# LarsELund/Bayesian-Neural-Nets

Hardware: AMD Instinct MI355X
Metric: ELBO forward samples/sec, 784-1200^2-10 MNF MLP, batch 4096 per GPU (higher is better)
Workload: dtype f16 (row-scaled fp16 hi + lo split of the f32 operands: 3 mean + 1 variance MFMA products, f32 accumulate)

## Files before the change

bayesian-neural-nets_amd/_lib.py:

```python
import ctypes
import os

_HERE = os.path.dirname(os.path.abspath(__file__))
LIB_PATH = os.environ.get("LBBNN_LIB_PATH") or os.path.join(_HERE, "csrc", "liblbbnn_hip.so")

c_p = ctypes.c_void_p
c_i = ctypes.c_int
c_u32 = ctypes.c_uint32
c_i64 = ctypes.c_int64
c_u64 = ctypes.c_uint64


class Priors(ctypes.Structure):
    _fields_ = [("mu_prior", ctypes.c_float), ("sigma_prior", ctypes.c_float),
                ("alpha_prior", ctypes.c_float), ("bias_mu_prior", ctypes.c_float),
                ("bias_sigma_prior", ctypes.c_float)]

    def __init__(self, mu_prior=0.0, sigma_prior=1.0, alpha_prior=0.05, bias_mu_prior=0.0,
                 bias_sigma_prior=1.0):
        super().__init__(mu_prior, sigma_prior, alpha_prior, bias_mu_prior, bias_sigma_prior)


MAX_FLOW_T = 16
MAX_LAYERS = 4
# ... 81 lines not shown


class AdamList(ctypes.Structure):
    _fields_ = [("p", c_p * ADAM_MAX_TENSORS), ("g", c_p * ADAM_MAX_TENSORS), ("m", c_p * ADAM_MAX_TENSORS),
                ("v", c_p * ADAM_MAX_TENSORS), ("numel", c_i64 * ADAM_MAX_TENSORS), ("n", c_i)]


ADAM_GROUPS_MAX_TENSORS = 64
ADAM_CHUNK = 4096
ADAM_F_DECOUPLED = 0x1
ADAM_F_INACTIVE = 0x2


class AdamHyper(ctypes.Structure):
    _fields_ = [("lr", ctypes.c_float), ("beta1", ctypes.c_float), ("beta2", ctypes.c_float), ("eps", ctypes.c_float),
                ("weight_decay", ctypes.c_float), ("flags", c_u32)]


class AdamGroupList(ctypes.Structure):
    _fields_ = [("p", c_p * ADAM_GROUPS_MAX_TENSORS), ("g", c_p * ADAM_GROUPS_MAX_TENSORS), ("m", c_p * ADAM_GROUPS_MAX_TENSORS),
                ("v", c_p * ADAM_GROUPS_MAX_TENSORS), ("mask", c_p * ADAM_GROUPS_MAX_TENSORS),
                ("numel", c_i64 * ADAM_GROUPS_MAX_TENSORS), ("group", c_i * ADAM_GROUPS_MAX_TENSORS), ("n", c_i)]


SGD_F_NESTEROV = 0x1
SGD_F_INACTIVE = 0x2


class SgdHyper(ctypes.Structure):
    _fields_ = [("lr", ctypes.c_float), ("momentum", ctypes.c_float), ("dampening", ctypes.c_float),
                ("weight_decay", ctypes.c_float), ("flags", c_u32)]


class StudyArgs(ctypes.Structure):
    _fields_ = [("params", c_p), ("exp_avg", c_p), ("exp_avg_sq", c_p), ("step", c_p), ("rng", c_p), ("skipped", c_p),
                ("x", c_p), ("x_rstride", c_i64), ("y", c_p), ("y_rstride", c_i64), ("priors", c_p), ("priors_rstride", c_i),
                ("hyper", c_p), ("lr", c_p), ("lr_rstride", c_i64), ("restarts", c_p), ("n_restarts", c_i), ("history", c_p),
                ("R", c_i), ("I", c_i), ("O", c_i), ("N", c_i), ("batch", c_i),
                ("epochs", c_i), ("first_epoch", c_i), ("n_epochs", c_i)]


STUDY_MAX_I, STUDY_MAX_O, STUDY_MAX_WEIGHTS, STUDY_MAX_BATCH, STUDY_HISTORY_COLS = 256, 16, 1024, 4096, 6


class CopyList(ctypes.Structure):
    _fields_ = [("dst", c_p * ADAM_MAX_TENSORS), ("src", c_p * ADAM_MAX_TENSORS), ("numel", c_i64 * ADAM_MAX_TENSORS), ("n", c_i)]


class DenseLayer(ctypes.Structure):
    _fields_ = [("q0_mean", c_p), ("q0_log_var", c_p), ("zt", ctypes.POINTER(DenseTransform)), ("rt", ctypes.POINTER(DenseTransform)),
                ("eps_fwd", c_p), ("eps_kl", c_p), ("z_fwd", c_p), ("z_kl", c_p), ("scal", c_p), ("work", c_p),
                ("Tz", c_i), ("Tr", c_i), ("I", c_i), ("want_kl", c_i), ("layer_id", c_u32), ("save", c_p), ("draw_masks", c_i)]


class DenseGrad(ctypes.Structure):
    _fields_ = [("w_in", c_p), ("b_in", c_p), ("w_mid", c_p * 3), ("b_mid", c_p * 3),
                ("w_a", c_p), ("b_a", c_p), ("w_b", c_p), ("b_b", c_p)]


MAX_DENSE_T = 8
MAX_HIDDEN = 128


class GateBwdArgs(ctypes.Structure):
    _fields_ = [(n, c_p) for n in ("mu", "rho", "gamma_alpha", "cgamma", "eps_w", "bias_mu", "bias_rho", "eps_b", "bias_a",
                                   "bias_b", "tau_b", "weight_a", "weight_b", "tau_w", "pa", "pb", "dW", "g_sum", "g_lp", "g_lq",
                                   "d_mu", "d_rho", "d_cgamma", "d_alpha", "w_out", "d_bias_mu", "d_bias_rho", "d_bias_a",
                                   "d_bias_b", "d_tau_b", "d_scalars", "rows")] + \
               [("O", c_i), ("I", c_i), ("exact", c_i), ("layer_id", c_u32)]


class GateDrawArgs(ctypes.Structure):
    _fields_ = [("g", GateArgs), ("lambdal", c_p), ("gammas", c_p), ("alpha", c_p), ("tau_w", c_p), ("tau_b", c_p),
                ("temperature", ctypes.c_float)]


class GateBwdDrawArgs(ctypes.Structure):
    _fields_ = [("g", GateBwdArgs), ("lambdal", c_p), ("d_lambdal", c_p), ("temperature", ctypes.c_float)]


class GateMemberDesc(ctypes.Structure):
    _fields_ = [(n, c_p) for n in ("mu", "rho", "lambdal", "bias_mu", "bias_rho", "w_out", "bias_out", "gate_rows", "gates")] + \
               [(n, c_i) for n in ("O", "I", "ld", "flags", "exact")] + [("layer_id", c_u32)]


class FrozenDesc(ctypes.Structure):
    _fields_ = [(n, c_p) for n in ("weight_mu", "weight_rho", "lambdal", "bias_rho", "q0_mean", "q0_log_var")] + \
               [("z_flow", PlanarFlow)] + \
               [(n, c_p) for n in ("e0", "e_w", "var_w", "bias_var", "kept_rows", "z_fwd", "e_w_members")] + \
               [("z_mstride", c_i64)] + [(n, c_i) for n in ("O", "I", "ld", "flags", "mode")] + \
               [("cut", ctypes.c_float), ("layer_id", c_u32)]


class CompactMap(ctypes.Structure):
    _fields_ = [("rows", c_p), ("cols", c_p), ("O_full", c_i), ("I_full", c_i)]


class SparseDesc(ctypes.Structure):
    _fields_ = [(n, c_p) for n in ("weight_mu", "weight_rho", "lambdal", "bias_rho", "row_ptr", "col", "mean", "var", "bias_var",
                                   "kept_rows")] + [("O", c_i), ("I", c_i), ("nnz", c_i), ("cut", ctypes.c_float)]


MAX_LEVELS = 16


class SparseLevelsDesc(ctypes.Structure):
    _fields_ = [(n, c_p) for n in ("weight_mu", "weight_rho", "lambdal", "bias_rho", "row_ptr", "col", "mean", "var", "bias_var",
                                   "kept_rows")] + [("O", c_i), ("I", c_i), ("nnz", c_i), ("levels", c_i),
                                                    ("cut", ctypes.c_float * MAX_LEVELS)]


class SparseDrawDesc(ctypes.Structure):
    _fields_ = [(n, c_p) for n in ("col", "mean", "var", "bias_mu", "bias_var", "z")] + [("z_mstride", c_i64), ("tpos", c_p), ("wt", c_p), ("w", c_p),
               ("w_mstride", c_i64), ("b", c_p), ("b_mstride", c_i64), ("O", c_i), ("I", c_i), ("nnz", c_i), ("layer_id", c_u32)]


class SparseGatherArgs(ctypes.Structure):
    _fields_ = [("ptr", c_p), ("idx", c_p), ("slot", c_p), ("w", c_p), ("w_mstride", c_i64), ("bias", c_p), ("b_mstride", c_i64),
                ("a", c_p), ("a_mstride", c_i64), ("h", c_p), ("h_mstride", c_i64), ("out", c_p), ("o_mstride", c_i64)] + \
               [(n, c_i) for n in ("lda", "ldh", "ldo", "B", "K", "N", "nnz", "mode", "relu", "out_rows", "a_shared", "blocks",
                                   "per_member")] + [("dot_bias", c_p), ("dot_b_mstride", c_i64), ("dot_acc", c_p)]


class MemberStatsArgs(ctypes.Structure):
    _fields_ = [("t", c_p), ("t_mstride", c_i64)] + [(n, c_i) for n in ("ldt", "S", "C", "F", "B")] + \
               [(n, c_p) for n in ("mean", "std", "prob_pos", "prob_neg", "members", "logits")] + \
               [("ldl", c_i), ("n_logits", c_i), ("targets", c_p), ("intercept", c_p), ("residual", c_p)]


class BaseSparseDesc(ctypes.Structure):
    _fields_ = [(n, c_p) for n in ("mu", "rho", "lambdal", "bias_mu", "bias_rho", "row_ptr", "col", "mean", "sigma", "b_mu",
                                   "b_sigma", "kept_rows")] + [("O", c_i), ("I", c_i), ("nnz", c_i)]


class BaseSparseDrawDesc(ctypes.Structure):
    _fields_ = [(n, c_p) for n in ("row_ptr", "col", "mean", "sigma", "b_mu", "b_sigma", "tpos", "wt", "w")] + \
               [("w_mstride", c_i64), ("b", c_p), ("b_mstride", c_i64), ("O", c_i), ("I", c_i), ("nnz", c_i), ("layer_id", c_u32)]


class BaseFrozenDesc(ctypes.Structure):
    _fields_ = [(n, c_p) for n in ("mu", "rho", "lambdal", "bias_mu", "bias_rho", "w_mu", "w_sigma", "alpha", "e_w", "b_mu",
                                   "b_sigma", "kept_rows", "alpha_rows", "keep")] + \
               [(n, c_i) for n in ("O", "I", "ld", "flags", "exact")] + [("layer_id", c_u32)]


class DenseMembers(ctypes.Structure):
    _fields_ = [("q0_mean", c_p), ("q0_log_var", c_p), ("zt", ctypes.POINTER(DenseTransform)), ("T", c_i), ("I", c_i),
                ("layer_id", c_u32), ("z_fwd", c_p), ("z_mstride", c_i64), ("mask_out", c_p)]


class OutGradArgs(ctypes.Structure):
    _fields_ = [(n, c_p) for n in ("g_out", "out", "std", "eps", "rng", "gm", "gv", "gmT", "gvT", "g_sum", "gv_sum", "work")] + \
               [("row_offset", c_i64), ("rng_stream", c_u32)] + [(n, c_i) for n in ("B", "O", "ldg", "ldo", "relu")] + \
               [("gv_scale", c_p)]


class FlowStep(ctypes.Structure):
    _fields_ = [("p0", c_p), ("p1", c_p), ("p2", c_p), ("type", c_i), ("M", c_i)]


class FlowChain(ctypes.Structure):
    _fields_ = [("step", FlowStep * MAX_FLOW_T), ("n", c_i)]


class PlanarGrad(ctypes.Structure):
    _fields_ = [("u", c_p * MAX_FLOW_T), ("w", c_p * MAX_FLOW_T), ("b", c_p * MAX_FLOW_T)]


class FlowBwdArgs(ctypes.Structure):
    _fields_ = [(n, c_p) for n in ("q0_mean", "q0_log_var", "eps_fwd", "eps_kl", "r0_b1", "r0_b2", "aux",
                                   "dz_fwd", "dz_kl", "g_kl", "bias_mu", "bias_rho", "g_sum", "gv_sum")] + \
               [("z_flow", PlanarFlow), ("r_flow", PlanarFlow), ("priors", Priors)] + \
               [(n, c_p) for n in ("d_q0_mean", "d_q0_log_var", "d_r0_b1", "d_r0_b2", "d_bias_mu", "d_bias_rho")] + \
               [("d_z_flow", PlanarGrad), ("d_r_flow", PlanarGrad), ("work", c_p), ("O", c_i), ("I", c_i),
                ("rng", c_p), ("layer_id", c_u32)]


class DenseBwdArgs(ctypes.Structure):
    _fields_ = [(n, c_p) for n in ("q0_mean", "q0_log_var", "eps_fwd", "eps_kl", "r0_b1", "r0_b2", "aux",
                                   "dz_fwd", "dz_kl", "g_kl", "bias_mu", "bias_rho", "g_sum", "gv_sum")] + \
               [("zt", ctypes.POINTER(DenseTransform)), ("rt", ctypes.POINTER(DenseTransform)),
                ("d_zt", ctypes.POINTER(DenseGrad)), ("d_rt", ctypes.POINTER(DenseGrad)), ("priors", Priors)] + \
               [(n, c_p) for n in ("d_q0_mean", "d_q0_log_var", "d_r0_b1", "d_r0_b2", "d_bias_mu", "d_bias_rho", "save", "work")] + \
               [("Tz", c_i), ("Tr", c_i), ("O", c_i), ("I", c_i), ("rng", c_p), ("layer_id", c_u32)]


EVAL_COUNTS = 6
EVAL_COUNT_NAMES = ("rows", "rows_with_target", "bad_targets", "correct_ensemble", "correct_posterior_mean",
                    "entropy_nonfinite")


class EvalMetricsArgs(ctypes.Structure):
    _fields_ = [("logp", c_p), ("m_stride", c_i64), ("ldp", c_i64), ("mean_logp", c_p), ("ldm", c_i64), ("target", c_p),
                ("ens_logp", c_p), ("pred_ensemble", c_p), ("pred_mean", c_p), ("entropy", c_p),
                ("counts", c_p), ("correct_member", c_p), ("confusion", c_p), ("sums", c_p), ("work", c_p),
                ("S", c_i), ("B", c_i), ("C", c_i)]


MONITOR_COUNTS = 8
MONITOR_COUNT_NAMES = ("steps", "rows", "correct", "bad_targets", "nonfinite_rows", "nonfinite_steps", "skipped_steps", "nll_rows")
MONITOR_SUMS = 5
MONITOR_SUM_NAMES = ("nll_sum", "kl_term_sum", "loss_sum", "last_nll", "last_loss")
MONITOR_WORDS = MONITOR_COUNTS + MONITOR_SUMS
MONITOR_SKIPPED_STEPS = 6


UNC_COUNTS = 6
UNC_COUNT_NAMES = ("rows", "rows_with_target", "bad_targets", "correct_bma", "nonfinite_rows", "log_score_nonfinite")
UNC_SUMS = 6
UNC_SUM_NAMES = ("total_entropy", "expected_entropy", "mutual_information", "confidence", "brier", "log_score")


class EvalUncertaintyArgs(ctypes.Structure):
    _fields_ = [("logp", c_p), ("m_stride", c_i64), ("ldp", c_i64), ("target", c_p),
                ("bma_probs", c_p), ("pred_bma", c_p), ("confidence", c_p), ("total_entropy", c_p), ("expected_entropy", c_p),
                ("mutual_information", c_p), ("brier", c_p), ("log_score", c_p),
                ("counts", c_p), ("sums", c_p), ("bin_rows", c_p), ("bin_rows_with_target", c_p), ("bin_correct", c_p),
                ("bin_conf_sum", c_p), ("hist", c_p), ("work", c_p),
                ("S", c_i), ("B", c_i), ("C", c_i), ("conf_bins", c_i), ("hist_bins", c_i), ("ent_scale", ctypes.c_float)]


REG_COUNTS = 5
REG_COUNT_NAMES = ("elements", "elements_with_target", "bad_targets", "nonfinite_elements", "scored_elements")
REG_SUMS = 8
REG_SUM_NAMES = ("sq_err", "abs_err", "log_density", "epistemic_var", "total_var", "y", "y2", "posterior_mean_sq_err")
REG_ROW_KEYS = ("pred_mean", "epistemic_var", "aleatoric_var", "total_std", "sq_err", "log_density", "pit")


class EvalRegressionArgs(ctypes.Structure):
    _fields_ = [("out", c_p), ("m_stride", c_i64), ("ldp", c_i64), ("mean_out", c_p), ("ldm", c_i64), ("target", c_p),
                ("ldt", c_i64), ("log_var", c_p)] + [(n, c_p) for n in REG_ROW_KEYS] + \
               [("counts", c_p), ("sums", c_p), ("pit_hist", c_p), ("work", c_p), ("S", c_i), ("B", c_i), ("O", c_i),
                ("pit_bins", c_i)]


SCORE_MAX_LEVELS = 4
SCORE_MAX_MEMBERS = 64
SCORE_COUNTS = REG_COUNTS + SCORE_MAX_LEVELS
SCORE_SUMS = REG_SUMS + 2 + 2 * SCORE_MAX_LEVELS
SCORE_SUM_NAMES = REG_SUM_NAMES + ("aleatoric_var", "crps")
SCORE_ROW_KEYS = REG_ROW_KEYS + ("crps",)
SCORE_LEVEL_KEYS = ("lower", "upper", "interval_score")


class EvalScoresArgs(ctypes.Structure):
    _fields_ = [("out", c_p), ("m_stride", c_i64), ("ldp", c_i64), ("mean_out", c_p), ("ldm", c_i64), ("target", c_p),
                ("ldt", c_i64), ("log_var", c_p), ("lv_mstride", c_i64), ("lv_ld", c_i64)] + \
               [(n, c_p) for n in SCORE_ROW_KEYS + SCORE_LEVEL_KEYS] + \
               [("counts", c_p), ("sums", c_p), ("pit_hist", c_p), ("work", c_p), ("S", c_i), ("B", c_i), ("O", c_i),
                ("pit_bins", c_i), ("n_levels", c_i), ("levels", ctypes.c_float * SCORE_MAX_LEVELS)]


STRUCTURE_MAX_LAYERS = 16
STRUCTURE_MAX_WIDTH = 4096


class StructureDesc(ctypes.Structure):
    _fields_ = [("lambdal", c_p), ("O", c_i), ("I", c_i), ("ld", c_i), ("layer_id", c_u32)]


EXPLAIN_SEED, EXPLAIN_MASK, EXPLAIN_FINISH = 0, 1, 2
GATHER_FORWARD, GATHER_SWEEP, GATHER_FINISH = 0, 1, 2
MEMBER_BLOCKS_MAX = 65535
EXPLAIN_MAX_OUTPUTS = 16
EXPLAIN_MAX_ROWS = 1 << 24


class ExplainStepArgs(ctypes.Structure):
    _fields_ = [("mode", c_i), ("B", c_i), ("C", c_i), ("width", c_i), ("g", c_p), ("ldg", c_i64), ("w", c_p), ("ldw", c_i64),
                ("w_rows", c_i), ("targets", c_p), ("h", c_p), ("ldh", c_i64), ("bias", c_p), ("bias_out", c_p),
                ("intercept", c_p), ("active", c_p), ("ld_active", c_i64), ("mask_out", c_p), ("ldm", c_i64),
                ("logits", c_p), ("ldl", c_i64), ("map", c_p), ("full_width", c_i), ("contributions", c_p), ("ldc", c_i64),
                ("residual", c_p)]


SIGNATURES = {
    "lbbnn_abi_version": (c_i, []),
    "lbbnn_error_string": (ctypes.c_char_p, [c_i]),
    "lbbnn_operand_ld": (c_i, [c_i]),
    "lbbnn_weight_pass": (c_i, [c_p, c_p, c_p, c_p, c_p, c_p, c_p, ctypes.POINTER(Priors),
                                c_p, c_p, c_i, c_p, c_p, c_p, c_p, c_i, c_i, c_i, c_p]),
    "lbbnn_weight_pass_f16": (c_i, [c_p, c_p, c_p, c_p, c_p, c_p, c_p, ctypes.POINTER(Priors),
                                    c_p, c_p, c_i, c_p, c_p, c_p, c_p, c_p, c_p, c_i, c_i, c_i, c_p]),
    "lbbnn_lrt_gemm_ex": (c_i, [ctypes.POINTER(GemmDesc), c_p]),
    "lbbnn_head_slab_floats": (c_i64, [c_i, c_i]),
    "lbbnn_format_x": (c_i, [c_p, c_i, c_p, c_i, c_i, c_i, c_p]),
    "lbbnn_lrt_gemm": (c_i, [c_p, c_i, c_p, c_p, c_i, c_p, c_p, c_p, c_p, c_p, c_u32, c_i64,
                             c_p, c_i, c_i, c_i, c_i, c_i, c_p]),
    "lbbnn_lrt_gemm_plan": (c_i, [c_i, c_i, c_i, c_i, c_i, c_i, c_i, c_i, c_i, ctypes.POINTER(GemmPlan)]),
    "lbbnn_transpose_operand": (c_i, [c_p, c_i, c_i, c_i, c_p, c_i, c_i, c_i, c_p]),
    "lbbnn_weight_pass_backward_workspace": (c_i64, [c_i, c_i]),
    "lbbnn_weight_pass_backward": (c_i, [ctypes.POINTER(WpbArgs), c_p]),
    "lbbnn_layers_dense_flows": (c_i, [ctypes.POINTER(DenseLayer), c_i, c_p, c_p]),
    "lbbnn_layers_dense_flows_phase": (c_i, [ctypes.POINTER(DenseLayer), c_i, c_p, c_i, c_p]),
    "lbbnn_flow_dense_save_size": (c_i64, [c_i, c_i, c_i]),
    "lbbnn_mnf_flow_dense_backward_workspace": (c_i64, [c_i]),
    "lbbnn_mnf_flow_dense_backward": (c_i, [ctypes.POINTER(DenseBwdArgs), c_p]),
    "lbbnn_mnf_flow_dense_backward_batch": (c_i, [ctypes.POINTER(DenseBwdArgs), c_i, c_p]),
    "lbbnn_flow_dense_apply_workspace": (c_i64, [c_i, c_i]),
    "lbbnn_flow_dense_apply": (c_i, [ctypes.POINTER(DenseTransform), c_i, c_i, c_p, c_i, c_p, c_p, c_p]),
    "lbbnn_flow_dense_apply_backward": (c_i, [ctypes.POINTER(DenseTransform), ctypes.POINTER(DenseGrad), c_i, c_i, c_p, c_p,
                                              c_p, c_i, c_p, c_p, c_p]),
    "lbbnn_q0_rows": (c_i, [c_p, c_p, c_p, c_p, c_u32, c_i, c_i, c_p, c_p]),
    "lbbnn_flow_dense_rows_max_dim": (c_i, []),
    "lbbnn_flow_dense_rows": (c_i, [ctypes.POINTER(DenseTransform), c_i, c_p, c_p, c_p, c_u32, c_u64, c_p, c_i, c_i, c_i,
                                    c_p, c_i, c_p, c_p]),
    "lbbnn_gate_backward": (c_i, [ctypes.POINTER(GateBwdArgs), c_p, c_p]),
    "lbbnn_format_operand": (c_i, [c_p, c_i, c_i, c_i, c_p, c_i, c_i, c_i, c_p]),
    "lbbnn_multi_copy": (c_i, [ctypes.POINTER(CopyList), c_p]),
    "lbbnn_adam_step": (c_i, [ctypes.POINTER(AdamList), ctypes.c_float, ctypes.c_float, ctypes.c_float, ctypes.c_float,
                              ctypes.c_float, c_p, c_i, c_p]),
    "lbbnn_adam_step_groups": (c_i, [ctypes.POINTER(AdamGroupList), c_p, c_p, c_i, c_p, c_p, c_i, c_p]),
    "lbbnn_sgd_step_groups": (c_i, [ctypes.POINTER(AdamGroupList), c_p, c_p, c_i, c_p, c_p, c_i, c_p]),
    "lbbnn_adam_step_groups_guarded": (c_i, [ctypes.POINTER(AdamGroupList), c_p, c_p, c_i, c_p, c_p, c_i, c_p, c_p, c_p]),
    "lbbnn_sgd_step_groups_guarded": (c_i, [ctypes.POINTER(AdamGroupList), c_p, c_p, c_i, c_p, c_p, c_i, c_p, c_p, c_p]),
    "lbbnn_lrt_study_fit": (c_i, [ctypes.POINTER(StudyArgs), c_p]),
    "lbbnn_grad_sumsq_workspace": (c_i64, [c_i64]),
    "lbbnn_grad_sumsq": (c_i, [ctypes.POINTER(AdamGroupList), c_p, c_i64, c_i64, ctypes.c_float, c_p, c_p, c_p]),
    "lbbnn_matmul_splitk": (c_i, [c_p, c_i, c_p, c_i, c_p, c_i, c_i, c_i, c_i, c_i, c_p]),
    "lbbnn_lrt_gemm_combine": (c_i, [c_p, c_i, c_p, c_i, c_p, c_i, c_p, c_i, c_p, c_i, c_i, c_i, c_i, c_i, c_p]),
    "lbbnn_dx_combine": (c_i, [c_p, c_p, c_p, c_i, c_i, c_i, c_p]),
    "lbbnn_output_grad_workspace": (c_i64, [c_i, c_i]),
    "lbbnn_output_grad": (c_i, [ctypes.POINTER(OutGradArgs), c_p]),
    "lbbnn_head_dx": (c_i, [c_p, c_p, c_i, c_p, c_p, c_i, c_p, c_i, c_p, c_i, c_i, c_i, c_i, c_p]),
    "lbbnn_head_dw": (c_i, [c_p, c_p, c_i, c_p, c_i, c_p, c_p, c_i, c_i, c_i, c_i, c_p]),
    "lbbnn_reduce_partials_batch": (c_i, [c_p, c_i, c_p]),
    "lbbnn_flow_chain": (c_i, [ctypes.POINTER(FlowChain), c_p, c_p, c_p, c_p, c_p, c_u32, c_i, c_p, c_p, c_p, c_p, c_p]),
    "lbbnn_flow_chain_rows": (c_i, [ctypes.POINTER(FlowChain), c_p, c_i, c_i, c_i, c_p, c_i, c_p, c_p]),
    "lbbnn_mnf_aux_backward": (c_i, [c_p, c_p, c_p, c_p, c_p, c_p, c_p, c_i, c_i, c_p, c_p, c_p, c_p, c_u32, c_p]),
    "lbbnn_mnf_aux_backward_batch": (c_i, [c_p, c_i, c_p]),
    "lbbnn_bias_backward": (c_i, [c_p, c_p, c_p, c_p, c_p, c_p, c_p, c_p, c_i, c_p]),
    "lbbnn_bias_backward_partials": (c_i, [c_p, c_i, c_i, c_i, c_p, c_p, c_p, c_p, c_p, c_p, c_p]),
    "lbbnn_mnf_flow_backward_workspace": (c_i64, [c_i, c_i, c_i]),
    "lbbnn_mnf_flow_planar_backward": (c_i, [ctypes.POINTER(FlowBwdArgs), c_p]),
    "lbbnn_mnf_flow_planar_backward_batch": (c_i, [ctypes.POINTER(FlowBwdArgs), c_i, c_p]),
    "lbbnn_mnf_flow_planar": (c_i, [c_p, c_p, c_p, c_p, c_p, c_i, c_p, c_p, c_p, c_i, c_p, c_p,
                                    c_p, c_u32, c_p, c_p, c_p, c_i, c_i, c_p]),
    "lbbnn_flow_dense_workspace": (c_i64, [c_i]),
    "lbbnn_mnf_flow_dense": (c_i, [c_p, c_p, ctypes.POINTER(DenseTransform), c_i, ctypes.POINTER(DenseTransform), c_i,
                                   c_p, c_p, c_p, c_u32, c_p, c_p, c_p, c_p, c_i, c_i, c_p]),
    "lbbnn_kl_finalize": (c_i, [c_p, c_p, c_p, c_i, c_p, c_p, c_p, c_p, c_p, c_i, c_p,
                                ctypes.POINTER(Priors), c_p, c_u32, c_p, c_p, c_i, c_p]),
    "lbbnn_flow_planar_form": (c_i, [c_i, c_p, c_p, c_p, c_p, c_p, c_i]),
    "lbbnn_kl_finalize_form": (c_i, [c_i, c_p, c_p, c_p, c_p, c_i]),
    "lbbnn_layers_prepare": (c_i, [ctypes.POINTER(LayerDesc), c_i, c_p, c_p]),
    "lbbnn_layers_operands_snap": (c_i, [ctypes.POINTER(LayerDesc), c_i, c_p, c_p, c_u64, c_p]),
    "lbbnn_layers_operands_x": (c_i, [ctypes.POINTER(LayerDesc), c_i, c_p, c_p, c_u64, c_p, c_i, c_p, c_i, c_i, c_i, c_p]),
    "lbbnn_ensemble_operands": (c_i, [ctypes.POINTER(LayerDesc), c_i, c_i, c_p, c_u64, c_p]),
    "lbbnn_lrt_gemm_members": (c_i, [c_p, c_i, c_i64, c_p, c_i64, c_p, c_i, c_p, c_p, c_p, c_u32, c_i64, c_u64,
                                     c_p, c_i, c_i64, c_i, c_i, c_i, c_i, c_i, c_p]),
    "lbbnn_layers_operands": (c_i, [ctypes.POINTER(LayerDesc), c_i, c_p, c_p]),
    "lbbnn_layers_finalize": (c_i, [ctypes.POINTER(LayerDesc), c_i, c_p, ctypes.c_uint64, c_p, c_p]),
    "lbbnn_kl_total": (c_i, [c_p, c_i, c_p, c_p]),
    "lbbnn_fold_rows": (c_i, [c_p, c_i, c_i, c_i, c_p, c_p]),
    "lbbnn_gate_sample": (c_i, [ctypes.POINTER(GateArgs), c_p, c_p]),
    "lbbnn_vd_operands": (c_i, [c_p, c_p, c_p, c_i, c_i, c_i, c_i, c_p]),
    "lbbnn_weight_operands_t": (c_i, [c_p, c_p, c_p, c_p, c_p, c_p, c_i, c_i, c_i, c_i, c_p]),
    "lbbnn_rng_advance": (c_i, [c_p, c_u64, c_p]),
    "lbbnn_philox_normal": (c_i, [c_p, c_u32, c_i64, c_i64, c_i64, c_p, c_p]),
    "lbbnn_gate_sample_draw": (c_i, [ctypes.POINTER(GateDrawArgs), c_p, c_p]),
    "lbbnn_gate_backward_draw": (c_i, [ctypes.POINTER(GateBwdDrawArgs), c_p, c_p]),
    "lbbnn_philox_uniform": (c_i, [c_p, c_u32, c_i64, c_i64, c_i64, c_p, c_p]),
    "lbbnn_gate_members": (c_i, [ctypes.POINTER(GateMemberDesc), c_i, c_i, c_i, ctypes.c_float, c_p, c_u64, c_p]),
    "lbbnn_gemm_members_mean": (c_i, [c_p, c_i, c_i64, c_p, c_i64, c_i, c_p, c_i64, c_p, c_i, c_i64, c_i, c_i, c_i, c_i, c_i,
                                      c_p]),
    "lbbnn_vd_gemm_members": (c_i, [c_p, c_i, c_i64, c_p, c_p, c_i, c_p, c_p, c_u32, c_i64, c_u64, c_p, c_i, c_i64,
                                    c_i, c_i, c_i, c_i, c_i, c_i, c_p]),
    "lbbnn_philox_std_gamma": (c_i, [c_p, c_u32, c_p, c_p, c_i64, c_p, c_p]),
    "lbbnn_gamma_grad": (c_i, [c_p, c_p, c_i64, c_p, c_p]),
    "lbbnn_elbo_loss": (c_i, [c_p, c_i, c_p, c_i, c_i, c_p, ctypes.c_float, c_p, c_p]),
    "lbbnn_elbo_loss_monitor": (c_i, [c_p, c_i, c_p, c_i, c_i, c_p, ctypes.c_float, c_p, c_p, c_p, c_p]),
    "lbbnn_elbo_loss_backward": (c_i, [c_p, c_p, c_i, c_i, ctypes.c_float, c_p, c_p, c_p]),
    "lbbnn_elbo_loss_backward_logits": (c_i, [c_p, c_p, c_p, c_i, c_i, c_i, ctypes.c_float, c_p, c_p, c_p, c_p]),
    "lbbnn_log_softmax_backward": (c_i, [c_p, c_i, c_p, c_i, c_p, c_i, c_i, c_i, c_p]),
    "lbbnn_log_softmax_rows": (c_i, [c_p, c_i, c_p, c_i, c_i, c_i, c_p]),
    "lbbnn_binary_head": (c_i, [c_p, c_i, c_i, c_i, c_p, c_i, c_p, c_i, c_p]),
    "lbbnn_elbo_bce_loss": (c_i, [c_p, c_i, c_p, c_i, c_i, c_i, c_p, ctypes.c_float, c_p, c_p, c_i, c_p]),
    "lbbnn_elbo_bce_loss_monitor": (c_i, [c_p, c_i, c_p, c_i, c_i, c_i, c_p, ctypes.c_float, c_p, c_p, c_i, c_p, c_p, c_p]),
    "lbbnn_elbo_bce_loss_backward": (c_i, [c_p, c_p, c_i, c_p, c_i, c_i, c_i, ctypes.c_float, c_p, c_p, c_p, c_p]),
    "lbbnn_sigmoid_backward": (c_i, [c_p, c_i, c_p, c_i, c_p, c_i, c_i, c_i, c_p]),
    "lbbnn_frozen_operands": (c_i, [ctypes.POINTER(FrozenDesc), c_i, c_p]),
    "lbbnn_frozen_members": (c_i, [ctypes.POINTER(FrozenDesc), c_i, c_i, c_p, c_u64, c_p]),
    "lbbnn_flow_dense_members_max_dim": (c_i, []),
    "lbbnn_flow_dense_members": (c_i, [ctypes.POINTER(DenseMembers), c_i, c_i, c_p, c_u64, c_p]),
    "lbbnn_frozen_members_dense": (c_i, [ctypes.POINTER(FrozenDesc), ctypes.POINTER(DenseMembers), c_i, c_i, c_p, c_u64, c_p]),
    "lbbnn_frozen_operands_compact": (c_i, [ctypes.POINTER(FrozenDesc), ctypes.POINTER(CompactMap), c_i, c_p]),
    "lbbnn_frozen_members_compact": (c_i, [ctypes.POINTER(FrozenDesc), ctypes.POINTER(CompactMap), c_i, c_i, c_p, c_u64, c_p]),
    "lbbnn_gather_columns": (c_i, [c_p, c_i, c_p, c_i, c_p, c_i, c_i, c_p]),
    "lbbnn_sparse_count": (c_i, [ctypes.POINTER(SparseDesc), c_i, c_p]),
    "lbbnn_sparse_pack": (c_i, [ctypes.POINTER(SparseDesc), c_i, c_p]),
    "lbbnn_frozen_members_z": (c_i, [ctypes.POINTER(FrozenDesc), c_i, c_i, c_p, c_u64, c_p]),
    "lbbnn_sparse_layer_members": (c_i, [c_p, c_p, c_p, c_p, c_i, c_p, c_p, c_p, c_i, c_i64, c_p, c_i64, c_p, c_u32, c_i64, c_u64,
                                         c_p, c_i, c_i64, c_i, c_i, c_i, c_i, c_i, c_i, c_p]),
    "lbbnn_sparse_count_levels": (c_i, [ctypes.POINTER(SparseLevelsDesc), c_i, c_p]),
    "lbbnn_sparse_pack_levels": (c_i, [ctypes.POINTER(SparseLevelsDesc), c_i, c_p]),
    "lbbnn_sparse_layer_levels": (c_i, [c_p, c_p, c_p, c_p, c_i, c_p, c_p, c_p, c_i, c_i64, c_p, c_i64, c_p, c_u32, c_i64, c_u64,
                                        c_p, c_i, c_i64, c_i, c_i, c_i, c_i, c_i, c_i, c_i, c_p]),
    "lbbnn_base_frozen_operands": (c_i, [ctypes.POINTER(BaseFrozenDesc), ctypes.POINTER(CompactMap), c_i, c_i, ctypes.c_float, c_p]),
    "lbbnn_base_frozen_members": (c_i, [ctypes.POINTER(BaseFrozenDesc), ctypes.POINTER(CompactMap), c_i, c_i, c_i, ctypes.c_float,
                                        ctypes.POINTER(c_p), ctypes.POINTER(c_p), ctypes.POINTER(c_p), c_p, c_u64, c_p]),
    "lbbnn_eval_metrics_work_bytes": (c_i64, [c_i, c_i, c_i]),
    "lbbnn_eval_metrics": (c_i, [ctypes.POINTER(EvalMetricsArgs), c_p]),
    "lbbnn_eval_uncertainty_work_bytes": (c_i64, [c_i, c_i, c_i, c_i]),
    "lbbnn_eval_uncertainty": (c_i, [ctypes.POINTER(EvalUncertaintyArgs), c_p]),
    "lbbnn_eval_regression_work_bytes": (c_i64, [c_i, c_i, c_i]),
    "lbbnn_eval_regression": (c_i, [ctypes.POINTER(EvalRegressionArgs), c_p]),
    "lbbnn_eval_regression_scores_work_bytes": (c_i64, [c_i, c_i, c_i, c_i]),
    "lbbnn_eval_regression_scores": (c_i, [ctypes.POINTER(EvalScoresArgs), c_p]),
    "lbbnn_elbo_gaussian_loss": (c_i, [c_p, c_i, c_p, c_i, c_p, c_i, c_i, c_i, c_p, ctypes.c_float, c_p, c_p, c_p, c_p]),
    "lbbnn_elbo_gaussian_loss_monitor": (c_i, [c_p, c_i, c_p, c_i, c_p, c_i, c_i, c_i, c_p, ctypes.c_float, c_p, c_p, c_p, c_p, c_p,
                                               c_p]),
    "lbbnn_elbo_gaussian_loss_backward": (c_i, [c_p, c_p, c_i, c_p, c_i, c_p, c_i, c_i, c_i, ctypes.c_float, c_p, c_p, c_p, c_p,
                                                c_p]),
    "lbbnn_gate_structure_width": (c_i64, [ctypes.POINTER(StructureDesc), c_i]),
    "lbbnn_gate_structure": (c_i, [ctypes.POINTER(StructureDesc), c_i, c_i, c_p, c_p, c_p, c_p, c_p, c_p, c_p, c_p]),
    "lbbnn_explain_step": (c_i, [ctypes.POINTER(ExplainStepArgs), c_p]),
    "lbbnn_explain_work_bytes": (c_i64, [c_i, c_i, c_i]),
    "lbbnn_explain_totals": (c_i, [c_p, c_i64, c_p, c_i, c_i, c_i, c_p, c_p, c_p, c_p, c_p]),
    "lbbnn_explain_operand": (c_i, [c_p, c_i, c_i, c_i, c_p, c_p]),
    "lbbnn_sparse_draw_members": (c_i, [ctypes.POINTER(SparseDrawDesc), c_i, c_i, c_p, c_i, c_p]),
    "lbbnn_sparse_gather_members": (c_i, [ctypes.POINTER(SparseGatherArgs), c_p]),
    "lbbnn_explain_seed": (c_i, [c_p, c_p, c_i, c_p, c_p, c_i64, c_p, c_i, c_p, c_i, c_i, c_i, c_i, c_p, c_u64, c_p]),
    "lbbnn_explain_member_stats": (c_i, [ctypes.POINTER(MemberStatsArgs), c_p]),
    "lbbnn_base_sparse_count": (c_i, [ctypes.POINTER(BaseSparseDesc), c_i, ctypes.c_float, c_p]),
    "lbbnn_base_sparse_pack": (c_i, [ctypes.POINTER(BaseSparseDesc), c_i, ctypes.c_float, c_p]),
    "lbbnn_base_sparse_draw_members": (c_i, [ctypes.POINTER(BaseSparseDrawDesc), c_i, c_i, c_p, c_u64, c_i, c_p]),
}

_lib = None


def lib():
    global _lib
    if _lib is None:
        if not os.path.exists(LIB_PATH):
            raise RuntimeError(
                "bnn_amd: HIP extension not built: %s is missing. Build it with "
                "`python -c 'import __graft_entry__ as g; g.build()'` or "
                "`make -C bayesian-neural-nets_amd/csrc` (hipcc, --offload-arch=gfx950). "
                "There is no CPU fallback." % LIB_PATH)
        l = ctypes.CDLL(LIB_PATH)
        for name, (res, args) in SIGNATURES.items():
            fn = getattr(l, name)
            fn.restype = res
            fn.argtypes = args
        _lib = l
    if RECORD is not None:
        return _Recorder(_lib)
    return _lib


RECORD = None


class _Recorder:
    def __init__(self, l):
        self._l = l

    def __getattr__(self, name):
        fn = getattr(self._l, name)

        def call(*args):
            if RECORD is not None and fn.argtypes and fn.argtypes[-1] is ctypes.c_void_p:
                RECORD.append((name, fn, args))
            return fn(*args)
        return call


def check(rc, what):
    if rc != 0:
        msg = lib().lbbnn_error_string(rc)
        raise RuntimeError("bnn_amd: %s failed (%d): %s" % (what, rc, msg.decode() if msg else "?"))
# ... 6 lines not shown
```

bayesian-neural-nets_amd/csrc/lrt_gemm.hip:

```cpp
#include <cstdlib>
#include "lbbnn_device.h"
#include "lbbnn_internal.h"
#include "kl_piggy.h"
#include "gemm_common.h"
#include "../../include/lbbnn.h"

namespace {

using namespace lbbnn;
typedef float floatx4 __attribute__((ext_vector_type(4)));

constexpr int BK = 16;
constexpr int LDS_LD = 20;

struct GemmArgs {
    const float* x; const float* e_w; const float* var_w;
    const float* bias_mean; const float* bias_var; const float* var_scale;
    const float* eps; const uint64_t* rng;
    float* out;
    float* std_out;
    long long row_offset;
    int ldx, ld, ldo, B, I, O;
    uint32_t rng_stream;
    int relu, log_softmax;
    int kchunk;
    long long split_stride;
    const float* comb_x; const float* comb_add;
    int ld_cx, ld_ca;
    FinalizePiggy fin;
    int single16;
    int members;
    long long x_ms, w_ms, o_ms, b_ms;
    unsigned long long m_adv, m_off;
    int fan;
};

__device__ __forceinline__ GemmArgs member_view(const GemmArgs& in) {
    GemmArgs a = in;
    a.m_off = 0;
    if (in.members > 1) {
        const long long m = blockIdx.z;
        a.x = in.x + m * in.x_ms; a.e_w = in.e_w + m * in.w_ms; a.out = in.out + m * in.o_ms;
        if (in.bias_mean) a.bias_mean = in.bias_mean + m * in.b_ms;
        a.m_off = (unsigned long long)m * in.m_adv;
    }
    return a;
}

struct EpiCtx { bool ovec; uint64_t seed, offs; };

template <bool MEAN_ONLY>
__device__ __forceinline__ EpiCtx make_epi_ctx(const GemmArgs& a) {
    EpiCtx c;
    c.ovec = ((a.O & 3) == 0) && ((a.ldo & 3) == 0) && ((reinterpret_cast<uintptr_t>(a.out) & 15u) == 0) &&
             (!a.eps || (reinterpret_cast<uintptr_t>(a.eps) & 15u) == 0) &&
             (!a.std_out || (reinterpret_cast<uintptr_t>(a.std_out) & 15u) == 0);
    c.seed = 0; c.offs = 0;
    if (!MEAN_ONLY && !a.eps) { c.seed = a.rng[0]; c.offs = a.rng[1] + a.m_off; }
    return c;
}

struct OConst { float bm[4], bv[4], vs[4]; };

__device__ __forceinline__ void load4_or_fill(const float* p, int o, int O, float fill, float out[4]) {
    if (!p) { out[0] = out[1] = out[2] = out[3] = fill; return; }
    if (o + 3 < O && ((reinterpret_cast<uintptr_t>(p + o) & 15u) == 0)) {
        const float4 t = *reinterpret_cast<const float4*>(p + o);
        out[0] = t.x; out[1] = t.y; out[2] = t.z; out[3] = t.w;
    } else {
#pragma unroll
        for (int r = 0; r < 4; ++r) out[r] = (o + r < O) ? p[o + r] : fill;
    }
}

__device__ __forceinline__ OConst load_oconst(const GemmArgs& a, int o) {
    OConst c;
    load4_or_fill(a.bias_mean, o, a.O, 0.f, c.bm);
    load4_or_fill(a.bias_var, o, a.O, 0.f, c.bv);
    load4_or_fill(a.var_scale, o, a.O, 1.f, c.vs);
    return c;
}

template <bool MEAN_ONLY>
__device__ __forceinline__ void epilogue4(const GemmArgs& a, const EpiCtx& c, const OConst& oc, int b, int o,
                                          const floatx4& am, const floatx4& av, const float* e_in, const float* cx_in,
                                          const float* ca_in, float res[4], float sd[4]) {
    float e[4] = {0.f, 0.f, 0.f, 0.f};
    if (!MEAN_ONLY) {
        if (a.eps) {
#pragma unroll
            for (int r = 0; r < 4; ++r) e[r] = e_in[r];
        } else {
            philox_normal4(c.seed, c.offs, a.rng_stream, (uint64_t)(a.row_offset + b), (uint32_t)(o >> 2), e);
        }
    }
#pragma unroll
    for (int r = 0; r < 4; ++r) {
        float mean = am[r] + oc.bm[r];
        sd[r] = 0.f;
        if (!MEAN_ONLY) { sd[r] = sqrt_hw(av[r] * oc.vs[r] + oc.bv[r]); mean += sd[r] * e[r]; }
        res[r] = a.relu ? fmaxf(mean, 0.f) : mean;
    }
    if (MEAN_ONLY && a.comb_x) {
#pragma unroll
        for (int r = 0; r < 4; ++r) res[r] = ca_in[r] + 2.f * cx_in[r] * res[r];
    }
}

__device__ __forceinline__ void load4_rows(const float* p, bool vec, int o, int O, float out[4]) {
    if (vec) { const float4 t = *reinterpret_cast<const float4*>(p); out[0] = t.x; out[1] = t.y; out[2] = t.z; out[3] = t.w; }
    else {
#pragma unroll
        for (int r = 0; r < 4; ++r) out[r] = (o + r < O) ? p[r] : 0.f;
    }
}

__device__ __forceinline__ void store4_rows(float* p, bool vec, int o, int O, const float v[4]) {
    if (vec) *reinterpret_cast<float4*>(p) = make_float4(v[0], v[1], v[2], v[3]);
    else {
#pragma unroll
        for (int r = 0; r < 4; ++r) if (o + r < O) p[r] = v[r];
    }
}

__device__ __forceinline__ void fan_store4(const GemmArgs& a, const EpiCtx& ec, const OConst& oc, int m, int b, int o,
                                           const floatx4& am, const floatx4& av) {
    EpiCtx em = ec;
    em.offs = ec.offs + (unsigned long long)m * a.m_adv;
    float res[4], sd[4];
    epilogue4<false>(a, em, oc, b, o, am, av, nullptr, nullptr, nullptr, res, sd);
    store4_rows(a.out + (size_t)m * a.o_ms + (size_t)b * a.ldo + o, ec.ovec, o, a.O, res);
}

template <int TO, int TB, bool MEAN_ONLY, bool FAN = false>
__device__ __forceinline__ void epilogue_tile(const GemmArgs& a, int o0, int q, int brow0,
                                              const floatx4 (&accm)[TO][TB], const floatx4 (&accv)[TO][TB]) {
    static_assert(!FAN || !MEAN_ONLY, "fan-out draws noise");
    EpiCtx ec = make_epi_ctx<MEAN_ONLY>(a);
    OConst oc[TO];
#pragma unroll
    for (int i = 0; i < TO; ++i) {
        const int o = o0 + i * 16 + 4 * q;
        if (o < a.O) oc[i] = load_oconst(a, o);
    }
    if (FAN) {
        __builtin_amdgcn_sched_barrier(0);
        for (int m = 0; m < a.fan; ++m) {
#pragma unroll
            for (int i = 0; i < TO; ++i) {
                const int o = o0 + i * 16 + 4 * q;
                if (o >= a.O) continue;
#pragma unroll
                for (int j = 0; j < TB; ++j) {
                    const int b = brow0 + j * 16;
                    if (b < a.B) fan_store4(a, ec, oc[i], m, b, o, accm[i][j], accv[i][j]);
                }
            }
        }
        return;
    }
    const bool pre_eps = !MEAN_ONLY && a.eps != nullptr;
    const bool pre_comb = MEAN_ONLY && a.comb_x != nullptr;
    const bool comb_vec = pre_comb && ec.ovec && ((a.ld_cx | a.ld_ca) & 3) == 0 &&
                          ((reinterpret_cast<uintptr_t>(a.comb_x) | reinterpret_cast<uintptr_t>(a.comb_add)) & 15u) == 0;
    float pa[TO][TB][4], pb[TO][TB][4];
    if (pre_eps || pre_comb) {
#pragma unroll
        for (int i = 0; i < TO; ++i) {
            const int o = o0 + i * 16 + 4 * q;
#pragma unroll
            for (int j = 0; j < TB; ++j) {
                const int b = brow0 + j * 16;
                if (o >= a.O || b >= a.B) continue;
                if (pre_eps) load4_rows(a.eps + (size_t)b * a.O + o, ec.ovec, o, a.O, pa[i][j]);
                else {
                    load4_rows(a.comb_x + (size_t)b * a.ld_cx + o, comb_vec, o, a.O, pa[i][j]);
                    load4_rows(a.comb_add + (size_t)b * a.ld_ca + o, comb_vec, o, a.O, pb[i][j]);
                }
            }
        }
    }
    __builtin_amdgcn_sched_barrier(0);
#pragma unroll
    for (int i = 0; i < TO; ++i) {
        const int o = o0 + i * 16 + 4 * q;
        if (o >= a.O) continue;
#pragma unroll
        for (int j = 0; j < TB; ++j) {
            const int b = brow0 + j * 16;
            if (b >= a.B) continue;
            float res[4], sd[4];
            epilogue4<MEAN_ONLY>(a, ec, oc[i], b, o, accm[i][j], accv[i][j], pa[i][j], pa[i][j], pb[i][j], res, sd);
            store4_rows(a.out + (size_t)b * a.ldo + o, ec.ovec, o, a.O, res);
            if (!MEAN_ONLY && a.std_out) store4_rows(a.std_out + (size_t)b * a.O + o, ec.ovec, o, a.O, sd);
        }
    }
}

template <int TO, int TB, int WB, bool MEAN_ONLY, bool XVEC, bool FAN = false>
__global__ __launch_bounds__(WB * 64, 2) void lrt_gemm_f32_kernel(const GemmArgs a_in) {
    const GemmArgs a = member_view(a_in);
    constexpr int NT = WB * 64;
    constexpr int BN = TO * 16;
    constexpr int BM = TB * WB * 16;
    constexpr int NW = MEAN_ONLY ? 1 : 2;
    extern __shared__ __attribute__((aligned(16))) float smem[];
    constexpr int ROWS = BM + NW * BN;
    constexpr int BUF = ROWS * LDS_LD;

    const int tid = threadIdx.x, lane = tid & 63, wv = tid >> 6;
    const int lr = lane & 15, q = lane >> 4;
    const int o0 = blockIdx.x * BN;
    const int b0 = blockIdx.y * BM;

    constexpr int SLOTS = ROWS * 4;
    constexpr int NIT = (SLOTS + NT - 1) / NT;
    const float* gp[NIT];
    int loff[NIT];
    int kcol[NIT];
#pragma unroll
    for (int it = 0; it < NIT; ++it) {
        int sl = tid + it * NT;
        if (sl >= SLOTS) sl -= SLOTS;
        const int row = sl >> 2, c4 = (sl & 3) << 2;
        loff[it] = row * LDS_LD + c4;
        if (row < BM) {
            const int bb = min(b0 + row, a.B - 1);
            gp[it] = a.x + (size_t)bb * a.ldx + c4;
            kcol[it] = c4;
        } else {
            const int wr = row - BM;
            const bool isv = (!MEAN_ONLY) && wr >= BN;
            const int oo = min(o0 + (isv ? wr - BN : wr), a.O - 1);
            gp[it] = (isv ? a.var_w : a.e_w) + (size_t)oo * a.ld + c4;
            kcol[it] = -1;
        }
    }
    float4 stage[NIT];
    auto load_full = [&](int c) {
#pragma unroll
        for (int it = 0; it < NIT; ++it) {
            const float* p = gp[it] + c * BK;
            if (XVEC) stage[it] = *reinterpret_cast<const float4*>(p);
            else if (kcol[it] < 0) stage[it] = *reinterpret_cast<const float4*>(p);
            else stage[it] = make_float4(p[0], p[1], p[2], p[3]);
        }
    };
    auto load_tail = [&](int c) {
#pragma unroll
        for (int it = 0; it < NIT; ++it) {
            const float* p = gp[it] + c * BK;
            if (kcol[it] < 0) {
                stage[it] = *reinterpret_cast<const float4*>(p);
            } else {
                const int k = c * BK + kcol[it];
                float4 v = make_float4(0.f, 0.f, 0.f, 0.f);
                if (k + 0 < a.I) v.x = p[0];
                if (k + 1 < a.I) v.y = p[1];
                if (k + 2 < a.I) v.z = p[2];
                if (k + 3 < a.I) v.w = p[3];
                stage[it] = v;
            }
        }
    };
    auto store_chunk = [&](float* buf) {
#pragma unroll
        for (int it = 0; it < NIT; ++it) *reinterpret_cast<float4*>(buf + loff[it]) = stage[it];
    };

    floatx4 accm[TO][TB], accv[TO][TB];
#pragma unroll
    for (int i = 0; i < TO; ++i)
#pragma unroll
        for (int j = 0; j < TB; ++j) { accm[i][j] = floatx4{0.f, 0.f, 0.f, 0.f}; accv[i][j] = floatx4{0.f, 0.f, 0.f, 0.f}; }

    const int nfull = a.I / BK;
    const int nchunks = (a.I + BK - 1) / BK;
    if (nfull > 0) load_full(0); else load_tail(0);
    store_chunk(smem);
    __syncthreads();

    const int xoff = (wv * TB * 16 + lr) * LDS_LD + 4 * q;
    const int woff = (BM + lr) * LDS_LD + 4 * q;

    auto compute = [&](const float* cur) {
        float xf[TB][4], xs[TB][4], wm[TO][4], wq[TO][4];
#pragma unroll
        for (int j = 0; j < TB; ++j) {
            const float4 t = *reinterpret_cast<const float4*>(cur + xoff + j * 16 * LDS_LD);
            xf[j][0] = t.x; xf[j][1] = t.y; xf[j][2] = t.z; xf[j][3] = t.w;
        }
#pragma unroll
        for (int i = 0; i < TO; ++i) {
            const float4 t = *reinterpret_cast<const float4*>(cur + woff + i * 16 * LDS_LD);
            wm[i][0] = t.x; wm[i][1] = t.y; wm[i][2] = t.z; wm[i][3] = t.w;
            if (!MEAN_ONLY) {
                const float4 u = *reinterpret_cast<const float4*>(cur + woff + (BN + i * 16) * LDS_LD);
                wq[i][0] = u.x; wq[i][1] = u.y; wq[i][2] = u.z; wq[i][3] = u.w;
            }
        }
#pragma unroll
        for (int j = 0; j < TB; ++j)
#pragma unroll
            for (int k = 0; k < 4; ++k) xs[j][k] = xf[j][k] * xf[j][k];
#pragma unroll
        for (int k = 0; k < 4; ++k) {
#pragma unroll
            for (int i = 0; i < TO; ++i) {
#pragma unroll
                for (int j = 0; j < TB; ++j) {
                    accm[i][j] = __builtin_amdgcn_mfma_f32_16x16x4f32(wm[i][k], xf[j][k], accm[i][j], 0, 0, 0);
                    if (!MEAN_ONLY)
                        accv[i][j] = __builtin_amdgcn_mfma_f32_16x16x4f32(wq[i][k], xs[j][k], accv[i][j], 0, 0, 0);
                }
            }
        }
    };

    int c = 0;
    for (; c + 1 < nfull; ++c) {
        load_full(c + 1);
        __builtin_amdgcn_sched_barrier(0);
        compute(smem + (c & 1) * BUF);
        __builtin_amdgcn_sched_barrier(0);
        store_chunk(smem + ((c & 1) ^ 1) * BUF);
        __syncthreads();
    }
    for (; c < nchunks; ++c) {
        const bool more = (c + 1) < nchunks;
        if (more) load_tail(c + 1);
        __builtin_amdgcn_sched_barrier(0);
        compute(smem + (c & 1) * BUF);
        __builtin_amdgcn_sched_barrier(0);
        if (more) store_chunk(smem + ((c & 1) ^ 1) * BUF);
        __syncthreads();
    }

    epilogue_tile<TO, TB, MEAN_ONLY, FAN>(a, o0, q, b0 + wv * TB * 16 + lr, accm, accv);
}

constexpr int DROW = 16;

__device__ __forceinline__ int swz(int rowgrp) { return (0x78 >> (2 * (rowgrp & 3))) & 3; }

template <int TO, int TB, int WB, bool MEAN_ONLY, bool FAN = false>
__global__ __launch_bounds__(WB * 64, 2) void lrt_gemm_f32_dma_kernel(const GemmArgs a_in) {
    const GemmArgs a = member_view(a_in);
    constexpr int BN = TO * 16, BM = TB * WB * 16;
    constexpr int NW = MEAN_ONLY ? 1 : 2;
    constexpr int ROWS = BM + NW * BN;
    constexpr int NG = ROWS / 16;
    constexpr int NPW = (NG + WB - 1) / WB;
    constexpr int BUF = ROWS * DROW;
    extern __shared__ __attribute__((aligned(16))) float smem[];

    const int tid = threadIdx.x, lane = tid & 63;
    const int wv = __builtin_amdgcn_readfirstlane(tid >> 6);
    const int lr = lane & 15, q = lane >> 4;
    if (a.fin.n > 0 && blockIdx.y == gridDim.y - 1) {
        if (blockIdx.x == 0) kl_finalize_piggy<WB>(kernarg_as<GemmArgs>()->fin, smem);
        return;
    }
    int tox, tby;
    tile_of_block(tox, tby, a.fin.n > 0 ? 1 : 0);
    const int o0 = tox * BN;
    const int b0 = tby * BM;

    const int srow = lane >> 2;
    const int scol = ((lane & 3) ^ swz(lane >> 4)) << 2;
    const float* gp[NPW];
#pragma unroll
    for (int u = 0; u < NPW; ++u) {
        const int g = wv + WB * u;
        const int row = 16 * g + srow;
        if (row < BM) {
            gp[u] = a.x + (size_t)min(b0 + row, a.B - 1) * a.ldx + scol;
        } else {
            const int wr = row - BM;
            const bool isv = (!MEAN_ONLY) && wr >= BN;
            const int oo = min(o0 + (isv ? wr - BN : wr), a.O - 1);
            gp[u] = (isv ? a.var_w : a.e_w) + (size_t)oo * a.ld + scol;
        }
    }
    auto dma_chunk = [&](int c, float* buf) {
#pragma unroll
        for (int u = 0; u < NPW; ++u) {
            const int g = wv + WB * u;
            if (g < NG)
                __builtin_amdgcn_global_load_lds(
                    (const __attribute__((address_space(1))) void*)(gp[u] + c * BK),
                    (__attribute__((address_space(3))) void*)(buf + g * 16 * DROW), 16, 0, 0);
        }
    };

    floatx4 accm[TO][TB], accv[TO][TB];
#pragma unroll
    for (int i = 0; i < TO; ++i)
#pragma unroll
        for (int j = 0; j < TB; ++j) { accm[i][j] = floatx4{0.f, 0.f, 0.f, 0.f}; accv[i][j] = floatx4{0.f, 0.f, 0.f, 0.f}; }

    const int fcol = (q ^ swz(lr >> 2)) << 2;
    const int xoff = (wv * TB * 16 + lr) * DROW + fcol;
    const int woff = (BM + lr) * DROW + fcol;

    float xf[TB][4], xs[TB][4], wm[TO][4], wq[TO][4];
    auto read_frags = [&](const float* cur) {
#pragma unroll
        for (int j = 0; j < TB; ++j) {
            const float4 t = *reinterpret_cast<const float4*>(cur + xoff + j * 16 * DROW);
            xf[j][0] = t.x; xf[j][1] = t.y; xf[j][2] = t.z; xf[j][3] = t.w;
        }
#pragma unroll
        for (int i = 0; i < TO; ++i) {
            const float4 t = *reinterpret_cast<const float4*>(cur + woff + i * 16 * DROW);
            wm[i][0] = t.x; wm[i][1] = t.y; wm[i][2] = t.z; wm[i][3] = t.w;
            if (!MEAN_ONLY) {
                const float4 u = *reinterpret_cast<const float4*>(cur + woff + (BN + i * 16) * DROW);
                wq[i][0] = u.x; wq[i][1] = u.y; wq[i][2] = u.z; wq[i][3] = u.w;
            }
        }
    };
    auto mfmas = [&]() {
#pragma unroll
        for (int j = 0; j < TB; ++j)
#pragma unroll
            for (int k = 0; k < 4; ++k) xs[j][k] = xf[j][k] * xf[j][k];
#pragma unroll
        for (int k = 0; k < 4; ++k) {
#pragma unroll
            for (int i = 0; i < TO; ++i) {
#pragma unroll
                for (int j = 0; j < TB; ++j) {
                    accm[i][j] = __builtin_amdgcn_mfma_f32_16x16x4f32(wm[i][k], xf[j][k], accm[i][j], 0, 0, 0);
                    if (!MEAN_ONLY)
                        accv[i][j] = __builtin_amdgcn_mfma_f32_16x16x4f32(wq[i][k], xs[j][k], accv[i][j], 0, 0, 0);
                }
            }
        }
    };

    const int nchunks = a.I / BK;
    dma_chunk(0, smem);
    __syncthreads();
    for (int c = 0; c < nchunks; ++c) {
        read_frags(smem + (c & 1) * BUF);
        __builtin_amdgcn_sched_barrier(0);
        if (c + 1 < nchunks) dma_chunk(c + 1, smem + ((c & 1) ^ 1) * BUF);
        __builtin_amdgcn_sched_barrier(0);
        mfmas();
        __builtin_amdgcn_sched_barrier(0);
        __syncthreads();
    }

    epilogue_tile<TO, TB, MEAN_ONLY, FAN>(a, o0, q, b0 + wv * TB * 16 + lr, accm, accv);
}

typedef __bf16 bf16x8 __attribute__((ext_vector_type(8)));
typedef __bf16 bf16x2 __attribute__((ext_vector_type(2)));
typedef float floatx2 __attribute__((ext_vector_type(2)));
constexpr int BKS = 32;

__device__ __forceinline__ int swzx(int r) { return (((r >> 1) & 3) << 1) | ((r >> 3) & 1); }

typedef _Float16 f16x8 __attribute__((ext_vector_type(8)));
typedef _Float16 f16x2 __attribute__((ext_vector_type(2)));
template <int TO, int TB, int WB, bool MEAN_ONLY, int NP, bool F16, bool FAN>
__device__ __forceinline__ void lrt_gemm_bf16x3_body(const GemmArgs& a_in) {
    static_assert(!F16 || NP == 1, "fp16 operands exist in the single-product form only");
    const GemmArgs a = member_view(a_in);
    constexpr int BN = TO * 16, BM = TB * WB * 16;
    constexpr int NWR = MEAN_ONLY ? 1 : 2;
    constexpr int XB = BM * 128;
    constexpr int WRB = BN * 128;
    constexpr int BUFB = XB + NWR * WRB;
    constexpr int NGX = BM / 8, NGW = BN / 8;
    constexpr int NG = NGX + NWR * NGW;
    constexpr int NPW = (NG + WB - 1) / WB;
    extern __shared__ __attribute__((aligned(16))) char smc[];

    const int tid = threadIdx.x, lane = tid & 63;
    const int wv = __builtin_amdgcn_readfirstlane(tid >> 6);
    const int lr = lane & 15, q = lane >> 4;
    if (a.fin.n > 0 && blockIdx.y == gridDim.y - 1) {
        if (blockIdx.x == 0) kl_finalize_piggy<WB>(kernarg_as<GemmArgs>()->fin, reinterpret_cast<float*>(smc));
        return;
    }
    int tox, tby;
    tile_of_block(tox, tby, a.fin.n > 0 ? 1 : 0);
    const int o0 = tox * BN;
    const int b0 = tby * BM;
    const int kbeg = a.kchunk ? (int)blockIdx.z * a.kchunk : 0;
    const int Iloc = a.kchunk ? min(a.I - kbeg, a.kchunk) : a.I;
    const char* const eb = reinterpret_cast<const char*>(a.e_w);
    const char* const vb = reinterpret_cast<const char*>(a.var_w);
    const char* const zsrc = eb + split_hi_index(0, a.I, a.ld) * 2;

    const unsigned xbytes = (unsigned)min((size_t)0x7FFFFFF0u, ((size_t)(a.B - 1) * a.ldx + a.I) * 4);
    const unsigned wbytes = (unsigned)min((size_t)0x7FFFFFF0u, (size_t)a.O * a.ld * 4);
    const __amdgpu_buffer_rsrc_t rx = __builtin_amdgcn_make_buffer_rsrc((void*)a.x, 0, (int)xbytes, 0x00020000);
    const __amdgpu_buffer_rsrc_t re = __builtin_amdgcn_make_buffer_rsrc((void*)a.e_w, 0, (int)wbytes, 0x00020000);
    const __amdgpu_buffer_rsrc_t rv = __builtin_amdgcn_make_buffer_rsrc((void*)(MEAN_ONLY ? a.e_w : a.var_w), 0, (int)wbytes, 0x00020000);
    (void)eb; (void)vb; (void)zsrc;
    int gv[NPW];
    int kx[NPW];
#pragma unroll
    for (int u = 0; u < NPW; ++u) {
        const int g = wv + WB * u;
        if (g < NGX) {
            const int row = 8 * g + (lane >> 3);
            const int slot = (lane & 7) ^ swzx(row & 15);
            gv[u] = (int)(((size_t)min(b0 + row, a.B - 1) * a.ldx + kbeg) * 4) + 16 * slot;
            kx[u] = 4 * slot;
        } else {
            const int gw = g - NGX, row = 8 * (gw % NGW) + (lane >> 3);
            const int slot = (lane & 7) ^ swzx(row & 15);
            gv[u] = (int)((size_t)min(o0 + row, a.O - 1) * a.ld * 4) + (kbeg >> 5) * 128 + 16 * slot;
            kx[u] = -1;
        }
    }
    const int nsteps = (Iloc + BKS - 1) / BKS;
    const bool has_tail = (Iloc % BKS) != 0;
    int gvt[NPW];
#pragma unroll
    for (int u = 0; u < NPW; ++u)
        gvt[u] = (kx[u] >= 0 && (nsteps - 1) * BKS + kx[u] >= Iloc) ? 0x7FFFFFF0 : gv[u];
    auto dma_pieces = [&](int c, char* buf, const int (&va)[NPW]) {
#pragma unroll
        for (int u = 0; u < NPW; ++u) {
            const int g = wv + WB * u;
            if (g < NG) {
                const int loff = g < NGX ? g * 1024 : XB + (g - NGX) * 1024;
                auto* dst = (__attribute__((address_space(3))) void*)(buf + loff);
                if (g < NGX)                 __builtin_amdgcn_raw_ptr_buffer_load_lds(rx, dst, 16, va[u], c * 128, 0, 0);
                else if (g - NGX < NGW)      __builtin_amdgcn_raw_ptr_buffer_load_lds(re, dst, 16, va[u], c * 128, 0, 0);
                else                         __builtin_amdgcn_raw_ptr_buffer_load_lds(rv, dst, 16, va[u], c * 128, 0, 0);
            }
        }
    };
    auto dma_step = [&](int c, char* buf) {
        if (has_tail && c == nsteps - 1) dma_pieces(c, buf, gvt);
        else dma_pieces(c, buf, gv);
    };

    floatx4 accm[TO][TB], accv[TO][TB];
#pragma unroll
    for (int i = 0; i < TO; ++i)
#pragma unroll
        for (int j = 0; j < TB; ++j) { accm[i][j] = floatx4{0.f, 0.f, 0.f, 0.f}; accv[i][j] = floatx4{0.f, 0.f, 0.f, 0.f}; }

    const int gx = swzx(lr);
    const int xo0 = (wv * TB * 16 + lr) * 128 + 16 * ((2 * q) ^ gx);
    const int xo1 = (wv * TB * 16 + lr) * 128 + 16 * ((2 * q + 1) ^ gx);
    const int woh = XB + lr * 128 + 16 * ((2 * q) ^ gx);
    const int wol = XB + lr * 128 + 16 * ((2 * q + 1) ^ gx);

    float4 xr[TB][2];
    uint4 wh[TO], wl[TO], wvh[TO], wvl[TO];
    auto read_frags = [&](const char* cur) {
#pragma unroll
        for (int j = 0; j < TB; ++j) {
            xr[j][0] = *reinterpret_cast<const float4*>(cur + xo0 + j * 16 * 128);
            xr[j][1] = *reinterpret_cast<const float4*>(cur + xo1 + j * 16 * 128);
        }
#pragma unroll
        for (int i = 0; i < TO; ++i) {
            wh[i] = *reinterpret_cast<const uint4*>(cur + woh + i * 16 * 128);
            if (NP == 3) wl[i] = *reinterpret_cast<const uint4*>(cur + wol + i * 16 * 128);
            if (!MEAN_ONLY) {
                wvh[i] = *reinterpret_cast<const uint4*>(cur + WRB + woh + i * 16 * 128);
                if (NP == 3) wvl[i] = *reinterpret_cast<const uint4*>(cur + WRB + wol + i * 16 * 128);
            }
        }
    };
    auto mfmas = [&]() {
        bf16x8 xh[TB], xl[TB], sh[TB], sl[TB];
#pragma unroll
        for (int j = 0; j < TB; ++j) {
            const float v[8] = {xr[j][0].x, xr[j][0].y, xr[j][0].z, xr[j][0].w, xr[j][1].x, xr[j][1].y, xr[j][1].z, xr[j][1].w};
            uint32_t ph[4], pl[4], qh[4], ql[4];
#pragma unroll
            for (int t = 0; t < 4; ++t) {
                if (NP == 1) {
                    const floatx2 hv = {v[2 * t], v[2 * t + 1]};
                    ph[t] = F16 ? __builtin_bit_cast(uint32_t, __builtin_convertvector(hv, f16x2))
                                : __builtin_bit_cast(uint32_t, __builtin_convertvector(hv, bf16x2));
                    pl[t] = 0; qh[t] = 0; ql[t] = 0;
                    if (!MEAN_ONLY) {
                        const floatx2 sv = {v[2 * t] * v[2 * t], v[2 * t + 1] * v[2 * t + 1]};
                        qh[t] = F16 ? __builtin_bit_cast(uint32_t, __builtin_convertvector(sv, f16x2))
                                    : __builtin_bit_cast(uint32_t, __builtin_convertvector(sv, bf16x2));
                    }
                    continue;
                }
                const uint32_t u0 = __float_as_uint(v[2 * t]), u1 = __float_as_uint(v[2 * t + 1]);
                ph[t] = __builtin_amdgcn_perm(u1, u0, 0x07060302);
                const floatx2 lo = {v[2 * t] - __uint_as_float(u0 & 0xFFFF0000u), v[2 * t + 1] - __uint_as_float(u1 & 0xFFFF0000u)};
                pl[t] = __builtin_bit_cast(uint32_t, __builtin_convertvector(lo, bf16x2));
                if (!MEAN_ONLY) {
                    const float s0 = v[2 * t] * v[2 * t], s1 = v[2 * t + 1] * v[2 * t + 1];
                    const uint32_t w0 = __float_as_uint(s0), w1 = __float_as_uint(s1);
                    qh[t] = __builtin_amdgcn_perm(w1, w0, 0x07060302);
                    const floatx2 slo = {s0 - __uint_as_float(w0 & 0xFFFF0000u), s1 - __uint_as_float(w1 & 0xFFFF0000u)};
                    ql[t] = __builtin_bit_cast(uint32_t, __builtin_convertvector(slo, bf16x2));
                }
            }
            xh[j] = __builtin_bit_cast(bf16x8, make_uint4(ph[0], ph[1], ph[2], ph[3]));
            xl[j] = __builtin_bit_cast(bf16x8, make_uint4(pl[0], pl[1], pl[2], pl[3]));
            if (!MEAN_ONLY) {
                sh[j] = __builtin_bit_cast(bf16x8, make_uint4(qh[0], qh[1], qh[2], qh[3]));
                sl[j] = __builtin_bit_cast(bf16x8, make_uint4(ql[0], ql[1], ql[2], ql[3]));
            }
        }
#pragma unroll
        for (int j = 0; j < TB; ++j) {
#pragma unroll
            for (int i = 0; i < TO; ++i) {
                if (F16) {
                    accm[i][j] = __builtin_amdgcn_mfma_f32_16x16x32_f16(__builtin_bit_cast(f16x8, wh[i]), __builtin_bit_cast(f16x8, xh[j]),
                                                                        accm[i][j], 0, 0, 0);
                    if (!MEAN_ONLY)
                        accv[i][j] = __builtin_amdgcn_mfma_f32_16x16x32_f16(__builtin_bit_cast(f16x8, wvh[i]), __builtin_bit_cast(f16x8, sh[j]),
                                                                            accv[i][j], 0, 0, 0);
                    continue;
                }
                const bf16x8 ah = __builtin_bit_cast(bf16x8, wh[i]);
                const bf16x8 al = NP == 3 ? __builtin_bit_cast(bf16x8, wl[i]) : ah;
                accm[i][j] = __builtin_amdgcn_mfma_f32_16x16x32_bf16(ah, xh[j], accm[i][j], 0, 0, 0);
                if (NP == 3) {
                    accm[i][j] = __builtin_amdgcn_mfma_f32_16x16x32_bf16(al, xh[j], accm[i][j], 0, 0, 0);
                    accm[i][j] = __builtin_amdgcn_mfma_f32_16x16x32_bf16(ah, xl[j], accm[i][j], 0, 0, 0);
                }
                if (!MEAN_ONLY) {
                    const bf16x8 bh = __builtin_bit_cast(bf16x8, wvh[i]);
                    accv[i][j] = __builtin_amdgcn_mfma_f32_16x16x32_bf16(bh, sh[j], accv[i][j], 0, 0, 0);
                    if (NP == 3) {
                        accv[i][j] = __builtin_amdgcn_mfma_f32_16x16x32_bf16(__builtin_bit_cast(bf16x8, wvl[i]), sh[j], accv[i][j], 0, 0, 0);
                        accv[i][j] = __builtin_amdgcn_mfma_f32_16x16x32_bf16(bh, sl[j], accv[i][j], 0, 0, 0);
                    }
                }
            }
        }
    };

    dma_step(0, smc);
    __syncthreads();
    for (int c = 0; c < nsteps; ++c) {
        read_frags(smc + (c & 1) * BUFB);
        __builtin_amdgcn_sched_barrier(0);
        if (c + 1 < nsteps) dma_step(c + 1, smc + ((c & 1) ^ 1) * BUFB);
        __builtin_amdgcn_sched_barrier(0);
        mfmas();
        __builtin_amdgcn_sched_barrier(0);
        __syncthreads();
    }

    GemmArgs ao = a;
    if (a.kchunk) ao.out = a.out + (size_t)blockIdx.z * a.split_stride;
    epilogue_tile<TO, TB, MEAN_ONLY, FAN>(ao, o0, q, b0 + wv * TB * 16 + lr, accm, accv);
}
template <int TO, int TB, int WB, bool MEAN_ONLY, int NP = 3, bool F16 = false, bool FAN = false>
__global__ __launch_bounds__(WB * 64, (TB * TO > 10) ? 1 : (WB == 8 ? 4 : 2)) void lrt_gemm_bf16x3_kernel(const GemmArgs a_in) {
    lrt_gemm_bf16x3_body<TO, TB, WB, MEAN_ONLY, NP, F16, FAN>(a_in);
}


constexpr int SK_WAVES = 16;
constexpr int SK_NCH = 5;

template <bool MEAN_ONLY, bool XVEC, bool FAN = false>
__global__ __launch_bounds__(SK_WAVES * 64) void lrt_gemm_skinny_kernel(const GemmArgs a_in) {
    static_assert(!FAN || !MEAN_ONLY, "fan-out draws noise");
    const GemmArgs a = member_view(a_in);
    __shared__ __attribute__((aligned(16))) float red[SK_WAVES][2][64][4];
    const int tid = threadIdx.x, lane = tid & 63, wv = tid >> 6;
    const int lr = lane & 15, q = lane >> 4;
    constexpr int SKR = 16;
    const int b0 = blockIdx.x * SKR;
    const int b = b0 + lr;
    const bool brow = b < a.B && lr < SKR, orow = lr < a.O;
    floatx4 accm = {0.f, 0.f, 0.f, 0.f}, accv = {0.f, 0.f, 0.f, 0.f};
    const EpiCtx ec = make_epi_ctx<MEAN_ONLY>(a);
    const int o = 4 * q;
    const bool live = brow && o < a.O;
    OConst oc;
    float pa[4] = {0.f, 0.f, 0.f, 0.f}, pb[4] = {0.f, 0.f, 0.f, 0.f};
    if (wv == 0 && live) {
        oc = load_oconst(a, o);
        if (!MEAN_ONLY && a.eps) load4_rows(a.eps + (size_t)b * a.O + o, ec.ovec, o, a.O, pa);
        if (MEAN_ONLY && a.comb_x) {
            const bool cvec = ec.ovec && ((a.ld_cx | a.ld_ca) & 3) == 0 &&
                              ((reinterpret_cast<uintptr_t>(a.comb_x) | reinterpret_cast<uintptr_t>(a.comb_add)) & 15u) == 0;
            load4_rows(a.comb_x + (size_t)b * a.ld_cx + o, cvec, o, a.O, pa);
            load4_rows(a.comb_add + (size_t)b * a.ld_ca + o, cvec, o, a.O, pb);
        }
    }
    const int nchunks = (a.I + BK - 1) / BK;
    for (int cb = wv; cb < nchunks; cb += SK_WAVES * SK_NCH) {
        float4 xf[SK_NCH], wm[SK_NCH], wvv[SK_NCH];
#pragma unroll
        for (int u = 0; u < SK_NCH; ++u) {
            const int c = cb + u * SK_WAVES;
            const int k = c * BK + 4 * q;
            float4 vx = make_float4(0.f, 0.f, 0.f, 0.f), vm = vx, vv = vx;
            if (c < nchunks) {
                if (brow) {
                    const float* p = a.x + (size_t)b * a.ldx + k;
                    if (XVEC) { if (k < a.I) vx = *reinterpret_cast<const float4*>(p); }
                    else {
                        if (k + 0 < a.I) vx.x = p[0];
                        if (k + 1 < a.I) vx.y = p[1];
                        if (k + 2 < a.I) vx.z = p[2];
                        if (k + 3 < a.I) vx.w = p[3];
                    }
                }
                if (orow) {
                    vm = *reinterpret_cast<const float4*>(a.e_w + (size_t)lr * a.ld + k);
                    if (!MEAN_ONLY) vv = *reinterpret_cast<const float4*>(a.var_w + (size_t)lr * a.ld + k);
                }
            }
            xf[u] = vx; wm[u] = vm; wvv[u] = vv;
        }
#pragma unroll
        for (int u = 0; u < SK_NCH; ++u) {
            accm = __builtin_amdgcn_mfma_f32_16x16x4f32(wm[u].x, xf[u].x, accm, 0, 0, 0);
            accm = __builtin_amdgcn_mfma_f32_16x16x4f32(wm[u].y, xf[u].y, accm, 0, 0, 0);
            accm = __builtin_amdgcn_mfma_f32_16x16x4f32(wm[u].z, xf[u].z, accm, 0, 0, 0);
            accm = __builtin_amdgcn_mfma_f32_16x16x4f32(wm[u].w, xf[u].w, accm, 0, 0, 0);
            if (!MEAN_ONLY) {
                accv = __builtin_amdgcn_mfma_f32_16x16x4f32(wvv[u].x, xf[u].x * xf[u].x, accv, 0, 0, 0);
                accv = __builtin_amdgcn_mfma_f32_16x16x4f32(wvv[u].y, xf[u].y * xf[u].y, accv, 0, 0, 0);
                accv = __builtin_amdgcn_mfma_f32_16x16x4f32(wvv[u].z, xf[u].z * xf[u].z, accv, 0, 0, 0);
                accv = __builtin_amdgcn_mfma_f32_16x16x4f32(wvv[u].w, xf[u].w * xf[u].w, accv, 0, 0, 0);
            }
        }
    }
    *reinterpret_cast<floatx4*>(&red[wv][0][lane][0]) = accm;
    if (!MEAN_ONLY) *reinterpret_cast<floatx4*>(&red[wv][1][lane][0]) = accv;
    __syncthreads();
    if (wv != 0) return;
    floatx4 sm = *reinterpret_cast<const floatx4*>(&red[0][0][lane][0]);
    floatx4 sv = {0.f, 0.f, 0.f, 0.f};
    if (!MEAN_ONLY) sv = *reinterpret_cast<const floatx4*>(&red[0][1][lane][0]);
#pragma unroll 3
    for (int w = 1; w < SK_WAVES; ++w) {
        sm += *reinterpret_cast<const floatx4*>(&red[w][0][lane][0]);
        if (!MEAN_ONLY) sv += *reinterpret_cast<const floatx4*>(&red[w][1][lane][0]);
    }
    if (FAN) {
        if (live)
            for (int m = 0; m < a.fan; ++m) fan_store4(a, ec, oc, m, b, o, sm, sv);
        return;
    }
    float res[4] = {0.f, 0.f, 0.f, 0.f}, sd[4] = {0.f, 0.f, 0.f, 0.f};
    if (live) epilogue4<MEAN_ONLY>(a, ec, oc, b, o, sm, sv, pa, pa, pb, res, sd);
    if (a.log_softmax) {
        float mx = -INFINITY;
#pragma unroll
        for (int r = 0; r < 4; ++r) if (live && o + r < a.O) mx = fmaxf(mx, res[r]);
        mx = fmaxf(mx, __shfl_xor(mx, 16, 64));
        mx = fmaxf(mx, __shfl_xor(mx, 32, 64));
        float se = 0.f;
#pragma unroll
        for (int r = 0; r < 4; ++r) if (live && o + r < a.O) se += expf(res[r] - mx);
        se += __shfl_xor(se, 16, 64);
        se += __shfl_xor(se, 32, 64);
        const float lse = mx + logf(se);
#pragma unroll
        for (int r = 0; r < 4; ++r) res[r] -= lse;
    }
    if (live) {
        store4_rows(a.out + (size_t)b * a.ldo + o, ec.ovec, o, a.O, res);
        if (!MEAN_ONLY && a.std_out) store4_rows(a.std_out + (size_t)b * a.O + o, ec.ovec, o, a.O, sd);
    }
}

struct PlanIn {
    int B, I, O, ldx;
    bool x_aligned;
    int flags, members, fan, kchunk;
    int ld;
    bool solo;
};

int plan_check(const PlanIn& p) {
    if (p.B <= 0 || p.I <= 0 || p.O <= 0 || p.ldx < p.I) return LBBNN_E_SHAPE;
    const int flags = p.flags;
    if (flags & ~(LBBNN_F_RELU | LBBNN_F_MEAN_ONLY | LBBNN_F_SPLIT16 | LBBNN_F_LOG_SOFTMAX | LBBNN_F_SINGLE16 | LBBNN_F_HALF16))
        return LBBNN_E_FLAGS;
    if ((flags & LBBNN_F_HALF16) && (!(flags & LBBNN_F_SINGLE16) || (flags & LBBNN_F_MEAN_ONLY))) return LBBNN_E_FLAGS;
    if ((flags & LBBNN_F_LOG_SOFTMAX) && (p.O > 16 || (flags & LBBNN_F_RELU))) return LBBNN_E_FLAGS;
    if ((flags & LBBNN_F_SINGLE16) && !(flags & LBBNN_F_SPLIT16)) return LBBNN_E_FLAGS;
    return 0;
}

constexpr int kPlanLarge = 1 << 2, kPlanXvec = 1 << 3, kPlanMean = 1 << 4, kPlanFan = 1 << 5, kPlanSingle = 1 << 6,
              kPlanHalf = 1 << 7;

int plan_select(const PlanIn& p, lbbnn_gemm_plan_t& out) {
    const int B = p.B, I = p.I, O = p.O;
    const bool split = (p.flags & LBBNN_F_SPLIT16) != 0;
    const bool mean_only = (p.flags & LBBNN_F_MEAN_ONLY) != 0;
    const bool solo = p.solo || p.kchunk;
    if (p.kchunk && !(split && mean_only)) return LBBNN_E_FLAGS;
    if (p.members > 1 && solo) return LBBNN_E_FLAGS;
    if (p.fan && (p.members != 1 || mean_only || solo || (p.flags & LBBNN_F_LOG_SOFTMAX))) return LBBNN_E_FLAGS;

    const bool xvec = ((I & 3) == 0) && ((p.ldx & 3) == 0) && p.x_aligned;
    lbbnn_gemm_plan_t pl{};
    pl.mean_only = mean_only; pl.fan = p.fan > 0; pl.products = 1;
    if (split) {
        const bool tail = (I % BKS) != 0;
        if (!xvec || (I & 7) || O <= 16 || (p.ld && tail && (p.ld - I) < 8)) return LBBNN_E_ALIGN;
        if (((size_t)(B - 1) * p.ldx + I) * 4 >= 0x7FFFFFF0u || (p.ld && (size_t)O * p.ld * 4 >= 0x7FFFFFF0u)) return LBBNN_E_SHAPE;
        const long nz = p.kchunk ? (I + p.kchunk - 1) / p.kchunk : 1;
        const long blocks_big = (long)((O + 79) / 80) * ((B + 127) / 128) * nz;
        pl.family = LBBNN_GEMM_SPLIT; pl.xvec = 1;
        pl.large_tile = blocks_big >= 256 && B >= 96;
        if ((p.flags & LBBNN_F_SINGLE16) && !mean_only) { pl.products = 1; pl.half = (p.flags & LBBNN_F_HALF16) != 0; }
        else pl.products = 3;
    } else if (O <= 16) {
        pl.family = LBBNN_GEMM_SKINNY; pl.xvec = xvec;
    } else {
        static const bool no_dma = getenv("LBBNN_GEMM_NO_DMA") != nullptr;
        const long blocks_big = (long)((O + 79) / 80) * ((B + 127) / 128);
        pl.large_tile = blocks_big >= 256;
        const bool dma = xvec && (I % BK) == 0 && !no_dma;
        pl.family = dma ? LBBNN_GEMM_DMA : LBBNN_GEMM_STAGED; pl.xvec = xvec;
    }
    pl.kernel_id = pl.family | (pl.large_tile ? kPlanLarge : 0) | (pl.xvec ? kPlanXvec : 0) | (pl.mean_only ? kPlanMean : 0) |
                   (pl.fan ? kPlanFan : 0) | ((pl.family == LBBNN_GEMM_SPLIT && pl.products == 1) ? kPlanSingle : 0) |
                   (pl.half ? kPlanHalf : 0);
    out = pl;
    return 0;
}

template <int TO, int TB, int WB>
int launch_f32(GemmArgs& a, const lbbnn_gemm_plan_t& p, hipStream_t s, bool* hosted) {
    constexpr int BN = TO * 16, BM = TB * WB * 16;
    dim3 grid((a.O + BN - 1) / BN, (a.B + BM - 1) / BM, a.members > 1 ? a.members : 1);
    dim3 block(WB * 64);
    const long nblocks = (long)grid.x * grid.y * grid.z;
    const int fin_n = a.fin.n;
    a.fin.n = 0;
    if (p.family == LBBNN_GEMM_DMA) {
        const size_t l_full = lds_request(2u * (BM + 2 * BN) * DROW * sizeof(float), nblocks);
        const size_t l_mean = lds_request(2u * (BM + BN) * DROW * sizeof(float), nblocks);
        if (fin_n > 0 && hosted) {
            a.fin.n = fin_n;
            if (piggy_lds_bytes(a.fin) <= (p.mean_only ? l_mean : l_full)) { grid.y += 1; *hosted = true; }
            else a.fin.n = 0;
        }
        if (p.fan) return launch_one(lrt_gemm_f32_dma_kernel<TO, TB, WB, false, true>, grid, block, l_full, s, a);
        if (p.mean_only) return launch_one(lrt_gemm_f32_dma_kernel<TO, TB, WB, true>, grid, block, l_mean, s, a);
        return launch_one(lrt_gemm_f32_dma_kernel<TO, TB, WB, false>, grid, block, l_full, s, a);
    }
    const size_t lds_full = lds_request(2u * (BM + 2 * BN) * LDS_LD * sizeof(float), nblocks);
    const size_t lds_mean = lds_request(2u * (BM + BN) * LDS_LD * sizeof(float), nblocks);
    if (p.fan) {
        if (p.xvec) return launch_one(lrt_gemm_f32_kernel<TO, TB, WB, false, true, true>, grid, block, lds_full, s, a);
        return launch_one(lrt_gemm_f32_kernel<TO, TB, WB, false, false, true>, grid, block, lds_full, s, a);
    }
    if (p.mean_only) {
        if (p.xvec) return launch_one(lrt_gemm_f32_kernel<TO, TB, WB, true, true>, grid, block, lds_mean, s, a);
        return launch_one(lrt_gemm_f32_kernel<TO, TB, WB, true, false>, grid, block, lds_mean, s, a);
    }
    if (p.xvec) return launch_one(lrt_gemm_f32_kernel<TO, TB, WB, false, true>, grid, block, lds_full, s, a);
    return launch_one(lrt_gemm_f32_kernel<TO, TB, WB, false, false>, grid, block, lds_full, s, a);
}

template <int TO, int TB, int WB>
int launch_split(GemmArgs& a, const lbbnn_gemm_plan_t& p, hipStream_t s, bool* hosted) {
    constexpr int BN = TO * 16, BM = TB * WB * 16;
    dim3 grid((a.O + BN - 1) / BN, (a.B + BM - 1) / BM,
              a.kchunk ? (a.I + a.kchunk - 1) / a.kchunk : (a.members > 1 ? a.members : 1));
    dim3 block(WB * 64);
    const long nblocks = (long)grid.x * grid.y * grid.z;
    const size_t l_full = lds_request(2u * (BM * 128 + 2 * BN * 128), nblocks);
    const size_t l_mean = lds_request(2u * (BM * 128 + 1 * BN * 128), nblocks);
    const int fin_n = a.fin.n;
    a.fin.n = 0;
    if (fin_n > 0 && hosted && !a.kchunk) {
        a.fin.n = fin_n;
        if (piggy_lds_bytes(a.fin) <= (p.mean_only ? l_mean : l_full)) { grid.y += 1; *hosted = true; }
        else a.fin.n = 0;
    }
    if (p.fan) {
        if (p.half) return launch_one(lrt_gemm_bf16x3_kernel<TO, TB, WB, false, 1, true, true>, grid, block, l_full, s, a);
        if (p.products == 1) return launch_one(lrt_gemm_bf16x3_kernel<TO, TB, WB, false, 1, false, true>, grid, block, l_full, s, a);
        return launch_one(lrt_gemm_bf16x3_kernel<TO, TB, WB, false, 3, false, true>, grid, block, l_full, s, a);
    }
    if (p.half) return launch_one(lrt_gemm_bf16x3_kernel<TO, TB, WB, false, 1, true>, grid, block, l_full, s, a);
    if (p.products == 1) return launch_one(lrt_gemm_bf16x3_kernel<TO, TB, WB, false, 1>, grid, block, l_full, s, a);
    if (p.mean_only) return launch_one(lrt_gemm_bf16x3_kernel<TO, TB, WB, true>, grid, block, l_mean, s, a);
    return launch_one(lrt_gemm_bf16x3_kernel<TO, TB, WB, false>, grid, block, l_full, s, a);
}

int launch_skinny(GemmArgs& a, const lbbnn_gemm_plan_t& p, hipStream_t s) {
    a.fin.n = 0;
    dim3 grid((a.B + 15) / 16, 1, a.members > 1 ? a.members : 1), block(SK_WAVES * 64);
    if (p.fan) {
        if (p.xvec) hipLaunchKernelGGL((lrt_gemm_skinny_kernel<false, true, true>), grid, block, 0, s, a);
        else        hipLaunchKernelGGL((lrt_gemm_skinny_kernel<false, false, true>), grid, block, 0, s, a);
    } else if (p.mean_only) {
        if (p.xvec) hipLaunchKernelGGL((lrt_gemm_skinny_kernel<true, true>), grid, block, 0, s, a);
        else        hipLaunchKernelGGL((lrt_gemm_skinny_kernel<true, false>), grid, block, 0, s, a);
    } else {
        if (p.xvec) hipLaunchKernelGGL((lrt_gemm_skinny_kernel<false, true>), grid, block, 0, s, a);
        else        hipLaunchKernelGGL((lrt_gemm_skinny_kernel<false, false>), grid, block, 0, s, a);
    }
    return (int)hipGetLastError();
}

int launch_plan(GemmArgs& a, const lbbnn_gemm_plan_t& p, hipStream_t s, bool* hosted) {
    switch (p.family) {
        case LBBNN_GEMM_SKINNY: return launch_skinny(a, p, s);
        case LBBNN_GEMM_SPLIT:
            return p.large_tile ? launch_split<5, 2, 4>(a, p, s, hosted) : launch_split<5, 1, 2>(a, p, s, hosted);
        default:
            return p.large_tile ? launch_f32<5, 2, 4>(a, p, s, hosted) : launch_f32<5, 1, 2>(a, p, s, hosted);
    }
}

}

static GemmArgs gemm_args(const float* x, int ldx, const void* e_w, const void* var_w, int ld, float* out, int ldo,
                          int B, int I, int O) {
    GemmArgs a{};
    a.x = x; a.e_w = static_cast<const float*>(e_w); a.var_w = static_cast<const float*>(var_w); a.out = out;
    a.ldx = ldx; a.ld = ld; a.ldo = ldo; a.B = B; a.I = I; a.O = O; a.members = 1;
    return a;
}

static int lrt_gemm_dispatch(GemmArgs& a, int flags, void* stream, bool* hosted = nullptr) {
    const int B = a.B, I = a.I, O = a.O, ld = a.ld;
    if (B == 0 && I > 0 && O > 0) return 0;
    if (!a.x || !a.e_w || !a.out) return LBBNN_E_NULL;
    if (a.ldo < O) return LBBNN_E_SHAPE;
    PlanIn pin{B, I, O, a.ldx, (reinterpret_cast<uintptr_t>(a.x) & 15u) == 0, flags, a.members, a.fan, a.kchunk, ld,
               a.fin.n > 0 || a.eps || a.std_out || a.comb_x};
    if (const int rc = plan_check(pin)) return rc;
    const bool mean_only = (flags & LBBNN_F_MEAN_ONLY) != 0;
    if (!mean_only && !a.var_w) return LBBNN_E_NULL;
    if (!mean_only && !a.eps && !a.rng) return LBBNN_E_NOISE;
    if (ld < I || (ld & 31)) return LBBNN_E_ALIGN;
    if ((reinterpret_cast<uintptr_t>(a.e_w) & 15u) || (reinterpret_cast<uintptr_t>(a.var_w) & 15u)) return LBBNN_E_ALIGN;

    a.relu = (flags & LBBNN_F_RELU) ? 1 : 0; a.log_softmax = (flags & LBBNN_F_LOG_SOFTMAX) ? 1 : 0;
    a.single16 = (flags & LBBNN_F_HALF16) ? 2 : ((flags & LBBNN_F_SINGLE16) ? 1 : 0);
    a.split_stride = (long long)B * a.ldo; a.m_off = 0;
    lbbnn_gemm_plan_t plan;
    if (const int rc = plan_select(pin, plan)) return rc;
    return launch_plan(a, plan, static_cast<hipStream_t>(stream), hosted);
}

extern "C" int lbbnn_lrt_gemm_plan(int B, int I, int O, int ldx, int x_aligned, int flags, int members, int fan, int kchunk,
                                   lbbnn_gemm_plan_t* plan) {
    if (!plan) return LBBNN_E_NULL;
    *plan = lbbnn_gemm_plan_t{};
    plan->family = LBBNN_GEMM_NONE; plan->kernel_id = -1;
    if (members < 1 || members > 65535 || fan < 0 || fan > 65535) return LBBNN_E_SHAPE;
    if (kchunk < 0 || (kchunk & 31)) return LBBNN_E_ALIGN;
    if (B == 0 && I > 0 && O > 0) return 0;
    const PlanIn pin{B, I, O, ldx, x_aligned != 0, flags, members, fan, kchunk, 0, false};
    if (const int rc = plan_check(pin)) return rc;
    return plan_select(pin, *plan);
}

extern "C" int lbbnn_lrt_gemm(const float* x, int ldx, const void* e_w, const void* var_w, int ld,
                              const float* bias_mean, const float* bias_var, const float* var_scale,
                              const float* eps, const uint64_t* rng, uint32_t rng_stream, int64_t row_offset,
                              float* out, int ldo, int B, int I, int O, int flags, void* stream) {
    GemmArgs a = gemm_args(x, ldx, e_w, var_w, ld, out, ldo, B, I, O);
    a.bias_mean = bias_mean; a.bias_var = bias_var; a.var_scale = var_scale;
    a.eps = eps; a.rng = rng; a.rng_stream = rng_stream; a.row_offset = row_offset;
    return lrt_gemm_dispatch(a, flags, stream);
}

int lbbnn::gemm_desc_f32(const lbbnn_gemm_desc_t& d, void* stream) {
    const int flags = d.flags, n = d.n_layers;
    if ((flags & (LBBNN_F_VAR1 | LBBNN_F_XPLANES)) || d.mean_scale || d.wvar_scale || d.out_planes || d.head_out) return LBBNN_E_FLAGS;
    if (n < 0 || (n > 0 && !d.layers)) return LBBNN_E_SHAPE;
    if (d.advance && !d.rng_live) return LBBNN_E_NULL;
    if ((flags & LBBNN_F_MEAN_ONLY) && d.std_out) return LBBNN_E_FLAGS;
    GemmArgs a = gemm_args(static_cast<const float*>(d.x), d.ldx, d.e_w, d.var_w, d.ld, d.out, d.ldo, d.B, d.I, d.O);
    a.bias_mean = d.bias_mean; a.bias_var = d.bias_var; a.var_scale = d.var_scale;
    a.eps = d.eps; a.rng = d.rng; a.rng_stream = d.rng_stream; a.row_offset = d.row_offset; a.std_out = d.std_out;
    if (n == 0) {
        const int rc = lrt_gemm_dispatch(a, flags, stream);
        if (rc || !d.advance) return rc;
        return lbbnn_rng_advance(d.rng_live, d.advance, stream);
    }
    FinalizePiggy& fin = a.fin;
    if (const int rc = fill_finalize_args(d.layers, n, d.fin_rng, fin.l, fin.active)) return rc;
    if (d.kl_total) for (int i = 0; i < n; ++i) if (!fin.active[i]) return LBBNN_E_NULL;
    fin.n = n; fin.total = d.kl_total;
    fin.rng_adv = d.advance ? d.rng_live : nullptr; fin.adv = d.advance;
    bool hosted = false;
    const int rc = lrt_gemm_dispatch(a, flags, stream, &hosted);
    if (rc) return rc;
    if (hosted) return 0;
    return launch_kl_finalize_all(fin.l, fin.active, n, fin.rng_adv, d.advance, d.kl_total, static_cast<hipStream_t>(stream));
}

extern "C" int lbbnn_lrt_gemm_members(const float* x, int ldx, int64_t x_mstride, const void* e_w, int64_t w_mstride,
                                      const void* var_w, int ld, const float* bias_mean, const float* bias_var,
                                      const uint64_t* rng, uint32_t rng_stream, int64_t row_offset, uint64_t member_advance,
                                      float* out, int ldo, int64_t o_mstride, int B, int I, int O, int flags, int members,
                                      void* stream) {
    if (members < 1 || members > 65535) return LBBNN_E_SHAPE;
    if (x_mstride < 0 || w_mstride < 0 || o_mstride < (int64_t)B * ldo) return LBBNN_E_SHAPE;
    if ((x_mstride & 3) || (w_mstride & 3) || (o_mstride & 3)) return LBBNN_E_ALIGN;
    if (flags & LBBNN_F_SPLIT16)
        if (((size_t)(B - 1) * ldx + I) * 4 >= 0x7FFFFFF0u) return LBBNN_E_SHAPE;
    GemmArgs a = gemm_args(x, ldx, e_w, var_w, ld, out, ldo, B, I, O);
    a.bias_mean = bias_mean; a.bias_var = bias_var; a.rng = rng; a.rng_stream = rng_stream; a.row_offset = row_offset;
    a.members = members; a.x_ms = x_mstride; a.w_ms = w_mstride; a.o_ms = o_mstride; a.m_adv = member_advance;
    return lrt_gemm_dispatch(a, flags, stream);
}

extern "C" int lbbnn_vd_gemm_members(const float* x, int ldx, int64_t x_mstride, const void* e_w, const void* var_w, int ld,
                                     const float* var_scale, const uint64_t* rng, uint32_t rng_stream, int64_t row_offset,
                                     uint64_t member_advance, float* out, int ldo, int64_t o_mstride,
                                     int B, int I, int O, int flags, int members, int fanout, void* stream) {
    if (members < 1 || members > 65535) return LBBNN_E_SHAPE;
    if (fanout != 0 && fanout != 1) return LBBNN_E_SHAPE;
    if (fanout && x_mstride != 0) return LBBNN_E_SHAPE;
    if (x_mstride < 0 || o_mstride < 0 || o_mstride < (int64_t)B * ldo) return LBBNN_E_SHAPE;
    if ((x_mstride & 3) || (o_mstride & 3)) return LBBNN_E_ALIGN;
    if (flags & ~(LBBNN_F_RELU | LBBNN_F_SPLIT16 | LBBNN_F_SINGLE16 | LBBNN_F_HALF16)) return LBBNN_E_FLAGS;
    if (!rng) return LBBNN_E_NOISE;
    if (flags & LBBNN_F_SPLIT16)
        if (((size_t)(B - 1) * ldx + I) * 4 >= 0x7FFFFFF0u) return LBBNN_E_SHAPE;
    GemmArgs a = gemm_args(x, ldx, e_w, var_w, ld, out, ldo, B, I, O);
    a.var_scale = var_scale; a.rng = rng; a.rng_stream = rng_stream; a.row_offset = row_offset;
    a.x_ms = x_mstride; a.o_ms = o_mstride; a.m_adv = member_advance;
    if (fanout) a.fan = members; else a.members = members;
    return lrt_gemm_dispatch(a, flags, stream);
}

extern "C" int lbbnn_gemm_members_mean(const float* x, int ldx, int64_t x_mstride, const void* w, int64_t w_mstride, int ld,
                                       const float* bias, int64_t b_mstride, float* out, int ldo, int64_t o_mstride,
                                       int B, int I, int O, int flags, int members, void* stream) {
    if (!x || !w || !out) return LBBNN_E_NULL;
    if (members < 1 || members > 65535) return LBBNN_E_SHAPE;
    if (flags & ~(LBBNN_F_RELU | LBBNN_F_SPLIT16 | LBBNN_F_LOG_SOFTMAX)) return LBBNN_E_FLAGS;
    if ((flags & LBBNN_F_LOG_SOFTMAX) && O > 16) return LBBNN_E_FLAGS;
    if (x_mstride < 0 || w_mstride < 0 || b_mstride < 0 || o_mstride < (int64_t)B * ldo) return LBBNN_E_SHAPE;
    if ((x_mstride & 3) || (w_mstride & 3) || (o_mstride & 3)) return LBBNN_E_ALIGN;
    if (flags & LBBNN_F_SPLIT16)
        if (((size_t)(B - 1) * ldx + I) * 4 >= 0x7FFFFFF0u) return LBBNN_E_SHAPE;
    GemmArgs a = gemm_args(x, ldx, w, nullptr, ld, out, ldo, B, I, O);
    a.bias_mean = bias; a.members = members; a.x_ms = x_mstride; a.w_ms = w_mstride; a.o_ms = o_mstride; a.b_ms = b_mstride;
    return lrt_gemm_dispatch(a, flags | LBBNN_F_MEAN_ONLY, stream);
}

extern "C" int lbbnn_lrt_gemm_combine(const float* x, int ldx, const void* w_op, int ld, const float* comb_x, int ld_cx,
                                      const float* comb_add, int ld_ca, float* out, int ldo, int B, int I, int O, int flags,
                                      void* stream) {
    if (!comb_x || !comb_add) return LBBNN_E_NULL;
    if (ld_cx < O || ld_ca < O) return LBBNN_E_SHAPE;
    if (flags & ~LBBNN_F_SPLIT16) return LBBNN_E_FLAGS;
    if (O <= 16) return LBBNN_E_SHAPE;
    GemmArgs a = gemm_args(x, ldx, w_op, nullptr, ld, out, ldo, B, I, O);
    a.comb_x = comb_x; a.ld_cx = ld_cx; a.comb_add = comb_add; a.ld_ca = ld_ca;
    return lrt_gemm_dispatch(a, flags | LBBNN_F_MEAN_ONLY, stream);
}

extern "C" int lbbnn_matmul_splitk(const float* x, int ldx, const void* w_op, int ld, float* out, int ldo,
                                   int B, int I, int O, int kchunk, void* stream) {
    if (kchunk <= 0 || (kchunk & 31)) return LBBNN_E_ALIGN;
    GemmArgs a = gemm_args(x, ldx, w_op, nullptr, ld, out, ldo, B, I, O);
    a.kchunk = kchunk;
    return lrt_gemm_dispatch(a, LBBNN_F_MEAN_ONLY | LBBNN_F_SPLIT16, stream);
}
```

bayesian-neural-nets_amd/csrc/output_grad.hip:

```cpp
#include "lbbnn_device.h"
#include "lbbnn_internal.h"
#include "reduce_partials.h"

namespace {

using namespace lbbnn;
constexpr int TS = 64;

__global__ __launch_bounds__(256) void output_grad_kernel(const lbbnn_outgrad_args_t a, int nbt) {
    __shared__ float tm[TS][TS + 1], tv[TS][TS + 1];
    const int b0 = blockIdx.y * TS, o0 = blockIdx.x * TS, tid = threadIdx.x;
    const bool stoch = a.std != nullptr;
    uint64_t seed = 0, offs = 0;
    if (stoch && !a.eps) { seed = a.rng[0]; offs = a.rng[1]; }
    const bool vec = ((a.O & 3) == 0) && ((a.ldg & 3) == 0) && ((a.ldo & 3) == 0) &&
                     ((reinterpret_cast<uintptr_t>(a.g_out) & 15u) == 0) && (!a.out || (reinterpret_cast<uintptr_t>(a.out) & 15u) == 0) &&
                     (!stoch || (reinterpret_cast<uintptr_t>(a.std) & 15u) == 0) && (!a.eps || (reinterpret_cast<uintptr_t>(a.eps) & 15u) == 0) &&
                     (!a.gm || (reinterpret_cast<uintptr_t>(a.gm) & 15u) == 0) && (!stoch || !a.gv || (reinterpret_cast<uintptr_t>(a.gv) & 15u) == 0);
#pragma unroll
    for (int k = 0; k < 4; ++k) {
        const int idx = tid + 256 * k, r = idx >> 4, c = (idx & 15) * 4;
        const int b = b0 + r, o = o0 + c;
        float gm[4] = {0.f, 0.f, 0.f, 0.f}, gv[4] = {0.f, 0.f, 0.f, 0.f};
        if (b < a.B && o < a.O) {
            float g[4], y[4] = {1.f, 1.f, 1.f, 1.f}, sd[4] = {1.f, 1.f, 1.f, 1.f}, e[4] = {0.f, 0.f, 0.f, 0.f};
            const size_t ig = (size_t)b * a.ldg + o, io = (size_t)b * a.ldo + o;
            if (vec) {
                const float4 t = *reinterpret_cast<const float4*>(a.g_out + ig);
                g[0] = t.x; g[1] = t.y; g[2] = t.z; g[3] = t.w;
                if (a.relu) { const float4 u = *reinterpret_cast<const float4*>(a.out + io); y[0] = u.x; y[1] = u.y; y[2] = u.z; y[3] = u.w; }
                if (stoch) { const float4 u = *reinterpret_cast<const float4*>(a.std + io); sd[0] = u.x; sd[1] = u.y; sd[2] = u.z; sd[3] = u.w; }
                if (stoch && a.eps) { const float4 u = *reinterpret_cast<const float4*>(a.eps + (size_t)b * a.O + o); e[0] = u.x; e[1] = u.y; e[2] = u.z; e[3] = u.w; }
            } else {
#pragma unroll
                for (int q = 0; q < 4; ++q) {
                    const bool in = o + q < a.O;
                    g[q] = in ? a.g_out[ig + q] : 0.f;
                    if (a.relu) y[q] = in ? a.out[io + q] : 0.f;
                    if (stoch) sd[q] = in ? a.std[io + q] : 1.f;
                    if (stoch && a.eps) e[q] = in ? a.eps[(size_t)b * a.O + o + q] : 0.f;
                }
            }
            if (stoch && !a.eps) philox_normal4(seed, offs, a.rng_stream, (uint64_t)(a.row_offset + b), (uint32_t)(o >> 2), e);
#pragma unroll
            for (int q = 0; q < 4; ++q) {
                gm[q] = (a.relu && !(y[q] > 0.f)) ? 0.f : g[q];
                if (stoch) gv[q] = gm[q] * e[q] / (2.f * sd[q]);
                if (o + q >= a.O) { gm[q] = 0.f; gv[q] = 0.f; }
                else if (stoch && a.gv_scale) gv[q] *= a.gv_scale[o + q];
            }
            const size_t id = (size_t)b * a.O + o;
            if (a.gm) {
                if (vec) {
                    *reinterpret_cast<float4*>(a.gm + id) = make_float4(gm[0], gm[1], gm[2], gm[3]);
                    if (stoch && a.gv) *reinterpret_cast<float4*>(a.gv + id) = make_float4(gv[0], gv[1], gv[2], gv[3]);
                } else {
#pragma unroll
                    for (int q = 0; q < 4; ++q) if (o + q < a.O) { a.gm[id + q] = gm[q]; if (stoch && a.gv) a.gv[id + q] = gv[q]; }
                }
            }
        }
#pragma unroll
        for (int q = 0; q < 4; ++q) { tm[r][c + q] = gm[q]; tv[r][c + q] = gv[q]; }
    }
    __syncthreads();
#pragma unroll
    for (int k = 0; k < 16; ++k) {
        const int idx = tid + 256 * k, oc = idx >> 6, br = idx & 63;
        const int o = o0 + oc, b = b0 + br;
        if (o < a.O && b < a.B) {
            a.gmT[(size_t)o * a.B + b] = tm[br][oc];
            if (stoch) a.gvT[(size_t)o * a.B + b] = tv[br][oc];
        }
    }
    if (tid < 2 * TS) {
        const int oc = tid & 63, which = tid >> 6;
        if (which == 0 || stoch) {
            float s = 0.f;
#pragma unroll 8
            for (int r = 0; r < TS; ++r) s += which ? tv[r][oc] : tm[r][oc];
            const int o = o0 + oc;
            if (o < a.O) a.work[((size_t)which * nbt + blockIdx.y) * a.O + o] = s;
        }
    }
}

__global__ __launch_bounds__(1024) void output_grad_sum_kernel(const float* __restrict__ work, int nbt, int O, float* g_sum, float* gv_sum) {
    __shared__ float part[3][16][64];
    float* const out[3] = {g_sum, gv_sum, nullptr};
    reduce_partials_body(work, O, (long long)nbt * O, nbt, O, gv_sum ? 2 : 1, out, blockIdx.x, part);
}

__global__ __launch_bounds__(1024) void bias_backward_partials_kernel(const float* __restrict__ work, int nbt, int O, int has_gv,
                                                                      const float* bias_mu, const float* bias_rho,
                                                                      const float* g_kl, lbbnn_priors_t priors,
                                                                      float* d_bias_mu, float* d_bias_rho) {
    __shared__ float part[2][16][64];
    const int lane = threadIdx.x & 63, w = threadIdx.x >> 6;
    const int i = blockIdx.x * 64 + lane;
    float s0 = 0.f, s1 = 0.f;
    if (i < O)
        for (int b = w; b < nbt; b += 16) {
            const float* p = work + (size_t)b * O + i;
            s0 += p[0];
            if (has_gv) s1 += p[(size_t)nbt * O];
        }
    part[0][w][lane] = s0; part[1][w][lane] = s1;
    __syncthreads();
    if (w < 2 && i < O) {
        float s = 0.f;
#pragma unroll
        for (int k = 0; k < 16; ++k) s += part[w][k][lane];
        const float G = g_kl ? g_kl[0] : 0.f, inv = 1.f / (priors.bias_sigma_prior * priors.bias_sigma_prior);
        if (w == 0) {
            float gm = s;
            if (g_kl) gm += G * (bias_mu[i] - priors.bias_mu_prior) * inv;
            d_bias_mu[i] = gm;
        } else {
            const float er = expf(bias_rho[i]);
            const float sb = log1pf(er), dsig = er / (1.f + er);
            float gs = has_gv ? s * 2.f * sb : 0.f;
            if (g_kl) gs += G * (sb * inv - 1.f / sb);
            d_bias_rho[i] = gs * dsig;
        }
    }
}

struct ReduceBatch { lbbnn_reduce_job_t j[LBBNN_MAX_REDUCE_JOBS]; };
__global__ __launch_bounds__(1024) void reduce_partials_batch_kernel(const ReduceBatch bt) {
    __shared__ float part[3][16][64];
    const LBBNN_CONST_AS lbbnn_reduce_job_t& j = kernarg_as<ReduceBatch>()->j[blockIdx.y];
    if ((int)blockIdx.x * 64 >= j.ncols) return;
    float* const out[3] = {j.out[0], j.out[1], j.out[2]};
    reduce_partials_body(j.work, j.block_stride, j.q_stride, j.nblk, j.ncols, j.nq, out, blockIdx.x, part);
}

__global__ __launch_bounds__(256) void dx_combine_kernel(float* __restrict__ gx, const float* __restrict__ gxv,
                                                         const float* __restrict__ x, int ldx, int B, int I) {
    const int b = blockIdx.y;
    for (int i = blockIdx.x * 256 + threadIdx.x; i < I; i += gridDim.x * 256)
        gx[(size_t)b * I + i] += 2.f * x[(size_t)b * ldx + i] * gxv[(size_t)b * I + i];
}

constexpr int HD_ROWS = 16, HD_COLS = 256, HD_MAXC = 16;

__global__ __launch_bounds__(HD_COLS) void head_dx_kernel(const float* __restrict__ gm, const float* __restrict__ gv, int ldg,
                                                          const float* __restrict__ wmT, const float* __restrict__ wvT, int ldw,
                                                          const float* __restrict__ x, int ldx, float* __restrict__ out, int ldo,
                                                          int B, int C, int I) {
    __shared__ float sgm[HD_ROWS][HD_MAXC], sgv[HD_ROWS][HD_MAXC];
    const int b0 = blockIdx.y * HD_ROWS, i = blockIdx.x * HD_COLS + threadIdx.x;
    for (int t = threadIdx.x; t < HD_ROWS * HD_MAXC; t += HD_COLS) {
        const int r = t / HD_MAXC, c = t % HD_MAXC;
        const bool in = b0 + r < B && c < C;
        sgm[r][c] = in ? gm[(size_t)(b0 + r) * ldg + c] : 0.f;
        sgv[r][c] = (in && gv) ? gv[(size_t)(b0 + r) * ldg + c] : 0.f;
    }
    float wm[HD_MAXC], wv[HD_MAXC];
#pragma unroll
    for (int c = 0; c < HD_MAXC; ++c) {
        const bool in = i < I && c < C;
        wm[c] = in ? wmT[(size_t)i * ldw + c] : 0.f;
        wv[c] = (in && wvT) ? wvT[(size_t)i * ldw + c] : 0.f;
    }
    __syncthreads();
    if (i >= I) return;
#pragma unroll 4
    for (int r = 0; r < HD_ROWS; ++r) {
        const int b = b0 + r;
        if (b >= B) break;
        float am = 0.f, av = 0.f;
#pragma unroll
        for (int c = 0; c < HD_MAXC; ++c) { am += sgm[r][c] * wm[c]; av += sgv[r][c] * wv[c]; }
        out[(size_t)b * ldo + i] = gv ? am + 2.f * x[(size_t)b * ldx + i] * av : am;
    }
}

template <int C>
__global__ __launch_bounds__(HD_COLS) void head_dx_c_kernel(const float* __restrict__ gm, const float* __restrict__ gv, int ldg,
                                                            const float* __restrict__ wmT, const float* __restrict__ wvT, int ldw,
                                                            const float* __restrict__ x, int ldx, float* __restrict__ out, int ldo,
                                                            int B, int I) {
    const int b0 = blockIdx.y * HD_ROWS, i = blockIdx.x * HD_COLS + threadIdx.x;
    if (i >= I) return;
    float wm[C], wv[C];
#pragma unroll
    for (int c = 0; c < C; ++c) { wm[c] = wmT[(size_t)i * ldw + c]; wv[c] = wvT[(size_t)i * ldw + c]; }
    const int nr = min(HD_ROWS, B - b0);
#pragma unroll 4
    for (int r = 0; r < nr; ++r) {
        const float* __restrict__ pm = gm + (size_t)(b0 + r) * ldg;
        const float* __restrict__ pv = gv + (size_t)(b0 + r) * ldg;
        const float xv = x[(size_t)(b0 + r) * ldx + i];
        float am = 0.f, av = 0.f;
#pragma unroll
        for (int c = 0; c < C; ++c) { am += pm[c] * wm[c]; av += pv[c] * wv[c]; }
        out[(size_t)(b0 + r) * ldo + i] = am + 2.f * xv * av;
    }
}

constexpr int HW_COLS = 64, HW_LANES = 8;

template <int C>
__global__ __launch_bounds__(HW_COLS * HW_LANES) void head_dw_kernel(const float* __restrict__ gm, const float* __restrict__ gv,
                                                                     int ldg, const float* __restrict__ x, int ldx,
                                                                     float* __restrict__ dWm, float* __restrict__ dWv,
                                                                     int B, int I, int rows_per_slab) {
    __shared__ float red[HW_LANES][2 * C][HW_COLS];
    const int cg = threadIdx.x & (HW_COLS - 1);
    const int rl = __builtin_amdgcn_readfirstlane(threadIdx.x / HW_COLS);
    const int i = blockIdx.x * HW_COLS + cg, s = blockIdx.y;
    const int r0 = s * rows_per_slab, r1 = min(r0 + rows_per_slab, B);
    float am[C], av[C];
#pragma unroll
    for (int c = 0; c < C; ++c) { am[c] = 0.f; av[c] = 0.f; }
    if (i < I) {
#pragma unroll 4
        for (int b = r0 + rl; b < r1; b += HW_LANES) {
            const float* __restrict__ pm = gm + (size_t)b * ldg;
            const float xv = x[(size_t)b * ldx + i], x2 = xv * xv;
#pragma unroll
            for (int c = 0; c < C; ++c) am[c] += pm[c] * xv;
            if (gv) {
                const float* __restrict__ pv = gv + (size_t)b * ldg;
#pragma unroll
                for (int c = 0; c < C; ++c) av[c] += pv[c] * x2;
            }
        }
    }
#pragma unroll
    for (int c = 0; c < C; ++c) { red[rl][c][cg] = am[c]; red[rl][C + c][cg] = av[c]; }
    __syncthreads();
    if (i < I)
        for (int q = rl; q < 2 * C; q += HW_LANES) {
            float v = red[0][q][cg];
#pragma unroll
            for (int l = 1; l < HW_LANES; ++l) v += red[l][q][cg];
            if (q < C) dWm[((size_t)s * C + q) * I + i] = v;
            else if (dWv) dWv[((size_t)s * C + (q - C)) * I + i] = v;
        }
}

}

extern "C" int lbbnn_head_dw(const float* gm, const float* gv, int ldg, const float* x, int ldx, float* dWm, float* dWv,
                             int B, int C, int I, int nslabs, void* stream) {
    if (!gm || !x || !dWm) return LBBNN_E_NULL;
    if ((gv == nullptr) != (dWv == nullptr)) return LBBNN_E_NULL;
    if (B <= 0 || C <= 0 || C > HD_MAXC || I <= 0 || ldg < C || ldx < I || nslabs <= 0 || nslabs > B) return LBBNN_E_SHAPE;
    const int rows = (B + nslabs - 1) / nslabs;
    const dim3 grid((I + HW_COLS - 1) / HW_COLS, nslabs), block(HW_COLS * HW_LANES);
    hipStream_t s = static_cast<hipStream_t>(stream);
#define LBBNN_HEAD_DW(CC) case CC: hipLaunchKernelGGL(head_dw_kernel<CC>, grid, block, 0, s, gm, gv, ldg, x, ldx, dWm, dWv, B, I, rows); break;
    switch (C) {
        LBBNN_HEAD_DW(1) LBBNN_HEAD_DW(2) LBBNN_HEAD_DW(3) LBBNN_HEAD_DW(4) LBBNN_HEAD_DW(5) LBBNN_HEAD_DW(6) LBBNN_HEAD_DW(7) LBBNN_HEAD_DW(8)
        LBBNN_HEAD_DW(9) LBBNN_HEAD_DW(10) LBBNN_HEAD_DW(11) LBBNN_HEAD_DW(12) LBBNN_HEAD_DW(13) LBBNN_HEAD_DW(14) LBBNN_HEAD_DW(15) LBBNN_HEAD_DW(16)
    }
#undef LBBNN_HEAD_DW
    return (int)hipGetLastError();
}

extern "C" int lbbnn_head_dx(const float* gm, const float* gv, int ldg, const float* wmT, const float* wvT, int ldw,
                             const float* x, int ldx, float* out, int ldo, int B, int C, int I, void* stream) {
    if (!gm || !wmT || !out) return LBBNN_E_NULL;
    if ((gv == nullptr) != (wvT == nullptr) || (gv && !x)) return LBBNN_E_NULL;
    if (B <= 0 || C <= 0 || C > HD_MAXC || I <= 0 || ldg < C || ldw < C || ldo < I || (x && ldx < I)) return LBBNN_E_SHAPE;
    const dim3 grid((I + HD_COLS - 1) / HD_COLS, (B + HD_ROWS - 1) / HD_ROWS);
    if (C == 10 && gv)
        hipLaunchKernelGGL(head_dx_c_kernel<10>, grid, dim3(HD_COLS), 0, static_cast<hipStream_t>(stream), gm, gv, ldg, wmT, wvT,
                           ldw, x, ldx, out, ldo, B, I);
    else
        hipLaunchKernelGGL(head_dx_kernel, grid, dim3(HD_COLS), 0, static_cast<hipStream_t>(stream), gm, gv, ldg, wmT, wvT, ldw,
                           x, ldx, out, ldo, B, C, I);
    return (int)hipGetLastError();
}

extern "C" int64_t lbbnn_output_grad_workspace(int B, int O) {
    if (B <= 0 || O <= 0) return 0;
    return 2LL * ((B + TS - 1) / TS) * O;
}

extern "C" int lbbnn_output_grad(const lbbnn_outgrad_args_t* p, void* stream) {
    if (!p) return LBBNN_E_NULL;
    const lbbnn_outgrad_args_t& a = *p;
    if (!a.g_out || !a.gmT || !a.work) return LBBNN_E_NULL;
    if (!a.g_sum && a.gv_sum) return LBBNN_E_NULL;
    if (a.relu && !a.out) return LBBNN_E_NULL;
    if (a.std && (!a.gvT || (a.g_sum && !a.gv_sum) || ((a.gm == nullptr) != (a.gv == nullptr)))) return LBBNN_E_NULL;
    if (a.std && !a.eps && !a.rng) return LBBNN_E_NOISE;
    if (a.B <= 0 || a.O <= 0 || a.ldg < a.O || ((a.relu || a.std) && a.ldo < a.O)) return LBBNN_E_SHAPE;
    hipStream_t s = static_cast<hipStream_t>(stream);
    const int nbt = (a.B + TS - 1) / TS;
    hipLaunchKernelGGL(output_grad_kernel, dim3((a.O + TS - 1) / TS, nbt), dim3(256), 0, s, a, nbt);
    if (a.g_sum)
        hipLaunchKernelGGL(output_grad_sum_kernel, dim3((a.O + 63) / 64), dim3(1024), 0, s, a.work, nbt, a.O, a.g_sum,
                           a.std ? a.gv_sum : nullptr);
    return (int)hipGetLastError();
}

extern "C" int lbbnn_bias_backward_partials(const float* work, int B, int O, int has_gv, const float* bias_mu,
                                            const float* bias_rho, const float* g_kl, const lbbnn_priors_t* priors,
                                            float* d_bias_mu, float* d_bias_rho, void* stream) {
    if (!work || !bias_mu || !bias_rho || !priors || !d_bias_mu || !d_bias_rho) return LBBNN_E_NULL;
    if (B <= 0 || O <= 0) return LBBNN_E_SHAPE;
    const int nbt = (B + TS - 1) / TS;
    hipLaunchKernelGGL(bias_backward_partials_kernel, dim3((O + 63) / 64), dim3(1024), 0, static_cast<hipStream_t>(stream), work,
                       nbt, O, has_gv ? 1 : 0, bias_mu, bias_rho, g_kl, *priors, d_bias_mu, d_bias_rho);
    return (int)hipGetLastError();
}

extern "C" int lbbnn_reduce_partials_batch(const lbbnn_reduce_job_t* jobs, int n, void* stream) {
    if (n == 0) return LBBNN_OK;
    if (!jobs) return LBBNN_E_NULL;
    if (n < 0 || n > LBBNN_MAX_REDUCE_JOBS) return LBBNN_E_SHAPE;
    ReduceBatch bt;
    int maxcols = 0;
    for (int k = 0; k < n; ++k) {
        const lbbnn_reduce_job_t& j = jobs[k];
        if (!j.work) return LBBNN_E_NULL;
        if (j.nblk <= 0 || j.ncols <= 0 || j.nq < 1 || j.nq > 3 || j.block_stride < j.ncols || j.q_stride < j.ncols) return LBBNN_E_SHAPE;
        bt.j[k] = j;
        maxcols = j.ncols > maxcols ? j.ncols : maxcols;
    }
    hipLaunchKernelGGL(reduce_partials_batch_kernel, dim3((maxcols + 63) / 64, n), dim3(1024), 0, static_cast<hipStream_t>(stream), bt);
    return (int)hipGetLastError();
}

extern "C" int lbbnn_dx_combine(float* gx, const float* gxv, const float* x, int ldx, int B, int I, void* stream) {
    if (!gx || !gxv || !x) return LBBNN_E_NULL;
    if (B <= 0 || I <= 0 || ldx < I) return LBBNN_E_SHAPE;
    hipLaunchKernelGGL(dx_combine_kernel, dim3((I + 1023) / 1024, B), dim3(256), 0, static_cast<hipStream_t>(stream),
                       gx, gxv, x, ldx, B, I);
    return (int)hipGetLastError();
}
```

bayesian-neural-nets_amd/layers.py:

```python
import itertools
import weakref
from typing import Dict, Optional

import torch
import torch.nn as nn
import torch.nn.functional as F

from . import _grad, _lib, ops
from ._lib import Priors
from .distributions import Bernoulli, Gaussian
from .flows import PropagateFlow

import os as _os
_DENSE_HIP_BWD = _os.environ.get("LBBNN_DENSE_TORCH_BWD", "0") != "1"
_MASKS_IN_KERNEL = _os.environ.get("LBBNN_TORCH_MASKS", "0") != "1"
_DENSE_DEFER = {"0": False, "always": "always"}.get(_os.environ.get("LBBNN_DENSE_DEFER", "1"), True)
_HEAD_FOLD = _os.environ.get("LBBNN_HEAD_FOLD", "1") != "0"
_ADV_RIDE = _os.environ.get("LBBNN_ADV_RIDE", "1") != "0"
_V1_BATCH = _os.environ.get("LBBNN_V1_BATCH", "1") != "0"
_DEFER_SUMS = _os.environ.get("LBBNN_DEFER_SUMS", "1") != "0"
_LRT_BIAS_HIP = _os.environ.get("LBBNN_LRT_BIAS_HIP", "1") != "0"
_HEAD_DW = _os.environ.get("LBBNN_HEAD_DW", "1") != "0"
_F16_FIRST_PLANES = {"f32": False, "planes": True}.get(_os.environ.get("LBBNN_F16_FIRST", ""))
_SIDE = {}


def _side_stream(dev):
    key = dev.index if dev.index is not None else torch.cuda.current_device()
    st = _SIDE.get(key)
    if st is None:
        st = _SIDE[key] = torch.cuda.Stream(device=dev)
    return st


_OVERLAP = {"on": False, "planar": [], "dense": [], "adopt": [], "sums": []}


def _drop_deferred():
    for k in ("planar", "dense", "adopt", "sums"):
        _OVERLAP[k].clear()


def join_vector_backward():
    bad = [name for (name, p, ptr) in _OVERLAP["adopt"] if p.grad is None or p.grad.data_ptr() != ptr]
    if bad:
        _drop_deferred()
        raise RuntimeError("bnn_amd: a deferred vector-backward gradient was not adopted as .grad (%s ...): the backward "
                           "pass ran under conditions vector_backward_overlap does not support; nothing was launched, "
                           "the gradients of this step are incomplete" % ", ".join(bad[:3]))
    _OVERLAP["adopt"].clear()
    if _OVERLAP["sums"]:
        ops.reduce_partials_flush(_OVERLAP["sums"])
    if _OVERLAP["planar"]:
        ops.mnf_flow_planar_backward_flush(_OVERLAP["planar"])
    if _OVERLAP["dense"]:
        ops.mnf_flow_dense_backward_flush(_OVERLAP["dense"])


class vector_backward_overlap:

    def __enter__(self):
        self._was = _OVERLAP["on"]
        _OVERLAP["on"] = True
        return self

    def __exit__(self, exc_type, exc, tb):
        _OVERLAP["on"] = self._was
        if exc_type is not None:
            _drop_deferred()
            return False
        join_vector_backward()
        return False


class _NodeToken:
    __slots__ = ("multi", "__weakref__")

    def __init__(self):
        self.multi = False


def _has_grad_hooks(p):
    return bool(getattr(p, "_backward_hooks", None)) or bool(getattr(p, "_post_accumulate_grad_hooks", None))


def _deferral_ok(layer, token):
    if not _OVERLAP["on"] or torch.is_grad_enabled() or token is None or token.multi:
        return False
    vec = layer._param_list()[3:]
    return all(p.grad is None and p.requires_grad and p.is_leaf and not _has_grad_hooks(p) for p in vec)


def _file_adoption_checks(layer, grads):
    vec = layer._param_list()[3:]
    assert len(vec) == len(grads)
    for k, (p, g) in enumerate(zip(vec, grads)):
        _OVERLAP["adopt"].append(("%s[%d]" % (type(layer).__name__, k), p, g.data_ptr()))


_layer_ids = itertools.count()
MAX_DEPTH = 16


class _BayesLinearFn(torch.autograd.Function):

    @staticmethod
    def forward(ctx, layer, x, cfg, *params):
        if layer._mnf:
            ws = layer._workspace()
            fresh = ("act_mu", "act_var") if layer._preflow is not None else ("z_fwd", "z_kl", "scal", "act_mu", "act_var")
            if layer._preprep is not None:
                fresh = ()
            for name in fresh:
                setattr(ws, name, torch.empty_like(getattr(ws, name)))
        dense = layer._mnf and layer._check_flows() == "dense" and _DENSE_HIP_BWD
        layer._keep_dense = dense
        layer._last_flow_rng = None
        try:
            out, kl, saved = layer._forward_hip(x, cfg, advance=layer._advance_rng, save_rng=True, want_std=cfg[0])
        finally:
            layer._keep_dense = False
            layer._preflow = None
            layer._preprep = None
        if dense:
            saved["dense_save"], layer._last_dense_save = layer._last_dense_save, None
            saved["rng_flow"], layer._last_flow_rng = layer._last_flow_rng, None
        if layer._mnf:
            saved["z_fwd"] = ws.z_fwd
            if cfg[1]:
                saved["act_mu"], saved["act_var"], saved["z_kl"], saved["scal"] = ws.act_mu, ws.act_var, ws.z_kl, ws.scal
        layer._v1_slot = None
        if layer._mnf and cfg[1] and _V1_BATCH and not saved.get("noise") and saved.get("rng") is not None \
                and (layer._check_flows() == "planar" or dense) and "r0_b1" in layer._vec_names:
            slot = {"in": dict(act_mu=saved["act_mu"], act_var=saved["act_var"], zb_last=saved["scal"][3:4], rng=saved["rng"],
                               r0_b1=layer.r0_b1, r0_b2=layer.r0_b2, layer_id=layer._layer_id)}
            saved["v1_slot"] = layer._v1_slot = slot
        ctx.layer, ctx.cfg, ctx.saved = layer, cfg, saved
        from . import graphs
        graphs.mark_autograd_node(ctx, layer)
        live = layer.__dict__.setdefault("_live_nodes", weakref.WeakSet())
        ctx.token = _NodeToken()
        if len(live):
            ctx.token.multi = True
            for t in live:
                t.multi = True
        live.add(ctx.token)
        std = saved.pop("std", None)
        ctx.has_std = std is not None
        ctx.save_for_backward(x, out, *([std] if std is not None else []), *params)
        if kl is None:
            kl = out.new_zeros(())
        return out, kl

    @staticmethod
    def backward(ctx, g_out, g_kl):
        layer, cfg = ctx.layer, ctx.cfg
        token = getattr(ctx, "token", None)
        can_defer = _deferral_ok(layer, token)
        if token is not None:
            layer.__dict__.get("_live_nodes", set()).discard(token)
        stochastic, want_kl, relu = cfg
        tens = list(ctx.saved_tensors)
        x, out = tens[0], tens[1]
        std = tens[2] if ctx.has_std else None
        params = tens[3 if ctx.has_std else 2:]
        mu, rho, lam = params[0], params[1], params[2]
        B = x.shape[0]
        explicit = ctx.saved.get("noise") or {}
        if ctx.saved.get("lsm"):
            from . import losses
            left = losses._HEAD_GRAD.take(out, g_out)
            g_out = left if left is not None else ops.log_softmax_backward(g_out, out)
        planar = layer._mnf and layer._check_flows() == "planar"
        dense = layer._mnf and ctx.saved.get("dense_save") is not None
        defer_sums = _OVERLAP["sums"] if (can_defer and (planar or dense) and _DEFER_SUMS) else None
        lrt_job = [] if (not layer._mnf and _LRT_BIAS_HIP and B > 0) else None
        g, g_v, gT, g_vT, g_sum, gv_sum = ops.output_grad(
            g_out, out=out if relu else None, std=std if stochastic else None, eps=explicit.get("eps_out"),
            rng=ctx.saved.get("rng"), rng_stream=ops.STREAM_EPS_OUT * 64 + layer._layer_id, row_offset=layer.row_offset,
            relu=relu, want_g=bool(ctx.needs_input_grad[1]), defer_sums=lrt_job if lrt_job is not None else defer_sums)
        rng_snap = ctx.saved.get("rng")
        in_kernel = (planar or dense) and not explicit and rng_snap is not None
        noise = {} if in_kernel else layer._noise_for_backward(ctx.saved, B, need_out=False)
        g_kl = g_kl.contiguous() if want_kl else None
        da_mu = da_var = aux = r0_c = vg = None
        if planar or dense:
            P = dict(zip(layer._vec_names, params[3:3 + len(layer._vec_names)]))
            z_k = ctx.saved["z_fwd"]
            z2 = ctx.saved["z_kl"] if want_kl else None
            if want_kl:
                r0_c = P["r0_c"]
                slot = ctx.saved.get("v1_slot")
                if slot is not None and "out" in slot and slot["out"][3].data_ptr() == g_kl.data_ptr():
                    da_mu, da_var, aux = slot.pop("out")[:3]
                else:
                    da_mu, da_var, aux = ops.mnf_aux_backward(ctx.saved["act_mu"], ctx.saved["act_var"], noise.get("eps_act"),
                                                              P["r0_b1"], P["r0_b2"], ctx.saved["scal"][3:4], g_kl,
                                                              rng=rng_snap, layer_id=layer._layer_id)
        elif not layer._mnf and _LRT_BIAS_HIP:
            z_k = z2 = None
        else:
            with torch.enable_grad():
                vs = [p.detach().requires_grad_(True) for p in params[3:]]
                am = av = None
                if layer._mnf and want_kl:
                    am = ctx.saved["act_mu"].detach().requires_grad_(True)
                    av = ctx.saved["act_var"].detach().requires_grad_(True)
                vg = layer._vector_graph(vs, cfg, noise, am, av)
            z_k = vg["z_k"].detach() if vg["z_k"] is not None else None
            z2 = vg["z2"].detach() if vg["z2"] is not None else None
            if am is not None:
                r0_c = params[3 + layer._vec_names.index("r0_c")]
                da_mu, da_var = torch.autograd.grad(vg["kl"], [am, av], g_kl, retain_graph=True)
        gx = None
        if ctx.needs_input_grad[1]:
            from . import _lib
            O, I = layer.out_features, layer.in_features
            split_m = _operand_split_ok(g, O, I, layer)
            split_v = _operand_split_ok(g_v, O, I, layer) if stochastic else split_m
            ld = ops.operand_ld(O)
            e_t = torch.empty((I, ld), dtype=torch.float32, device=x.device)
            v_t = torch.empty((I, ld), dtype=torch.float32, device=x.device) if stochastic else None
            if split_m == split_v:
                _lib.check(_lib.lib().lbbnn_weight_operands_t(
                    mu.data_ptr(), rho.data_ptr(), lam.data_ptr(), z_k.data_ptr() if z_k is not None else None,
                    e_t.data_ptr(), v_t.data_ptr() if v_t is not None else None, ld, O, I,
                    ops.F_SPLIT16 if split_m else 0, torch.cuda.current_stream(x.device).cuda_stream), "lbbnn_weight_operands_t")
                w_shape = torch.empty((O, I), device="meta")
                if O <= 16 and not split_m and x.stride(1) == 1 and g.stride(0) == (g_v.stride(0) if stochastic else g.stride(0)):
                    gx = ops.head_dx(g, g_v if stochastic else None, e_t, v_t if stochastic else None, x, C=O, I=I)
                    stochastic_done = True
                else:
                    stochastic_done = False
                    gx = _hip_matmul_nt(g, None, w_shape, op=e_t, module=layer)
                if stochastic and not stochastic_done:
                    if I > 16 and x.stride(1) == 1:
                        gx = ops.lrt_gemm_combine(g_v, v_t, K=O, N=I, comb_x=x, comb_add=gx, split=split_v)
                    else:
                        gx = ops.dx_combine(gx, _hip_matmul_nt(g_v, None, w_shape, op=v_t, module=layer), x)
            else:
                ws = layer._workspace()
                bw = ws.backward_operands()
                ops.weight_pass(mu, rho, lam, z_fwd=z_k, priors=layer.priors, e_w=bw[0],
                                var_w=bw[1] if stochastic else None)
                gx = _hip_matmul_nt(g, ops.transpose_operand, bw[0][:, :I], module=layer)
                if stochastic:
                    gx = ops.dx_combine(gx, _hip_matmul_nt(g_v, ops.transpose_operand, bw[1][:, :I], module=layer), x)
        if (_HEAD_DW and layer.out_features <= 16 and g is not None and (g_v is not None or not stochastic) and x.dim() == 2
                and x.stride(1) == 1 and x.dtype == torch.float32 and B >= 64):
            dWm, dWv = ops.head_dw(g, g_v if stochastic else None, x,
                                   nslabs=16 if (layer.out_features * layer.in_features) % 4 == 0 else 1)
            if dWm.shape[0] == 1:
                dWm, dWv = dWm[0], (dWv[0] if dWv is not None else None)
        else:
            pair = _x_operand_pair(x, gT, g_vT, layer) if stochastic else None
            dWm = _hip_matmul_nt(gT, ops.transpose_operand, x, allow_splitk=True, op=pair[0] if pair else None, module=layer)
            dWv = (_hip_matmul_nt(g_vT, ops.transpose_operand, x, square=True, allow_splitk=True, op=pair[1] if pair else None,
                                  module=layer) if stochastic else None)
        dmu, drho, dlam, dz_k, dz2, dr0c = ops.weight_pass_backward(
            mu, rho, lam, dWm, dWv, z_fwd=z_k, z_kl=z2, r0_c=r0_c, da_mu=da_mu, da_var=da_var, g_kl=g_kl,
            priors=layer.priors, defer_sums=defer_sums)
        if not layer._mnf and _LRT_BIAS_HIP:
            if lrt_job:
                d_bmu, d_brho = ops.bias_backward_partials(lrt_job[0], B, params[3], params[4], g_kl, layer.priors)
            else:
                d_bmu, d_brho = ops.bias_backward(params[3], params[4], g_sum, gv_sum if stochastic else None, g_kl, layer.priors)
            return (None, gx, None, dmu, drho, dlam, d_bmu, d_brho)
        if planar:
            zp, rp = layer._planar_params_from(params)
            e1 = None if in_kernel else noise["eps_z"].contiguous()
            e2 = noise["eps_z2"].contiguous() if (want_kl and not in_kernel) else None
            G = ops.mnf_flow_planar_backward(
                P["q0_mean"], P["q0_log_var"], zp, rp, eps_fwd=e1, eps_kl=e2,
                rng=rng_snap, layer_id=layer._layer_id, r0_b1=P["r0_b1"], r0_b2=P["r0_b2"], aux=aux,
                dz_fwd=dz_k, dz_kl=dz2, g_kl=g_kl, bias_mu=P["bias_mu"], bias_rho=P["bias_rho"], g_sum=g_sum,
                gv_sum=gv_sum, priors=layer.priors, defer=_OVERLAP["planar"] if can_defer else None)
            G["r0_c"] = dr0c if dr0c is not None else torch.zeros_like(P["q0_mean"])
            vgrads = [G[n] for n in layer._vec_names]
            for key in ("z_flow", "r_flow"):
                for g3 in G[key]:
                    vgrads += list(g3)
            if can_defer:
                _file_adoption_checks(layer, vgrads)
            return (None, gx, None, dmu, drho, dlam, *vgrads)
        if dense:
            masks = ctx.saved["masks"]
            zd, Tz, k1 = layer.z_flow.dense_descs(masks["zmask"], masks.get("zmask2"))
            rd, Tr, k2 = layer.r_flow.dense_descs(None, masks.get("rmask")) if want_kl else (None, 0, None)
            rest = list(params[len(layer._names):])
            nz = len(list(layer.z_flow.parameters()))
            e1 = None if in_kernel else noise["eps_z"].contiguous()
            e2 = noise["eps_z2"].contiguous() if (want_kl and not in_kernel) else None
            rng_f = ctx.saved.get("rng_flow") if ctx.saved.get("rng_flow") is not None else rng_snap
            G = ops.mnf_flow_dense_backward(
                P["q0_mean"], P["q0_log_var"], zd, Tz, 0 if layer.z_flow.kind == "RNVP" else 1, rest[:nz],
                rd, Tr, 0 if layer.r_flow.kind == "RNVP" else 1, rest[nz:], save=ctx.saved["dense_save"],
                eps_fwd=e1, eps_kl=e2, rng=rng_f, layer_id=layer._layer_id, r0_b1=P["r0_b1"], r0_b2=P["r0_b2"], aux=aux,
                dz_fwd=dz_k, dz_kl=dz2, g_kl=g_kl, bias_mu=P["bias_mu"], bias_rho=P["bias_rho"], g_sum=g_sum,
                gv_sum=gv_sum, priors=layer.priors, defer=_OVERLAP["dense"] if can_defer else None,
                keep=(k1, k2))
            del k1, k2
            G["r0_c"] = dr0c if dr0c is not None else torch.zeros_like(P["q0_mean"])
            if not want_kl:
                G["r_flow"] = [torch.zeros_like(p) for p in rest[nz:]]
            vgrads = [*[G[n] for n in layer._vec_names], *G["z_flow"], *G["r_flow"]]
            if can_defer:
                _file_adoption_checks(layer, vgrads)
            return (None, gx, None, dmu, drho, dlam, *vgrads)
        outs, gouts = [vg["bmean"]], [g_sum]
        if stochastic:
            outs.append(vg["bvar"]); gouts.append(gv_sum)
        if z_k is not None:
            outs.append(vg["z_k"]); gouts.append(dz_k)
        if want_kl and vg["kl"] is not None:
            outs.append(vg["kl"]); gouts.append(g_kl)
            if z2 is not None:
                outs.append(vg["z2"]); gouts.append(dz2)
        vgrads = list(torch.autograd.grad(outs, vs, gouts, allow_unused=True))
        if dr0c is not None:
            k = layer._vec_names.index("r0_c")
            vgrads[k] = dr0c if vgrads[k] is None else vgrads[k] + dr0c
        return (None, gx, None, dmu, drho, dlam, *vgrads)


def _operand_split_ok(a, K, N, module=None):
    return (ops.split_precision(module) and ops.split_eligible(K, N)
            and a.stride(0) % 4 == 0 and a.data_ptr() % 16 == 0)


def _hip_matmul_nt(a, transpose_fn, w, square=False, allow_splitk=False, op=None, module=None):
    M, K = a.shape
    N = w.shape[1]
    assert w.shape[0] == K
    split = _operand_split_ok(a, K, N, module)
    if op is None:
        op = transpose_fn(w if w.stride(1) == 1 else w.contiguous(), square=square, split=split)
    if allow_splitk and split and K >= 1024:
        tiles = ((N + 79) // 80) * ((M + 127) // 128 if M >= 96 else (M + 31) // 32)
        S = max(1, min(16, (400 + tiles - 1) // tiles, K // 256))
        if S > 1:
            kchunk = ((K + S - 1) // S + 31) // 32 * 32
            return ops.matmul_splitk(a, op, K=K, N=N, kchunk=kchunk)
    return ops.lrt_gemm(a, op, None, I=K, O=N, mean_only=True, split=split)


def _x_operand_pair(x, gT, g_vT, module=None):
    from . import _lib
    B, I = x.shape
    if not x.is_contiguous():
        return None
    split = _operand_split_ok(gT, B, I, module)
    if split != _operand_split_ok(g_vT, B, I, module):
        return None
    ld = ops.operand_ld(B)
    xt = torch.empty((I, ld), dtype=torch.float32, device=x.device)
    x2t = torch.empty((I, ld), dtype=torch.float32, device=x.device)
    _lib.check(_lib.lib().lbbnn_vd_operands(x.data_ptr(), xt.data_ptr(), x2t.data_ptr(), ld, B, I,
                                            ops.F_SPLIT16 if split else 0, torch.cuda.current_stream(x.device).cuda_stream),
               "lbbnn_vd_operands")
    return xt, x2t


class _SigmoidHeadFn(torch.autograd.Function):

    @staticmethod
    def forward(ctx, logits):
        probs = ops.binary_head(logits)
        ctx.save_for_backward(probs)
        return probs

    @staticmethod
    def backward(ctx, g):
        from . import losses
        (probs,) = ctx.saved_tensors
        left = losses._HEAD_GRAD.take(probs, g)
        losses.HANDOVER["sigmoid_backward" if left is None else "taken"] += 1
        return left if left is not None else ops.sigmoid_backward(g, probs)


HEADS = ("log_softmax", "sigmoid", "identity")


class _BayesLinearBase(nn.Module):
    _mnf = False

    def _common_init(self, in_features, out_features, mu_range, priors, lambdal_init=(0, 1)):
        self.in_features = in_features
        self.out_features = out_features
        self.priors = priors if priors is not None else Priors()
        self.weight_mu = nn.Parameter(torch.Tensor(out_features, in_features).uniform_(-mu_range, mu_range))
        self.weight_rho = nn.Parameter(torch.Tensor(out_features, in_features).uniform_(-5, -4))
        self.weight = Gaussian(self.weight_mu, self.weight_rho)
        lo, hi = (float(v) for v in lambdal_init)
        if not lo <= hi:
            raise ValueError("bnn_amd: lambdal_init must be (lo, hi) with lo <= hi, got %r" % (lambdal_init,))
        self.lambdal = nn.Parameter(torch.Tensor(out_features, in_features).uniform_(lo, hi))
        self._alpha_q_init = torch.Tensor(out_features, in_features).uniform_(0.999, 0.9999)
        self.gamma = Bernoulli(self._alpha_q_init)
        self.gamma.bind(self._alpha_now)
        self.bias_mu = nn.Parameter(torch.Tensor(out_features).uniform_(-0.2, 0.2))
        self.bias_rho = nn.Parameter(torch.Tensor(out_features).uniform_(-5, -4))
        self.bias = Gaussian(self.bias_mu, self.bias_rho)
        self.kl = 0
        self.noise: Optional[Dict[str, torch.Tensor]] = None
        self.row_offset = 0
        self._layer_id = next(_layer_ids) % 64
        self._ws = None
        self._split_now = False
        self._keep_dense = False
        self._last_dense_save = None
        self._preflow = None
        self._advance_rng = True
        self._last_flow_rng = None
        self._mask_pool = None
        self._preprep = None
        self._lsm_now = False
        self._kl_slot = None
        self._last_masks = None

    @property
    def mu_prior(self):
        return torch.full_like(self.weight_mu, self.priors.mu_prior).detach()

    @property
    def sigma_prior(self):
        return torch.full_like(self.weight_mu, self.priors.sigma_prior).detach()

    @property
    def alpha_prior(self):
        return torch.full_like(self.weight_mu, self.priors.alpha_prior).detach()

    def _workspace(self):
        dev = self.weight_mu.device
        if self._ws is None or self._ws.device != dev:
            self._ws = ops.LayerWorkspace(self.out_features, self.in_features, dev, self._mnf)
        return self._ws

    def _alpha_now(self):
        return 1 / (1 + torch.exp(-self.lambdal))

    precision = None

    def _split(self, x=None, cfg=None):
        if not ops.split_precision(self) or not ops.split_eligible(self.in_features, self.out_features):
            return 0
        if x is not None and (x.stride(0) % 4 != 0 or x.data_ptr() % 16 != 0 or x.stride(1) != 1
                              or x.shape[0] * x.stride(0) * 4 >= 0x7FFFFFF0):
            return 0
        if (ops.f16s_precision(self) and (cfg is None or cfg[0]) and ops.f16s_eligible(self.in_features, self.out_features)
                and getattr(self, "_f16s_net_ok", True)):
            return 3 if (ops.get_precision(self) == "fp16x3f" and self.in_features >= ops.F16_VAR1_MIN_I) else 2
        return 1

    def _single(self):
        return ops.get_precision(self) in ("bf16", "fp16")

    @property
    def alpha_q(self):
        return self._alpha_now()

    def _param_list(self):
        raise NotImplementedError

    def _fusable(self):
        return True

    def _fill_desc(self, d, cfg, kl_layer):
        ws = self._workspace()
        noise = self.noise or {}
        d.weight_mu, d.weight_rho, d.lambdal = self.weight_mu.data_ptr(), self.weight_rho.data_ptr(), self.lambdal.data_ptr()
        d.bias_mu, d.bias_rho = self.bias_mu.data_ptr(), self.bias_rho.data_ptr()
        d.priors = self.priors
        d.O, d.I, d.layer_id = self.out_features, self.in_features, self._layer_id
        d.stochastic, d.want_kl = int(cfg[0]), int(cfg[1])
        d.split = int(self._split_now)
# ... 820 lines not shown
```

bayesian-neural-nets_amd/ops.py:

```python
import ctypes
from typing import NamedTuple, Optional, Sequence

import torch

from . import _lib
from ._lib import Priors

F_RELU = 0x1
F_MEAN_ONLY = 0x2
F_SPLIT16 = 0x4
F_LOG_SOFTMAX = 0x8
F_SINGLE16 = 0x10
F_HALF16 = 0x20
F_F16S = 0x40
F_VAR1 = 0x80
F_XPLANES = 0x100

STREAM_EPS_OUT = 0
STREAM_EPS_Z = 1
STREAM_EPS_Z2 = 2
STREAM_EPS_ACT = 3
STREAM_EPS_W = 4
STREAM_EPS_B = 5
STREAM_MASK = 6
STREAM_ROW_MASK = 7
STREAM_GATE = 8
STREAM_GAMMA_W = 9
STREAM_GAMMA_B = 10
GATES_SAMPLE = 0
GATES_MPM = 1
GATE_MEMBERS_MAX_LD = 4096


PRECISIONS = ("fp32", "bf16x3", "bf16", "fp16", "fp16x3", "fp16x3f")
_PRECISION = "fp32"


def set_precision(name: str):
    global _PRECISION
    if name not in PRECISIONS:
        raise ValueError("precision must be one of %s" % (PRECISIONS,))
    _PRECISION = name


def get_precision(module=None) -> str:
    own = getattr(module, "precision", None) if module is not None else None
    if own is not None:
        if own not in PRECISIONS:
            raise ValueError("precision must be one of %s" % (PRECISIONS,))
        return own
    return _PRECISION


def split_precision(module=None) -> bool:
    return get_precision(module) != "fp32"


def f16s_precision(module=None) -> bool:
    return get_precision(module) in ("fp16x3", "fp16x3f")


def split_eligible(I: int, O: int) -> bool:
    return O > 16 and I % 8 == 0 and (I % 32 == 0 or operand_ld(I) - I >= 8) and O * operand_ld(I) * 4 < 0x7FFFFFF0


F16_VAR1_MIN_I = 256


def f16s_eligible(I: int, O: int) -> bool:
    return split_eligible(I, O) and operand_ld(I) <= 1280


def _stream() -> int:
    return torch.cuda.current_stream().cuda_stream


def _ptr(t: Optional[torch.Tensor], name: str = "tensor") -> Optional[int]:
    if t is None:
        return None
    if not t.is_cuda:
        raise RuntimeError("bnn_amd: %s is on %s; the HIP path needs a GPU tensor (no CPU fallback)" % (name, t.device))
    if t.dtype != torch.float32 and t.dtype != torch.int64:
        raise RuntimeError("bnn_amd: %s has dtype %s, expected float32" % (name, t.dtype))
    if not t.is_contiguous():
        raise RuntimeError("bnn_amd: %s must be contiguous" % name)
    return t.data_ptr()


def _ptr_rows(t: torch.Tensor, name: str) -> int:
    if not t.is_cuda:
        raise RuntimeError("bnn_amd: %s is on %s; the HIP path needs a GPU tensor (no CPU fallback)" % (name, t.device))
    if t.dtype != torch.float32 or t.dim() != 2 or t.stride(1) != 1:
        raise RuntimeError("bnn_amd: %s must be a 2-D float32 tensor with dense rows" % name)
    return t.data_ptr()


def operand_ld(I: int) -> int:
    return ((I + 31) // 32) * 32


class RngState:
    _states = {}
    _requested = None

    def __init__(self, device: torch.device):
        self.device = device
        self.seed = None
        self.t = torch.zeros(4, dtype=torch.int64, device=device)
        req = RngState._requested
        self.reseed(torch.initial_seed(), req[1] if (req is not None and req[0] == torch.initial_seed()) else 0)

    def reseed(self, seed: int, offset: int = 0):
        self.seed = int(seed)
        s = self.seed & 0xFFFFFFFFFFFFFFFF
        if s >= 1 << 63:
            s -= 1 << 64
        self.t[:2].copy_(torch.tensor([s, int(offset)], dtype=torch.int64))

    @classmethod
    def get(cls, device: torch.device) -> "RngState":
        key = (device.type, device.index if device.index is not None else torch.cuda.current_device())
        st = cls._states.get(key)
        if st is None:
            st = cls(device)
            cls._states[key] = st
        elif st.seed != torch.initial_seed() and not torch.cuda.is_current_stream_capturing():
            st.reseed(torch.initial_seed())
        return st

    def advance(self, delta: int = 1):
        _lib.check(_lib.lib().lbbnn_rng_advance(self.t.data_ptr(), delta, _stream()), "lbbnn_rng_advance")


def manual_seed(seed: int, offset: int = 0):
    torch.manual_seed(seed)
    RngState._requested = (int(seed), int(offset))
    for st in RngState._states.values():
        st.reseed(seed, offset)


def philox_normal(rng: torch.Tensor, stream_id: int, rows: int, cols: int, row_base: int = 0) -> torch.Tensor:
    out = torch.empty((rows, cols) if rows > 0 else (cols,), dtype=torch.float32, device=rng.device)
    _lib.check(_lib.lib().lbbnn_philox_normal(rng.data_ptr(), stream_id, row_base, rows, cols, out.data_ptr(),
                                              _stream()), "lbbnn_philox_normal")
    return out


def philox_uniform(rng: torch.Tensor, stream_id: int, rows: int, cols: int, row_base: int = 0) -> torch.Tensor:
    out = torch.empty((rows, cols), dtype=torch.float32, device=rng.device)
    _lib.check(_lib.lib().lbbnn_philox_uniform(rng.data_ptr(), stream_id, row_base, rows, cols, out.data_ptr(), _stream()),
               "lbbnn_philox_uniform")
    return out


def philox_std_gamma(rng: torch.Tensor, stream_id: int, a: torch.Tensor, rate: Optional[torch.Tensor] = None) -> torch.Tensor:
    a = a.detach().float().contiguous()
    rate = None if rate is None else rate.detach().float().contiguous()
    out = torch.empty_like(a)
    _lib.check(_lib.lib().lbbnn_philox_std_gamma(rng.data_ptr(), stream_id, a.data_ptr(), _ptr(rate, "rate"), a.numel(),
                                                 out.data_ptr(), _stream()), "lbbnn_philox_std_gamma")
    return out


def gamma_grad(x: torch.Tensor, a: torch.Tensor) -> torch.Tensor:
    x = x.detach().float().contiguous()
    a = a.detach().float().contiguous()
    if x.shape != a.shape:
        raise ValueError("bnn_amd.ops.gamma_grad: x and a must have the same shape")
    out = torch.empty_like(x)
    _lib.check(_lib.lib().lbbnn_gamma_grad(x.data_ptr(), a.data_ptr(), x.numel(), out.data_ptr(), _stream()), "lbbnn_gamma_grad")
    return out


def weight_pass(mu, rho, lambdal, *, z_fwd=None, z_kl=None, r0_c=None, bias_rho=None,
                priors: Priors, e_w=None, var_w=None, kl_rows=None, act_mu=None, act_var=None,
                bias_var=None, split=False, e_scale=None, v_scale=None):
    O, I = mu.shape
    ld = operand_ld(I)
    if int(split) >= 2:
        rc = _lib.lib().lbbnn_weight_pass_f16(
            _ptr(mu, "weight_mu"), _ptr(rho, "weight_rho"), _ptr(lambdal, "lambdal"),
            _ptr(z_fwd), _ptr(z_kl), _ptr(r0_c), _ptr(bias_rho), ctypes.byref(priors),
            _ptr(e_w), _ptr(var_w), ld, _ptr(e_scale, "e_scale"), _ptr(v_scale, "v_scale"),
            _ptr(kl_rows), _ptr(act_mu), _ptr(act_var), _ptr(bias_var), O, I, F_VAR1 if int(split) == 3 else 0, _stream())
        _lib.check(rc, "lbbnn_weight_pass_f16")
        return
    rc = _lib.lib().lbbnn_weight_pass(
        _ptr(mu, "weight_mu"), _ptr(rho, "weight_rho"), _ptr(lambdal, "lambdal"),
        _ptr(z_fwd), _ptr(z_kl), _ptr(r0_c), _ptr(bias_rho), ctypes.byref(priors),
        _ptr(e_w), _ptr(var_w), ld, _ptr(kl_rows), _ptr(act_mu), _ptr(act_var), _ptr(bias_var),
        O, I, F_SPLIT16 if split else 0, _stream())
    _lib.check(rc, "lbbnn_weight_pass")


def output_grad(g_out, *, out=None, std=None, eps=None, rng=None, rng_stream: int = 0, row_offset: int = 0,
                relu: bool = False, gv_scale=None, want_g: bool = True, defer_sums=None):
    B, O = g_out.shape
    f = dict(dtype=torch.float32, device=g_out.device)
    if g_out.stride(1) != 1:
        g_out = g_out.contiguous()
    stoch = std is not None
    gm, gmT, g_sum = (torch.empty((B, O), **f) if want_g else None), torch.empty((O, B), **f), torch.empty(O, **f)
    gv = gvT = gv_sum = None
    if stoch:
        gv, gvT, gv_sum = (torch.empty((B, O), **f) if want_g else None), torch.empty((O, B), **f), torch.empty(O, **f)
    if B == 0:
        g_sum.zero_()
        if stoch:
            gv_sum.zero_()
        return gm, gv, gmT, gvT, g_sum, gv_sum
    a = _lib.OutGradArgs()
    a.g_out = _ptr_rows(g_out, "g_out")
    a.out = _ptr_rows(out, "out") if (relu and out is not None) else None
    a.std = _ptr_rows(std, "std") if stoch else None
    ldo = out.stride(0) if (relu and out is not None) else (std.stride(0) if stoch else O)
    if relu and stoch and out.stride(0) != std.stride(0):
        raise ValueError("bnn_amd: out and std must share a row stride")
    a.eps = _ptr(eps, "eps") if (stoch and eps is not None) else None
    a.rng = rng.data_ptr() if rng is not None else None
    work = torch.empty(_lib.lib().lbbnn_output_grad_workspace(B, O), **f)
    a.gm, a.gmT, a.work = (gm.data_ptr() if gm is not None else None), gmT.data_ptr(), work.data_ptr()
    a.g_sum = g_sum.data_ptr() if defer_sums is None else None
    if stoch:
        a.gv, a.gvT = (gv.data_ptr() if gv is not None else None), gvT.data_ptr()
        a.gv_sum = gv_sum.data_ptr() if defer_sums is None else None
    if defer_sums is not None:
        nbt = (B + 63) // 64
        defer_sums.append(dict(work=work, outs=(g_sum, gv_sum, None), block_stride=O, q_stride=nbt * O, nblk=nbt, ncols=O,
                               nq=2 if stoch else 1))
    a.row_offset, a.rng_stream = row_offset, rng_stream
    a.gv_scale = _ptr(gv_scale, "gv_scale") if (stoch and gv_scale is not None) else None
    a.B, a.O, a.ldg, a.ldo, a.relu = B, O, g_out.stride(0), ldo, 1 if relu else 0
    _lib.check(_lib.lib().lbbnn_output_grad(ctypes.byref(a), _stream()), "lbbnn_output_grad")
    return gm, gv, gmT, gvT, g_sum, gv_sum


def head_dx(gm, gv, wmT, wvT, x, *, C: int, I: int):
    B = gm.shape[0]
    gm_ptr, gv_ptr = _ptr_rows(gm, "gm"), (_ptr_rows(gv, "gv") if gv is not None else None)
    if gv is not None and gv.stride(0) != gm.stride(0):
        raise ValueError("bnn_amd: gm and gv must share a row stride (got %d and %d)" % (gm.stride(0), gv.stride(0)))
    out = torch.empty((B, I), dtype=torch.float32, device=gm.device)
    rc = _lib.lib().lbbnn_head_dx(gm_ptr, gv_ptr, gm.stride(0),
                                  _ptr(wmT), _ptr(wvT), wmT.stride(0), _ptr_rows(x, "x") if gv is not None else None,
                                  x.stride(0) if gv is not None else 0, out.data_ptr(), I, B, C, I, _stream())
    _lib.check(rc, "lbbnn_head_dx")
    return out



def head_dw(gm, gv, x, *, nslabs: int = 16):
    B, C = gm.shape
    I = x.shape[1]
    S = max(1, min(int(nslabs), B))
    dWm = torch.empty((S, C, I), dtype=torch.float32, device=gm.device)
    dWv = torch.empty((S, C, I), dtype=torch.float32, device=gm.device) if gv is not None else None
    rc = _lib.lib().lbbnn_head_dw(_ptr_rows(gm, "gm"), _ptr_rows(gv, "gv") if gv is not None else None, gm.stride(0),
                                  _ptr_rows(x, "x"), x.stride(0), dWm.data_ptr(), dWv.data_ptr() if dWv is not None else None,
                                  B, C, I, S, _stream())
    _lib.check(rc, "lbbnn_head_dw")
    return dWm, dWv


def matmul_splitk(a, w_op, *, K: int, N: int, kchunk: int):
    M = a.shape[0]
    S = (K + kchunk - 1) // kchunk
    out = torch.empty((S, M, N), dtype=torch.float32, device=a.device)
    rc = _lib.lib().lbbnn_matmul_splitk(_ptr_rows(a, "a"), a.stride(0), _ptr(w_op), operand_ld(K), out.data_ptr(), N,
                                        M, K, N, kchunk, _stream())
    _lib.check(rc, "lbbnn_matmul_splitk")
    return out


def dx_combine(gx, gxv, x):
    B, I = gx.shape
    rc = _lib.lib().lbbnn_dx_combine(_ptr(gx, "gx"), _ptr(gxv, "gxv"), _ptr_rows(x, "x"), x.stride(0), B, I, _stream())
    _lib.check(rc, "lbbnn_dx_combine")
    return gx


def weight_pass_backward(mu, rho, lambdal, dWm, dWv=None, *, z_fwd=None, z_kl=None, r0_c=None, da_mu=None,
                         da_var=None, g_kl=None, priors: Priors, work: Optional[torch.Tensor] = None, defer_sums=None):
    O, I = mu.shape
    a = _lib.WpbArgs()
    a.mu, a.rho, a.lambdal = _ptr(mu, "weight_mu"), _ptr(rho, "weight_rho"), _ptr(lambdal, "lambdal")
    nsplit = dWm.shape[0] if dWm.dim() == 3 else 1
    for t, name in ((dWm, "dWm"), (dWv, "dWv")):
        if t is not None and (tuple(t.shape[-2:]) != tuple(mu.shape) or not t.is_contiguous()
                              or (t.shape[0] if t.dim() == 3 else 1) != nsplit):
            raise ValueError("bnn_amd: %s must be a contiguous (O,I) or (S,O,I) tensor" % name)
    a.dWm, a.dWv = _ptr(dWm, "dWm"), _ptr(dWv)
    a.z_fwd, a.z_kl, a.r0_c = _ptr(z_fwd), _ptr(z_kl), _ptr(r0_c)
    a.da_mu, a.da_var, a.g_kl = _ptr(da_mu), _ptr(da_var), _ptr(g_kl)
    a.priors = priors
    f = dict(dtype=torch.float32, device=mu.device)
    dmu, drho, dlam = torch.empty_like(mu), torch.empty_like(mu), torch.empty_like(mu)
    dz_fwd = torch.empty(I, **f) if z_fwd is not None else None
    dz_kl = torch.empty(I, **f) if (z_kl is not None and (g_kl is not None or da_mu is not None)) else None
    dr0_c = torch.empty(I, **f) if (r0_c is not None and da_mu is not None) else None
    need = _lib.lib().lbbnn_weight_pass_backward_workspace(O, I)
    if work is None or work.numel() < need:
        work = torch.empty(need, **f)
    a.dmu, a.drho, a.dlambdal = dmu.data_ptr(), drho.data_ptr(), dlam.data_ptr()
    deferred = defer_sums is not None and (dz_fwd is not None or dz_kl is not None or dr0_c is not None)
    a.work = work.data_ptr()
    a.dz_fwd, a.dz_kl, a.dr0_c = (None, None, None) if deferred else (_ptr(dz_fwd), _ptr(dz_kl), _ptr(dr0_c))
    a.O, a.I = O, I
    a.nsplit, a.split_stride = nsplit, O * I
    _lib.check(_lib.lib().lbbnn_weight_pass_backward(ctypes.byref(a), _stream()), "lbbnn_weight_pass_backward")
    if deferred:
        ld = (I + 3) & ~3
        defer_sums.append(dict(work=work, outs=(dz_fwd, dz_kl, None), ptrs=(_ptr(dz_fwd), _ptr(dz_kl), _ptr(dr0_c)),
                               block_stride=3 * ld, q_stride=ld, nblk=(O + 7) // 8, ncols=I, nq=3))
    return dmu, drho, dlam, dz_fwd, dz_kl, dr0_c


def reduce_partials_flush(pending):
    i = 0
    while i < len(pending):
        grp = pending[i:i + 8]
        arr = (_lib.ReduceJob * len(grp))()
        for k, j in enumerate(grp):
            arr[k].work = j["work"].data_ptr()
            for q in range(3):
                arr[k].out[q] = j["ptrs"][q] if "ptrs" in j else (j["outs"][q].data_ptr() if j["outs"][q] is not None else None)
            arr[k].block_stride, arr[k].q_stride = j["block_stride"], j["q_stride"]
            arr[k].nblk, arr[k].ncols, arr[k].nq = j["nblk"], j["ncols"], j["nq"]
        _lib.check(_lib.lib().lbbnn_reduce_partials_batch(arr, len(grp), _stream()), "lbbnn_reduce_partials_batch")
        i += 8
    pending.clear()


class GemmEventLog(list):

    def __init__(self, launches: int, group: int = 1, every: int = 1):
        super().__init__()
        self._pool = [(torch.cuda.Event(enable_timing=True), torch.cuda.Event(enable_timing=True)) for _ in range(launches)]
        for s, e in self._pool:
            s.record()
            e.record()
        torch.cuda.synchronize()
        self._group, self._every, self._n = group, every, 0

    def take(self):
        k = self._n
        self._n += 1
        if (k // self._group) % self._every:
            return None
        return self._pool.pop() if self._pool else None


GEMM_EVENTS = None


class Finalize(NamedTuple):
    layers: object
    n: int
    fin_rng: Optional[int]
    kl_total: Optional[int]
    rng_live: Optional[int] = None
    advance: int = 0


def _gemm_input(x, cols: int, what: str, O: int, eps, finalize):
    if x.dim() != 2 or x.shape[1] != cols:
        raise RuntimeError("bnn_amd: %s must be (B,%d), got %s" % (what, cols, tuple(x.shape)))
    B = x.shape[0]
    if eps is not None and tuple(eps.shape) != (B, O):
        raise RuntimeError("bnn_amd: eps must be (%d,%d), got %s" % (B, O, tuple(eps.shape)))
    if B == 0 and finalize is None:
        return None
    if x.stride(1) != 1 or x.stride(0) < cols:
        x = x.contiguous()
    return x


def _gemm_desc(x, e_w, var_w, *, I, O, bias_mean, bias_var, var_scale, eps, rng, rng_stream, row_offset, out, std_out, flags,
               finalize):
    d = _lib.GemmDesc()
    d.x, d.ldx = _ptr_rows(x, "input"), x.stride(0)
    d.e_w, d.var_w, d.ld = _ptr(e_w), _ptr(var_w), operand_ld(I)
    d.bias_mean, d.bias_var, d.var_scale, d.eps = _ptr(bias_mean), _ptr(bias_var), _ptr(var_scale), _ptr(eps, "eps")
    d.rng = rng.data_ptr() if rng is not None else None
    d.rng_stream, d.row_offset = rng_stream, row_offset
    d.out, d.ldo = (out.data_ptr(), out.stride(0)) if out is not None else (None, 0)
    d.std_out = _ptr(std_out, "std_out")
    d.B, d.I, d.O, d.flags = x.shape[0], I, O, flags
    if finalize is not None:
        d.layers, d.n_layers, d.fin_rng, d.kl_total, d.rng_live, d.advance = finalize if len(finalize) == 6 else Finalize(*finalize)
    return d


def _gemm_call(name: str, args, B: int, I: int, O: int):
    ev = GEMM_EVENTS.take() if GEMM_EVENTS is not None else None
    if ev is not None:
        ev[0].record()
    _lib.check(getattr(_lib.lib(), name)(*args, _stream()), name)
    if ev is not None:
        ev[1].record()
        GEMM_EVENTS.append((B, I, O, ev[0], ev[1]))


def lrt_gemm(x, e_w, var_w, *, I: int, O: int, bias_mean=None, bias_var=None, var_scale=None,
             eps=None, rng: Optional[torch.Tensor] = None, rng_stream: int = 0, row_offset: int = 0,
             relu: bool = False, mean_only: bool = False, log_softmax: bool = False,
             split: bool = False, out: Optional[torch.Tensor] = None, std_out: Optional[torch.Tensor] = None,
             finalize=None, half: bool = False, single: Optional[bool] = None):
    dev = x.device
    x = _gemm_input(x, I, "input", O, eps, finalize)
    B = 0 if x is None else x.shape[0]
    if out is None:
        out = torch.empty((B, O), dtype=torch.float32, device=dev)
    if x is None:
        return out
    flags = ((F_RELU if relu else 0) | (F_MEAN_ONLY if mean_only else 0) | (F_LOG_SOFTMAX if log_softmax else 0)
             | (F_SPLIT16 if split else 0)
             | (F_SINGLE16 if (split and not mean_only and (single if single is not None else _PRECISION in ("bf16", "fp16"))) else 0)
             | (F_HALF16 if (half and split and not mean_only) else 0))
    if std_out is None and finalize is None:
        _gemm_call("lbbnn_lrt_gemm", (
            _ptr_rows(x, "input"), x.stride(0), _ptr(e_w), _ptr(var_w), operand_ld(I),
            _ptr(bias_mean), _ptr(bias_var), _ptr(var_scale), _ptr(eps, "eps"),
            rng.data_ptr() if rng is not None else None, rng_stream, row_offset,
            out.data_ptr(), out.stride(0), B, I, O, flags), B, I, O)
# ... 761 lines not shown
```

include/lbbnn.h:

```cpp
#ifndef LBBNN_H_
#define LBBNN_H_

#include <stdint.h>

#ifdef __cplusplus
extern "C" {
#endif

#define LBBNN_ABI_VERSION 1

#define LBBNN_OK 0
#define LBBNN_E_NULL (-1)
#define LBBNN_E_SHAPE (-2)
#define LBBNN_E_ALIGN (-3)
#define LBBNN_E_FLAGS (-4)
#define LBBNN_E_NOISE (-5)

#define LBBNN_MAX_FLOW_T 16
#define LBBNN_MAX_FLOW_DIM 16384

#define LBBNN_F_RELU 0x1
#define LBBNN_F_MEAN_ONLY 0x2
#define LBBNN_F_SPLIT16 0x4
#define LBBNN_F_LOG_SOFTMAX 0x8
#define LBBNN_F_HALF16 0x20
#define LBBNN_F_SINGLE16 0x10

#define LBBNN_STREAM_EPS_OUT 0
#define LBBNN_STREAM_EPS_Z 1
#define LBBNN_STREAM_EPS_Z2 2
#define LBBNN_STREAM_EPS_ACT 3
#define LBBNN_STREAM_MASK 6
#define LBBNN_STREAM_ROW_MASK 7

typedef struct lbbnn_priors {
    float mu_prior;
    float sigma_prior;
    float alpha_prior;
    float bias_mu_prior;
    float bias_sigma_prior;
} lbbnn_priors_t;

int lbbnn_abi_version(void);
const char* lbbnn_error_string(int code);

int lbbnn_operand_ld(int I);

int lbbnn_weight_pass(const float* mu, const float* rho, const float* lambdal,
                      const float* z_fwd, const float* z_kl, const float* r0_c,
                      const float* bias_rho, const lbbnn_priors_t* priors,
                      void* e_w, void* var_w, int ld,
                      float* kl_rows, float* act_mu, float* act_var, float* bias_var,
                      int O, int I, int flags, void* stream);

int lbbnn_lrt_gemm(const float* x, int ldx, const void* e_w, const void* var_w, int ld,
                   const float* bias_mean, const float* bias_var, const float* var_scale,
                   const float* eps, const uint64_t* rng, uint32_t rng_stream, int64_t row_offset,
                   float* out, int ldo, int B, int I, int O, int flags, void* stream);

#define LBBNN_GEMM_NONE (-1)
#define LBBNN_GEMM_SKINNY 0
#define LBBNN_GEMM_STAGED 1
#define LBBNN_GEMM_DMA 2
#define LBBNN_GEMM_SPLIT 3
typedef struct lbbnn_gemm_plan {
    int family, large_tile, xvec, mean_only, products, half, fan, kernel_id;
} lbbnn_gemm_plan_t;
int lbbnn_lrt_gemm_plan(int B, int I, int O, int ldx, int x_aligned, int flags, int members, int fan, int kchunk,
                        lbbnn_gemm_plan_t* plan);

int lbbnn_mnf_flow_planar(const float* q0_mean, const float* q0_log_var,
                          const float* const* zu, const float* const* zw, const float* const* zb, int Tz,
                          const float* const* ru, const float* const* rw, const float* const* rb, int Tr,
                          const float* eps_fwd, const float* eps_kl,
                          const uint64_t* rng, uint32_t layer_id,
                          float* z_fwd, float* z_kl, float* scal,
                          int I, int want_kl, void* stream);


#define LBBNN_FLOW_RNVP 0
#define LBBNN_FLOW_MNF 1
#define LBBNN_MAX_HIDDEN 128

typedef struct lbbnn_dense_transform {
    int kind;
    int hidden;
    const float *w_in, *b_in;
    const float *w_mid[3], *b_mid[3];
    const float *w_a, *b_a;
    const float *w_b, *b_b;
    const float *mask_fwd, *mask_kl;
} lbbnn_dense_transform_t;

int64_t lbbnn_flow_dense_workspace(int I);

int lbbnn_mnf_flow_dense(const float* q0_mean, const float* q0_log_var,
                         const lbbnn_dense_transform_t* zt, int Tz,
                         const lbbnn_dense_transform_t* rt, int Tr,
                         const float* eps_fwd, const float* eps_kl,
                         const uint64_t* rng, uint32_t layer_id,
                         float* z_fwd, float* z_kl, float* scal, float* work,
                         int I, int want_kl, void* stream);

typedef struct lbbnn_dense_layer {
    const float *q0_mean, *q0_log_var;
    const lbbnn_dense_transform_t *zt, *rt;
    const float *eps_fwd, *eps_kl;
    float *z_fwd, *z_kl, *scal, *work;
    int Tz, Tr, I, want_kl;
    uint32_t layer_id;
    float *save;
    int draw_masks;
} lbbnn_dense_layer_t;

int64_t lbbnn_flow_dense_save_size(int I, int Tz, int Tr);
int lbbnn_layers_dense_flows(const lbbnn_dense_layer_t* layers, int n, const uint64_t* rng, void* stream);
int lbbnn_layers_dense_flows_phase(const lbbnn_dense_layer_t* layers, int n, const uint64_t* rng, int phase, void* stream);

int lbbnn_kl_finalize(const float* kl_rows, const float* bias_mu, const float* bias_rho, int O,
                      const float* act_mu, const float* act_var, const float* eps_act,
                      const float* r0_b1, const float* r0_b2, int I,
                      const float* scal, const lbbnn_priors_t* priors,
                      const uint64_t* rng, uint32_t layer_id,
                      float* kl_out, float* kl_layer, int kl_accum, void* stream);

#define LBBNN_K3_GENERIC 0
#define LBBNN_K3_LDS 1
#define LBBNN_K3_FAST 2
#define LBBNN_K3_VEC 3
#define LBBNN_K5_GENERIC 0
#define LBBNN_K5_LDS 1
#define LBBNN_K5_UNSTAGED 0
#define LBBNN_K5_STAGED 1
int lbbnn_flow_planar_form(int n, const int* I, const int* Tz, const int* Tr, const int* want_kl, const int* aligned16,
                           int members);
int lbbnn_kl_finalize_form(int n, const int* O, const int* I, const int* mnf, const int* active, int all_layers);


#define LBBNN_MAX_LAYERS 4

typedef struct lbbnn_planar_flow {
    const float* u[LBBNN_MAX_FLOW_T];
    const float* w[LBBNN_MAX_FLOW_T];
    const float* b[LBBNN_MAX_FLOW_T];
    int T;
} lbbnn_planar_flow_t;

typedef struct lbbnn_layer_desc {
    const float *weight_mu, *weight_rho, *lambdal, *bias_mu, *bias_rho;
    const float *q0_mean, *q0_log_var, *r0_c, *r0_b1, *r0_b2;
    lbbnn_planar_flow_t z_flow, r_flow;
    lbbnn_priors_t priors;
    int O, I;
    uint32_t layer_id;
    int stochastic;
    int want_kl;
    int split;
    const float *eps_z, *eps_z2, *eps_act;
    float *z_fwd, *z_kl, *scal;
    void *e_w, *var_w;
    float *kl_rows, *act_mu, *act_var, *bias_var;
    float* kl_layer;
    int flows_done;
    float *e_scale, *v_scale;
} lbbnn_layer_desc_t;

int lbbnn_layers_prepare(const lbbnn_layer_desc_t* layers, int n, const uint64_t* rng, void* stream);
int lbbnn_layers_operands(const lbbnn_layer_desc_t* layers, int n, const uint64_t* rng, void* stream);
int lbbnn_layers_finalize(const lbbnn_layer_desc_t* layers, int n, uint64_t* rng, uint64_t advance, float* kl_total,
                          void* stream);

int lbbnn_layers_operands_snap(const lbbnn_layer_desc_t* layers, int n, uint64_t* rng, uint64_t* rng_snap,
                               uint64_t advance, void* stream);

int lbbnn_ensemble_operands(const lbbnn_layer_desc_t* layers, int n, int members, const uint64_t* rng,
                            uint64_t member_advance, void* stream);
int lbbnn_lrt_gemm_members(const float* x, int ldx, int64_t x_mstride, const void* e_w, int64_t w_mstride,
                           const void* var_w, int ld, const float* bias_mean, const float* bias_var,
                           const uint64_t* rng, uint32_t rng_stream, int64_t row_offset, uint64_t member_advance,
// ... 179 lines not shown
    float *mean, *var;
    float* bias_var;
    int32_t* kept_rows;
    int O, I;
    int nnz;
    int levels;
    float cut[LBBNN_MAX_LEVELS];
} lbbnn_sparse_levels_desc_t;

int lbbnn_sparse_count_levels(const lbbnn_sparse_levels_desc_t* layers, int n, void* stream);
int lbbnn_sparse_pack_levels(const lbbnn_sparse_levels_desc_t* layers, int n, void* stream);
int lbbnn_sparse_layer_levels(const int32_t* row_ptr, const int32_t* col, const float* mean, const float* var, int nnz,
                              const float* bias_mu, const float* bias_var, const float* a, int lda, int64_t a_mstride,
                              const float* z, int64_t z_mstride, const uint64_t* rng, uint32_t rng_stream,
                              int64_t row_offset, uint64_t member_advance, float* out, int ldo, int64_t o_mstride,
                              int out_rows, int B, int I, int O, int flags, int levels, int members_per_level, void* stream);

typedef struct lbbnn_base_frozen_desc {
    const float *mu, *rho, *lambdal;
    const float *bias_mu, *bias_rho;
    float *w_mu, *w_sigma;
    float* alpha;
    void* e_w;
    float *b_mu, *b_sigma;
    int32_t* kept_rows;
    float* alpha_rows;
    uint8_t* keep;
    int O, I, ld;
    int flags;
    int exact;
    uint32_t layer_id;
} lbbnn_base_frozen_desc_t;

int lbbnn_base_frozen_operands(const lbbnn_base_frozen_desc_t* layers, const lbbnn_compact_map_t* maps, int n, int mode,
                               float threshold, void* stream);
int lbbnn_base_frozen_members(const lbbnn_base_frozen_desc_t* layers, const lbbnn_compact_map_t* maps, int n, int members,
                              int mode, float temperature, void* w_out[], float* bias_out[], float* gate_rows[],
                              const uint64_t* rng, uint64_t member_advance, void* stream);

int lbbnn_vd_operands(const float* theta, void* e_w, void* var_w, int ld, int I, int O, int flags, void* stream);

int lbbnn_weight_operands_t(const float* weight_mu, const float* weight_rho, const float* lambdal, const float* z,
                            void* e_t, void* v_t, int ld, int O, int I, int flags, void* stream);



int lbbnn_format_operand(const float* src, int R, int C, int lds_src, void* dst, int ld, int square, int flags, void* stream);
int lbbnn_transpose_operand(const float* src, int R, int C, int lds_src, void* dst, int ld,
                            int square, int flags, void* stream);

typedef struct lbbnn_wpb_args {
    const float *mu, *rho, *lambdal, *dWm, *dWv;
    const float *z_fwd, *z_kl, *r0_c;
    const float *da_mu, *da_var;
    const float *g_kl;
    lbbnn_priors_t priors;
    float *dmu, *drho, *dlambdal;
    float *dz_fwd, *dz_kl, *dr0_c;
    float *work;
    int O, I;
    int nsplit;
    int64_t split_stride;
} lbbnn_wpb_args_t;

int64_t lbbnn_weight_pass_backward_workspace(int O, int I);
int lbbnn_weight_pass_backward(const lbbnn_wpb_args_t* args, void* stream);


int lbbnn_rng_advance(uint64_t* rng, uint64_t delta, void* stream);

int lbbnn_philox_normal(const uint64_t* rng, uint32_t rng_stream, int64_t row_base, int64_t rows,
                        int64_t cols, float* out, void* stream);

int lbbnn_log_softmax_rows(const float* in, int ldi, float* out, int ldo, int B, int O, void* stream);

typedef struct lbbnn_planar_grad {
    float* u[LBBNN_MAX_FLOW_T];
    float* w[LBBNN_MAX_FLOW_T];
    float* b[LBBNN_MAX_FLOW_T];
} lbbnn_planar_grad_t;

typedef struct lbbnn_flow_bwd_args {
    const float *q0_mean, *q0_log_var, *eps_fwd, *eps_kl;
    const float *r0_b1, *r0_b2;
    const float *aux;
    const float *dz_fwd, *dz_kl;
    const float *g_kl;
    const float *bias_mu, *bias_rho, *g_sum, *gv_sum;
    lbbnn_planar_flow_t z_flow, r_flow;
    lbbnn_priors_t priors;
    float *d_q0_mean, *d_q0_log_var, *d_r0_b1, *d_r0_b2;
    float *d_bias_mu, *d_bias_rho;
    lbbnn_planar_grad_t d_z_flow, d_r_flow;
    float *work;
    int O, I;
    const uint64_t* rng;
    uint32_t layer_id;
} lbbnn_flow_bwd_args_t;

int lbbnn_mnf_aux_backward(const float* act_mu, const float* act_var, const float* eps_act, const float* r0_b1,
                           const float* r0_b2, const float* zb_last, const float* g_kl, int O, int I,
                           float* da_mu, float* da_var, float* aux, const uint64_t* rng, uint32_t layer_id, void* stream);
typedef struct {
    const float *act_mu, *act_var, *eps_act, *r0_b1, *r0_b2, *zb_last, *g_kl;
    float *da_mu, *da_var, *aux;
    const uint64_t* rng;
    int O, I;
    uint32_t layer_id;
} lbbnn_aux_bwd_args_t;
int lbbnn_mnf_aux_backward_batch(const lbbnn_aux_bwd_args_t* args, int n, void* stream);

int lbbnn_bias_backward(const float* bias_mu, const float* bias_rho, const float* g_sum, const float* gv_sum,
                        const float* g_kl, const lbbnn_priors_t* priors, float* d_bias_mu, float* d_bias_rho, int O,
                        void* stream);
int lbbnn_bias_backward_partials(const float* work, int B, int O, int has_gv, const float* bias_mu, const float* bias_rho,
                                 const float* g_kl, const lbbnn_priors_t* priors, float* d_bias_mu, float* d_bias_rho,
                                 void* stream);
int64_t lbbnn_mnf_flow_backward_workspace(int I, int Tz, int Tr);
int lbbnn_mnf_flow_planar_backward(const lbbnn_flow_bwd_args_t* args, void* stream);
int lbbnn_mnf_flow_planar_backward_batch(const lbbnn_flow_bwd_args_t* args, int n, void* stream);

#define LBBNN_FLOW_PLANAR 0
#define LBBNN_FLOW_RADIAL 1
#define LBBNN_FLOW_HOUSEHOLDER 2
#define LBBNN_FLOW_SYLVESTER 3
#define LBBNN_MAX_SYLVESTER_M 8

typedef struct lbbnn_flow_step {
    const float *p0, *p1, *p2;
    int type, M;
} lbbnn_flow_step_t;

typedef struct lbbnn_flow_chain {
    lbbnn_flow_step_t step[LBBNN_MAX_FLOW_T];
    int n;
} lbbnn_flow_chain_t;

int lbbnn_flow_chain(const lbbnn_flow_chain_t* chain, const float* z_in, const float* q0_mean,
                     const float* q0_log_var, const float* eps, const uint64_t* rng, uint32_t rng_stream, int I,
                     float* z_out, float* logdet, float* log_q0, float* z_last, void* stream);
int lbbnn_flow_chain_rows(const lbbnn_flow_chain_t* chain, const float* z_in, int ldz, int R, int I,
                          float* z_out, int ldo, float* logdet_rows, void* stream);


typedef struct lbbnn_outgrad_args {
    const float *g_out, *out, *std, *eps;
    const uint64_t* rng;
    float *gm, *gv, *gmT, *gvT;
    float *g_sum, *gv_sum, *work;
    int64_t row_offset;
    uint32_t rng_stream;
    int B, O, ldg, ldo, relu;
    const float* gv_scale;
} lbbnn_outgrad_args_t;

int64_t lbbnn_output_grad_workspace(int B, int O);
int lbbnn_output_grad(const lbbnn_outgrad_args_t* args, void* stream);
#define LBBNN_MAX_REDUCE_JOBS 8
typedef struct {
    const float* work;
    float* out[3];
    int64_t block_stride, q_stride;
    int nblk, ncols, nq;
} lbbnn_reduce_job_t;
int lbbnn_reduce_partials_batch(const lbbnn_reduce_job_t* jobs, int n, void* stream);
int lbbnn_head_dx(const float* gm, const float* gv, int ldg, const float* wmT, const float* wvT, int ldw,
                  const float* x, int ldx, float* out, int ldo, int B, int C, int I, void* stream);
int lbbnn_head_dw(const float* gm, const float* gv, int ldg, const float* x, int ldx, float* dWm, float* dWv,
                  int B, int C, int I, int nslabs, void* stream);
int lbbnn_lrt_gemm_combine(const float* x, int ldx, const void* w_op, int ld, const float* comb_x, int ld_cx,
                           const float* comb_add, int ld_ca, float* out, int ldo, int B, int I, int O, int flags,
                           void* stream);
int lbbnn_dx_combine(float* gx, const float* gxv, const float* x, int ldx, int B, int I, void* stream);

#define LBBNN_ADAM_MAX_TENSORS 80
typedef struct lbbnn_adam_list {
    float* p[LBBNN_ADAM_MAX_TENSORS];
    const float* g[LBBNN_ADAM_MAX_TENSORS];
    float* m[LBBNN_ADAM_MAX_TENSORS];
    float* v[LBBNN_ADAM_MAX_TENSORS];
    int64_t numel[LBBNN_ADAM_MAX_TENSORS];
    int n;
} lbbnn_adam_list_t;

int lbbnn_adam_step(const lbbnn_adam_list_t* list, float lr, float beta1, float beta2, float eps, float weight_decay,
                    float* step, int advance, void* stream);

#define LBBNN_ADAM_GROUPS_MAX_TENSORS 64
#define LBBNN_ADAM_CHUNK 4096
#define LBBNN_ADAM_F_DECOUPLED 0x1
#define LBBNN_ADAM_F_INACTIVE 0x2
typedef struct lbbnn_adam_hyper {
    float lr, beta1, beta2, eps, weight_decay;
    uint32_t flags;
} lbbnn_adam_hyper_t;
typedef struct lbbnn_adam_group_list {
    float* p[LBBNN_ADAM_GROUPS_MAX_TENSORS];
    const float* g[LBBNN_ADAM_GROUPS_MAX_TENSORS];
    float* m[LBBNN_ADAM_GROUPS_MAX_TENSORS];
    float* v[LBBNN_ADAM_GROUPS_MAX_TENSORS];
    const float* mask[LBBNN_ADAM_GROUPS_MAX_TENSORS];
    int64_t numel[LBBNN_ADAM_GROUPS_MAX_TENSORS];
    int group[LBBNN_ADAM_GROUPS_MAX_TENSORS];
    int n;
} lbbnn_adam_group_list_t;

int lbbnn_adam_step_groups(const lbbnn_adam_group_list_t* list, const lbbnn_adam_hyper_t* hyper, float* step, int n_groups,
                           const float* grad_scale, uint32_t* ticket, int advance, void* stream);

#define LBBNN_SGD_F_NESTEROV 0x1
#define LBBNN_SGD_F_INACTIVE 0x2
typedef struct lbbnn_sgd_hyper {
    float lr, momentum, dampening, weight_decay;
    uint32_t flags;
} lbbnn_sgd_hyper_t;

int lbbnn_sgd_step_groups(const lbbnn_adam_group_list_t* list, const lbbnn_sgd_hyper_t* hyper, float* step, int n_groups,
                          const float* grad_scale, uint32_t* ticket, int advance, void* stream);

int lbbnn_adam_step_groups_guarded(const lbbnn_adam_group_list_t* list, const lbbnn_adam_hyper_t* hyper, float* step, int n_groups,
                                   const float* grad_scale, uint32_t* ticket, int advance, const int32_t* guard, int64_t* skipped,
                                   void* stream);
int lbbnn_sgd_step_groups_guarded(const lbbnn_adam_group_list_t* list, const lbbnn_sgd_hyper_t* hyper, float* step, int n_groups,
                                  const float* grad_scale, uint32_t* ticket, int advance, const int32_t* guard, int64_t* skipped,
                                  void* stream);

int64_t lbbnn_grad_sumsq_workspace(int64_t partials);
int lbbnn_grad_sumsq(const lbbnn_adam_group_list_t* list, float* work, int64_t work_offset, int64_t finalize_count,
                     float max_norm, float* norm, float* grad_scale, void* stream);

int lbbnn_matmul_splitk(const float* x, int ldx, const void* w_op, int ld, float* out, int ldo,
                        int B, int I, int O, int kchunk, void* stream);

typedef struct lbbnn_copy_list {
    float* dst[LBBNN_ADAM_MAX_TENSORS];
    const float* src[LBBNN_ADAM_MAX_TENSORS];
    int64_t numel[LBBNN_ADAM_MAX_TENSORS];
    int n;
} lbbnn_copy_list_t;

int lbbnn_multi_copy(const lbbnn_copy_list_t* list, void* stream);

#define LBBNN_MAX_DENSE_T 8
typedef struct lbbnn_dense_grad {
    float *w_in, *b_in, *w_mid[3], *b_mid[3], *w_a, *b_a, *w_b, *b_b;
} lbbnn_dense_grad_t;

int64_t lbbnn_flow_dense_apply_workspace(int I, int T);
int lbbnn_flow_dense_apply(const lbbnn_dense_transform_t* tr, int T, int which_mask, const float* z_in, int I,
                           float* z_out, float* logdet, void* stream);
int lbbnn_flow_dense_apply_backward(const lbbnn_dense_transform_t* tr, const lbbnn_dense_grad_t* grads, int T,
                                    int which_mask, const float* z_in, const float* d_zout, const float* d_logdet, int I,
                                    float* dz_in, float* work, void* stream);

int lbbnn_q0_rows(const float* q0_mean, const float* q0_log_var, const float* eps, const uint64_t* rng,
                  uint32_t rng_stream, int R, int I, float* z0, void* stream);
int lbbnn_flow_dense_rows_max_dim(void);
int lbbnn_flow_dense_rows(const lbbnn_dense_transform_t* tr, int T, const float* masks, float* mask_out,
                          const uint64_t* rng, uint32_t rng_stream, uint64_t row_base,
                          const float* z_in, int ldz, int R, int I,
                          float* z_out, int ldo, float* logdet_rows, void* stream);

typedef struct lbbnn_dense_bwd_args {
    const float *q0_mean, *q0_log_var, *eps_fwd, *eps_kl;
    const float *r0_b1, *r0_b2;
    const float *aux;
    const float *dz_fwd, *dz_kl;
    const float *g_kl;
    const float *bias_mu, *bias_rho, *g_sum, *gv_sum;
    const lbbnn_dense_transform_t *zt, *rt;
    const lbbnn_dense_grad_t *d_zt, *d_rt;
    lbbnn_priors_t priors;
    float *d_q0_mean, *d_q0_log_var, *d_r0_b1, *d_r0_b2;
    float *d_bias_mu, *d_bias_rho;
    const float *save;
    float *work;
    int Tz, Tr, O, I;
    const uint64_t* rng;
    uint32_t layer_id;
} lbbnn_dense_bwd_args_t;

int64_t lbbnn_mnf_flow_dense_backward_workspace(int I);
int lbbnn_mnf_flow_dense_backward(const lbbnn_dense_bwd_args_t* args, void* stream);
int lbbnn_mnf_flow_dense_backward_batch(const lbbnn_dense_bwd_args_t* args, int n, void* stream);

#define LBBNN_F_F16S 0x40
#define LBBNN_F_VAR1 0x80
#define LBBNN_F_XPLANES 0x100

typedef struct lbbnn_gemm_desc {
    const void* x; int ldx;
    const void* e_w; const void* var_w; int ld;
    const float* mean_scale;
    const float* wvar_scale;
    const float* bias_mean;
    const float* bias_var;
    const float* var_scale;
    const float* eps;
    const uint64_t* rng; uint32_t rng_stream; int64_t row_offset;
    float* out; int ldo;
    void* out_planes; int ldp;
    float* std_out;
    int B, I, O, flags;
    const lbbnn_layer_desc_t* layers; int n_layers; const uint64_t* fin_rng; float* kl_total;
    uint64_t* rng_live; uint64_t advance;
    const float* head_e; const float* head_v; int head_ld; int head_classes;
    const float* head_bias_mean; const float* head_bias_var; const float* head_eps; uint32_t head_rng_stream;
    float* head_out; int head_ldo; float* head_slab; int head_flags;
} lbbnn_gemm_desc_t;

int lbbnn_lrt_gemm_ex(const lbbnn_gemm_desc_t* d, void* stream);
int64_t lbbnn_head_slab_floats(int B, int O);

int lbbnn_format_x(const float* x, int ldx, void* planes, int ldp, int B, int I, void* stream);

int lbbnn_elbo_loss(const float* logp, int ldp, const int64_t* target, int B, int C, const float* kl, float kl_scale,
                    float* loss, void* stream);
int lbbnn_elbo_loss_backward(const float* g, const int64_t* target, int B, int C, float kl_scale, float* g_logp, float* g_kl,
                             void* stream);
#define LBBNN_MONITOR_COUNTS 8
#define LBBNN_MONITOR_STEPS 0
#define LBBNN_MONITOR_ROWS 1
#define LBBNN_MONITOR_CORRECT 2
#define LBBNN_MONITOR_BAD_TARGETS 3
#define LBBNN_MONITOR_NONFINITE_ROWS 4
#define LBBNN_MONITOR_NONFINITE_STEPS 5
#define LBBNN_MONITOR_SKIPPED_STEPS 6
#define LBBNN_MONITOR_NLL_ROWS 7
#define LBBNN_MONITOR_SUMS 5
#define LBBNN_MONITOR_NLL_SUM 0
#define LBBNN_MONITOR_KL_TERM_SUM 1
#define LBBNN_MONITOR_LOSS_SUM 2
#define LBBNN_MONITOR_LAST_NLL 3
#define LBBNN_MONITOR_LAST_LOSS 4
#define LBBNN_MONITOR_WORDS (LBBNN_MONITOR_COUNTS + LBBNN_MONITOR_SUMS)
int lbbnn_elbo_loss_monitor(const float* logp, int ldp, const int64_t* target, int B, int C, const float* kl, float kl_scale,
                            float* loss, int64_t* totals, int32_t* guard, void* stream);
int lbbnn_elbo_loss_backward_logits(const float* g, const int64_t* target, const float* logp, int ldp, int B, int C,
                                    float kl_scale, float* g_logp, float* g_logits, float* g_kl, void* stream);
int lbbnn_log_softmax_backward(const float* g, int ldg, const float* logp, int ldp, float* out, int ldo, int B, int C,
                               void* stream);

int lbbnn_binary_head(const float* logits, int ldi, int B, int O, float* probs, int ldp, float* logp2, int ld2, void* stream);
int lbbnn_elbo_bce_loss(const float* probs, int ldp, const float* target, int ldt, int B, int O, const float* kl, float kl_scale,
                        float* loss, int* stats, int accumulate, void* stream);
int lbbnn_elbo_bce_loss_backward(const float* g, const float* probs, int ldp, const float* target, int ldt, int B, int O,
                                 float kl_scale, float* g_probs, float* g_logits, float* g_kl, void* stream);
int lbbnn_sigmoid_backward(const float* g, int ldg, const float* probs, int ldp, float* out, int ldo, int B, int O, void* stream);
int lbbnn_elbo_bce_loss_monitor(const float* probs, int ldp, const float* target, int ldt, int B, int O, const float* kl,
                                float kl_scale, float* loss, int* stats, int accumulate, int64_t* totals, int32_t* guard,
                                void* stream);

int lbbnn_layers_operands_x(const lbbnn_layer_desc_t* layers, int n, uint64_t* rng, uint64_t* rng_snap, uint64_t advance,
                            const float* x, int ldx, void* planes, int ldp, int B, int I, void* stream);

int lbbnn_weight_pass_f16(const float* mu, const float* rho, const float* lambdal,
                          const float* z_fwd, const float* z_kl, const float* r0_c,
                          const float* bias_rho, const lbbnn_priors_t* priors,
                          void* e_w, void* var_w, int ld, float* e_scale, float* v_scale,
                          float* kl_rows, float* act_mu, float* act_var, float* bias_var,
                          int O, int I, int flags , void* stream);

#define LBBNN_EVAL_COUNTS 6
typedef struct lbbnn_eval_metrics_args {
    const float* logp;
    int64_t m_stride, ldp;
    const float* mean_logp;
    int64_t ldm;
    const int64_t* target;
    float* ens_logp;
    int64_t* pred_ensemble;
    int64_t* pred_mean;
    float* entropy;
    int64_t* counts;
    int64_t* correct_member;
    int64_t* confusion;
    double* sums;
    void* work;
    int S, B, C;
} lbbnn_eval_metrics_args_t;

int64_t lbbnn_eval_metrics_work_bytes(int S, int B, int C);
int lbbnn_eval_metrics(const lbbnn_eval_metrics_args_t* args, void* stream);

#define LBBNN_UNC_COUNTS 6
// ... 279 lines not shown
```

Baseline: 35.20 million.

## Fuse mean and variance weight-gradient GEMMs into one dual split-K kernel

Adds a RAW variant of the bf16x3 split-K GEMM that computes the mean and variance weight gradients in one pass. It shares the transposed-x operand loads across both products and stores raw per-split partials for dWm and dWv. The output-gradient kernel can now write its transposed gradients straight into padded, operand-aligned rows (t_ld), so the backward pass skips separate reformatting. This only touches the backward weight-gradient path, which may not be on the timed forward path, and it adds a new flag, kernel instantiation and layout constraints.

```diff
diff --git a/bayesian-neural-nets_amd/_lib.py b/bayesian-neural-nets_amd/_lib.py
--- a/bayesian-neural-nets_amd/_lib.py
+++ b/bayesian-neural-nets_amd/_lib.py
@@ -257,7 +257,7 @@
 class OutGradArgs(ctypes.Structure):
     _fields_ = [(n, c_p) for n in ("g_out", "out", "std", "eps", "rng", "gm", "gv", "gmT", "gvT", "g_sum", "gv_sum", "work")] + \
                [("row_offset", c_i64), ("rng_stream", c_u32)] + [(n, c_i) for n in ("B", "O", "ldg", "ldo", "relu")] + \
-               [("gv_scale", c_p)]
+               [("gv_scale", c_p), ("t_ld", c_i)]
 
 
 class FlowStep(ctypes.Structure):
@@ -423,6 +423,7 @@
     "lbbnn_grad_sumsq_workspace": (c_i64, [c_i64]),
     "lbbnn_grad_sumsq": (c_i, [ctypes.POINTER(AdamGroupList), c_p, c_i64, c_i64, ctypes.c_float, c_p, c_p, c_p]),
     "lbbnn_matmul_splitk": (c_i, [c_p, c_i, c_p, c_i, c_p, c_i, c_i, c_i, c_i, c_i, c_p]),
+    "lbbnn_matmul_dual_splitk": (c_i, [c_p, c_i, c_p, c_p, c_i, c_p, c_p, c_i, c_i, c_i, c_i, c_i, c_p]),
     "lbbnn_lrt_gemm_combine": (c_i, [c_p, c_i, c_p, c_i, c_p, c_i, c_p, c_i, c_p, c_i, c_i, c_i, c_i, c_i, c_p]),
     "lbbnn_dx_combine": (c_i, [c_p, c_p, c_p, c_i, c_i, c_i, c_p]),
     "lbbnn_output_grad_workspace": (c_i64, [c_i, c_i]),
diff --git a/bayesian-neural-nets_amd/csrc/lrt_gemm.hip b/bayesian-neural-nets_amd/csrc/lrt_gemm.hip
--- a/bayesian-neural-nets_amd/csrc/lrt_gemm.hip
+++ b/bayesian-neural-nets_amd/csrc/lrt_gemm.hip
@@ -33,6 +33,7 @@
     long long x_ms, w_ms, o_ms, b_ms;
     unsigned long long m_adv, m_off;
     int fan;
+    float* out_v;
 };
 
 __device__ __forceinline__ GemmArgs member_view(const GemmArgs& in) {
@@ -193,6 +194,27 @@
             epilogue4<MEAN_ONLY>(a, ec, oc[i], b, o, accm[i][j], accv[i][j], pa[i][j], pa[i][j], pb[i][j], res, sd);
             store4_rows(a.out + (size_t)b * a.ldo + o, ec.ovec, o, a.O, res);
             if (!MEAN_ONLY && a.std_out) store4_rows(a.std_out + (size_t)b * a.O + o, ec.ovec, o, a.O, sd);
+        }
+    }
+}
+
+template <int TO, int TB>
+__device__ __forceinline__ void raw_store_tile(const GemmArgs& a, int o0, int lr, int brow0,
+                                               const floatx4 (&accm)[TO][TB], const floatx4 (&accv)[TO][TB]) {
+    const bool vec = ((a.B & 3) == 0) && ((a.ldo & 3) == 0) &&
+                     (((reinterpret_cast<uintptr_t>(a.out) | reinterpret_cast<uintptr_t>(a.out_v)) & 15u) == 0);
+#pragma unroll
+    for (int i = 0; i < TO; ++i) {
+        const int o = o0 + i * 16 + lr;
+        if (o >= a.O) continue;
+#pragma unroll
+        for (int j = 0; j < TB; ++j) {
+            const int b = brow0 + j * 16;
+            if (b >= a.B) continue;
+            const float vm[4] = {accm[i][j][0], accm[i][j][1], accm[i][j][2], accm[i][j][3]};
+            const float vv[4] = {accv[i][j][0], accv[i][j][1], accv[i][j][2], accv[i][j][3]};
+            store4_rows(a.out + (size_t)o * a.ldo + b, vec, b, a.B, vm);
+            store4_rows(a.out_v + (size_t)o * a.ldo + b, vec, b, a.B, vv);
         }
     }
 }
@@ -464,9 +486,10 @@
 
 typedef _Float16 f16x8 __attribute__((ext_vector_type(8)));
 typedef _Float16 f16x2 __attribute__((ext_vector_type(2)));
-template <int TO, int TB, int WB, bool MEAN_ONLY, int NP, bool F16, bool FAN>
+template <int TO, int TB, int WB, bool MEAN_ONLY, int NP, bool F16, bool FAN, bool RAW>
 __device__ __forceinline__ void lrt_gemm_bf16x3_body(const GemmArgs& a_in) {
     static_assert(!F16 || NP == 1, "fp16 operands exist in the single-product form only");
+    static_assert(!RAW || (!MEAN_ONLY && NP == 3 && !F16 && !FAN), "the raw form is the dual-moment bf16x3 loop");
     const GemmArgs a = member_view(a_in);
     constexpr int BN = TO * 16, BM = TB * WB * 16;
     constexpr int NWR = MEAN_ONLY ? 1 : 2;
@@ -625,6 +648,16 @@
                 }
                 const bf16x8 ah = __builtin_bit_cast(bf16x8, wh[i]);
                 const bf16x8 al = NP == 3 ? __builtin_bit_cast(bf16x8, wl[i]) : ah;
+                if (RAW) {
+                    const bf16x8 bh = __builtin_bit_cast(bf16x8, wvh[i]);
+                    accm[i][j] = __builtin_amdgcn_mfma_f32_16x16x32_bf16(xh[j], ah, accm[i][j], 0, 0, 0);
+                    accm[i][j] = __builtin_amdgcn_mfma_f32_16x16x32_bf16(xh[j], al, accm[i][j], 0, 0, 0);
+                    accm[i][j] = __builtin_amdgcn_mfma_f32_16x16x32_bf16(xl[j], ah, accm[i][j], 0, 0, 0);
+                    accv[i][j] = __builtin_amdgcn_mfma_f32_16x16x32_bf16(sh[j], bh, accv[i][j], 0, 0, 0);
+                    accv[i][j] = __builtin_amdgcn_mfma_f32_16x16x32_bf16(sh[j], __builtin_bit_cast(bf16x8, wvl[i]), accv[i][j], 0, 0, 0);
+                    accv[i][j] = __builtin_amdgcn_mfma_f32_16x16x32_bf16(sl[j], bh, accv[i][j], 0, 0, 0);
+                    continue;
+                }
                 accm[i][j] = __builtin_amdgcn_mfma_f32_16x16x32_bf16(ah, xh[j], accm[i][j], 0, 0, 0);
                 if (NP == 3) {
                     accm[i][j] = __builtin_amdgcn_mfma_f32_16x16x32_bf16(al, xh[j], accm[i][j], 0, 0, 0);
@@ -656,11 +689,16 @@
 
     GemmArgs ao = a;
     if (a.kchunk) ao.out = a.out + (size_t)blockIdx.z * a.split_stride;
+    if (RAW) {
+        if (a.kchunk) ao.out_v = a.out_v + (size_t)blockIdx.z * a.split_stride;
+        raw_store_tile<TO, TB>(ao, o0, lr, b0 + wv * TB * 16 + 4 * q, accm, accv);
+        return;
+    }
     epilogue_tile<TO, TB, MEAN_ONLY, FAN>(ao, o0, q, b0 + wv * TB * 16 + lr, accm, accv);
 }
-template <int TO, int TB, int WB, bool MEAN_ONLY, int NP = 3, bool F16 = false, bool FAN = false>
+template <int TO, int TB, int WB, bool MEAN_ONLY, int NP = 3, bool F16 = false, bool FAN = false, bool RAW = false>
 __global__ __launch_bounds__(WB * 64, (TB * TO > 10) ? 1 : (WB == 8 ? 4 : 2)) void lrt_gemm_bf16x3_kernel(const GemmArgs a_in) {
-    lrt_gemm_bf16x3_body<TO, TB, WB, MEAN_ONLY, NP, F16, FAN>(a_in);
+    lrt_gemm_bf16x3_body<TO, TB, WB, MEAN_ONLY, NP, F16, FAN, RAW>(a_in);
 }
 
 
@@ -785,8 +823,10 @@
 int plan_check(const PlanIn& p) {
     if (p.B <= 0 || p.I <= 0 || p.O <= 0 || p.ldx < p.I) return LBBNN_E_SHAPE;
     const int flags = p.flags;
-    if (flags & ~(LBBNN_F_RELU | LBBNN_F_MEAN_ONLY | LBBNN_F_SPLIT16 | LBBNN_F_LOG_SOFTMAX | LBBNN_F_SINGLE16 | LBBNN_F_HALF16))
+    if (flags & ~(LBBNN_F_RELU | LBBNN_F_MEAN_ONLY | LBBNN_F_SPLIT16 | LBBNN_F_LOG_SOFTMAX | LBBNN_F_SINGLE16 | LBBNN_F_HALF16 |
+                  LBBNN_F_DUAL_RAW))
         return LBBNN_E_FLAGS;
+    if ((flags & LBBNN_F_DUAL_RAW) && flags != (LBBNN_F_DUAL_RAW | LBBNN_F_SPLIT16)) return LBBNN_E_FLAGS;
     if ((flags & LBBNN_F_HALF16) && (!(flags & LBBNN_F_SINGLE16) || (flags & LBBNN_F_MEAN_ONLY))) return LBBNN_E_FLAGS;
     if ((flags & LBBNN_F_LOG_SOFTMAX) && (p.O > 16 || (flags & LBBNN_F_RELU))) return LBBNN_E_FLAGS;
     if ((flags & LBBNN_F_SINGLE16) && !(flags & LBBNN_F_SPLIT16)) return LBBNN_E_FLAGS;
@@ -794,14 +834,15 @@
 }
 
 constexpr int kPlanLarge = 1 << 2, kPlanXvec = 1 << 3, kPlanMean = 1 << 4, kPlanFan = 1 << 5, kPlanSingle = 1 << 6,
-              kPlanHalf = 1 << 7;
+              kPlanHalf = 1 << 7, kPlanRaw = 1 << 8;
 
 int plan_select(const PlanIn& p, lbbnn_gemm_plan_t& out) {
     const int B = p.B, I = p.I, O = p.O;
     const bool split = (p.flags & LBBNN_F_SPLIT16) != 0;
     const bool mean_only = (p.flags & LBBNN_F_MEAN_ONLY) != 0;
-    const bool solo = p.solo || p.kchunk;
-    if (p.kchunk && !(split && mean_only)) return LBBNN_E_FLAGS;
+    const bool raw = (p.flags & LBBNN_F_DUAL_RAW) != 0;
+    const bool solo = p.solo || p.kchunk || raw;
+    if (p.kchunk && !(split && (mean_only || raw))) return LBBNN_E_FLAGS;
     if (p.members > 1 && solo) return LBBNN_E_FLAGS;
     if (p.fan && (p.members != 1 || mean_only || solo || (p.flags & LBBNN_F_LOG_SOFTMAX))) return LBBNN_E_FLAGS;
 
@@ -829,7 +870,7 @@
     }
     pl.kernel_id = pl.family | (pl.large_tile ? kPlanLarge : 0) | (pl.xvec ? kPlanXvec : 0) | (pl.mean_only ? kPlanMean : 0) |
                    (pl.fan ? kPlanFan : 0) | ((pl.family == LBBNN_GEMM_SPLIT && pl.products == 1) ? kPlanSingle : 0) |
-                   (pl.half ? kPlanHalf : 0);
+                   (pl.half ? kPlanHalf : 0) | (raw ? kPlanRaw : 0);
     out = pl;
     return 0;
 }
@@ -884,6 +925,7 @@
         if (piggy_lds_bytes(a.fin) <= (p.mean_only ? l_mean : l_full)) { grid.y += 1; *hosted = true; }
         else a.fin.n = 0;
     }
+    if (p.kernel_id & kPlanRaw) return launch_one(lrt_gemm_bf16x3_kernel<TO, TB, WB, false, 3, false, false, true>, grid, block, l_full, s, a);
     if (p.fan) {
         if (p.half) return launch_one(lrt_gemm_bf16x3_kernel<TO, TB, WB, false, 1, true, true>, grid, block, l_full, s, a);
         if (p.products == 1) return launch_one(lrt_gemm_bf16x3_kernel<TO, TB, WB, false, 1, false, true>, grid, block, l_full, s, a);
@@ -935,19 +977,21 @@
     const int B = a.B, I = a.I, O = a.O, ld = a.ld;
     if (B == 0 && I > 0 && O > 0) return 0;
     if (!a.x || !a.e_w || !a.out) return LBBNN_E_NULL;
-    if (a.ldo < O) return LBBNN_E_SHAPE;
+    if (a.ldo < (a.out_v ? B : O)) return LBBNN_E_SHAPE;
     PlanIn pin{B, I, O, a.ldx, (reinterpret_cast<uintptr_t>(a.x) & 15u) == 0, flags, a.members, a.fan, a.kchunk, ld,
                a.fin.n > 0 || a.eps || a.std_out || a.comb_x};
     if (const int rc = plan_check(pin)) return rc;
     const bool mean_only = (flags & LBBNN_F_MEAN_ONLY) != 0;
+    const bool raw = (flags & LBBNN_F_DUAL_RAW) != 0;
+    if (raw != (a.out_v != nullptr)) return LBBNN_E_FLAGS;
     if (!mean_only && !a.var_w) return LBBNN_E_NULL;
-    if (!mean_only && !a.eps && !a.rng) return LBBNN_E_NOISE;
+    if (!mean_only && !raw && !a.eps && !a.rng) return LBBNN_E_NOISE;
     if (ld < I || (ld & 31)) return LBBNN_E_ALIGN;
     if ((reinterpret_cast<uintptr_t>(a.e_w) & 15u) || (reinterpret_cast<uintptr_t>(a.var_w) & 15u)) return LBBNN_E_ALIGN;
 
     a.relu = (flags & LBBNN_F_RELU) ? 1 : 0; a.log_softmax = (flags & LBBNN_F_LOG_SOFTMAX) ? 1 : 0;
     a.single16 = (flags & LBBNN_F_HALF16) ? 2 : ((flags & LBBNN_F_SINGLE16) ? 1 : 0);
-    a.split_stride = (long long)B * a.ldo; a.m_off = 0;
+    a.split_stride = (long long)(raw ? O : B) * a.ldo; a.m_off = 0;
     lbbnn_gemm_plan_t plan;
     if (const int rc = plan_select(pin, plan)) return rc;
     return launch_plan(a, plan, static_cast<hipStream_t>(stream), hosted);
@@ -1073,3 +1117,16 @@
     a.kchunk = kchunk;
     return lrt_gemm_dispatch(a, LBBNN_F_MEAN_ONLY | LBBNN_F_SPLIT16, stream);
 }
+
+extern "C" int lbbnn_matmul_dual_splitk(const float* xt, int ldx, const void* gm_op, const void* gv_op, int ld,
+                                        float* dwm, float* dwv, int ldo, int M, int K, int N, int kchunk, void* stream) {
+    if (!xt || !gm_op || !gv_op || !dwm || !dwv) return LBBNN_E_NULL;
+    if (M <= 0 || K <= 0 || N <= 0 || ldo < M || K > 0x7FFFFFE0) return LBBNN_E_SHAPE;
+    if (kchunk <= 0 || (kchunk & 31)) return LBBNN_E_ALIGN;
+    const int Kp = (K + 31) & ~31;
+    if (ldx < Kp) return LBBNN_E_SHAPE;
+    if ((reinterpret_cast<uintptr_t>(dwm) | reinterpret_cast<uintptr_t>(dwv)) & 3u) return LBBNN_E_ALIGN;
+    GemmArgs a = gemm_args(xt, ldx, gm_op, gv_op, ld, dwm, ldo, M, Kp, N);
+    a.out_v = dwv; a.kchunk = kchunk;
+    return lrt_gemm_dispatch(a, LBBNN_F_DUAL_RAW | LBBNN_F_SPLIT16, stream);
+}
diff --git a/bayesian-neural-nets_amd/csrc/output_grad.hip b/bayesian-neural-nets_amd/csrc/output_grad.hip
--- a/bayesian-neural-nets_amd/csrc/output_grad.hip
+++ b/bayesian-neural-nets_amd/csrc/output_grad.hip
@@ -1,6 +1,7 @@
 #include "lbbnn_device.h"
 #include "lbbnn_internal.h"
 #include "reduce_partials.h"
+#include "operand_store.h"
 
 namespace {
 
@@ -64,13 +65,28 @@
         for (int q = 0; q < 4; ++q) { tm[r][c + q] = gm[q]; tv[r][c + q] = gv[q]; }
     }
     __syncthreads();
-#pragma unroll
-    for (int k = 0; k < 16; ++k) {
-        const int idx = tid + 256 * k, oc = idx >> 6, br = idx & 63;
-        const int o = o0 + oc, b = b0 + br;
-        if (o < a.O && b < a.B) {
-            a.gmT[(size_t)o * a.B + b] = tm[br][oc];
-            if (stoch) a.gvT[(size_t)o * a.B + b] = tv[br][oc];
+    if (a.t_ld > 0) {
+#pragma unroll
+        for (int k = 0; k < 2; ++k) {
+            const int idx = tid + 256 * k, oc = idx >> 3, br = (idx & 7) * 8;
+            const int o = o0 + oc, b = b0 + br;
+            if (o < a.O && b < a.t_ld) {
+                float wm[8], wv[8];
+#pragma unroll
+                for (int t = 0; t < 8; ++t) { wm[t] = tm[br + t][oc]; wv[t] = tv[br + t][oc]; }
+                store8_operand(a.gmT, true, (size_t)o, b, a.t_ld, wm);
+                if (stoch) store8_operand(a.gvT, true, (size_t)o, b, a.t_ld, wv);
+            }
+        }
+    } else {
+#pragma unroll
+        for (int k = 0; k < 16; ++k) {
+            const int idx = tid + 256 * k, oc = idx >> 6, br = idx & 63;
+            const int o = o0 + oc, b = b0 + br;
+            if (o < a.O && b < a.B) {
+                a.gmT[(size_t)o * a.B + b] = tm[br][oc];
+                if (stoch) a.gvT[(size_t)o * a.B + b] = tv[br][oc];
+            }
         }
     }
     if (tid < 2 * TS) {
@@ -289,6 +305,9 @@
     if (a.std && (!a.gvT || (a.g_sum && !a.gv_sum) || ((a.gm == nullptr) != (a.gv == nullptr)))) return LBBNN_E_NULL;
     if (a.std && !a.eps && !a.rng) return LBBNN_E_NOISE;
     if (a.B <= 0 || a.O <= 0 || a.ldg < a.O || ((a.relu || a.std) && a.ldo < a.O)) return LBBNN_E_SHAPE;
+    if (a.t_ld < 0 || (a.t_ld > 0 && a.t_ld < a.B)) return LBBNN_E_SHAPE;
+    if (a.t_ld > 0 && ((a.t_ld & 31) || (reinterpret_cast<uintptr_t>(a.gmT) & 15u) || (a.std && (reinterpret_cast<uintptr_t>(a.gvT) & 15u))))
+        return LBBNN_E_ALIGN;
     hipStream_t s = static_cast<hipStream_t>(stream);
     const int nbt = (a.B + TS - 1) / TS;
     hipLaunchKernelGGL(output_grad_kernel, dim3((a.O + TS - 1) / TS, nbt), dim3(256), 0, s, a, nbt);
diff --git a/bayesian-neural-nets_amd/layers.py b/bayesian-neural-nets_amd/layers.py
--- a/bayesian-neural-nets_amd/layers.py
+++ b/bayesian-neural-nets_amd/layers.py
@@ -21,6 +21,7 @@
 _DEFER_SUMS = _os.environ.get("LBBNN_DEFER_SUMS", "1") != "0"
 _LRT_BIAS_HIP = _os.environ.get("LBBNN_LRT_BIAS_HIP", "1") != "0"
 _HEAD_DW = _os.environ.get("LBBNN_HEAD_DW", "1") != "0"
+_DUAL_DW = _os.environ.get("LBBNN_DUAL_DW", "1") != "0"
 _F16_FIRST_PLANES = {"f32": False, "planes": True}.get(_os.environ.get("LBBNN_F16_FIRST", ""))
 _SIDE = {}
 
@@ -175,10 +176,12 @@
         dense = layer._mnf and ctx.saved.get("dense_save") is not None
         defer_sums = _OVERLAP["sums"] if (can_defer and (planar or dense) and _DEFER_SUMS) else None
         lrt_job = [] if (not layer._mnf and _LRT_BIAS_HIP and B > 0) else None
+        dual = _dual_dw_plan(x, layer, stochastic)
         g, g_v, gT, g_vT, g_sum, gv_sum = ops.output_grad(
             g_out, out=out if relu else None, std=std if stochastic else None, eps=explicit.get("eps_out"),
             rng=ctx.saved.get("rng"), rng_stream=ops.STREAM_EPS_OUT * 64 + layer._layer_id, row_offset=layer.row_offset,
-            relu=relu, want_g=bool(ctx.needs_input_grad[1]), defer_sums=lrt_job if lrt_job is not None else defer_sums)
+            relu=relu, want_g=bool(ctx.needs_input_grad[1]), defer_sums=lrt_job if lrt_job is not None else defer_sums,
+            t_operand=dual is not None)
         rng_snap = ctx.saved.get("rng")
         in_kernel = (planar or dense) and not explicit and rng_snap is not None
         noise = {} if in_kernel else layer._noise_for_backward(ctx.saved, B, need_out=False)
@@ -252,6 +255,11 @@
                                    nslabs=16 if (layer.out_features * layer.in_features) % 4 == 0 else 1)
             if dWm.shape[0] == 1:
                 dWm, dWv = dWm[0], (dWv[0] if dWv is not None else None)
+        elif dual is not None:
+            dWm, dWv = ops.matmul_dual_splitk(ops.transpose_operand(x), gT, g_vT, B=B, I=layer.in_features,
+                                              O=layer.out_features, kchunk=dual[1])
+            if dWm.shape[0] == 1:
+                dWm, dWv = dWm[0], dWv[0]
         else:
             pair = _x_operand_pair(x, gT, g_vT, layer) if stochastic else None
             dWm = _hip_matmul_nt(gT, ops.transpose_operand, x, allow_splitk=True, op=pair[0] if pair else None, module=layer)
@@ -321,6 +329,20 @@
             k = layer._vec_names.index("r0_c")
             vgrads[k] = dr0c if vgrads[k] is None else vgrads[k] + dr0c
         return (None, gx, None, dmu, drho, dlam, *vgrads)
+
+
+def _head_dw_ok(x, layer, B):
+    return (_HEAD_DW and layer.out_features <= 16 and x.dim() == 2 and x.stride(1) == 1 and x.dtype == torch.float32 and B >= 64)
+
+
+def _dual_dw_plan(x, layer, stochastic):
+    if not (_DUAL_DW and stochastic and ops.split_precision(layer)):
+        return None
+    if not ops.split_eligible(x.shape[0], layer.in_features) or x.data_ptr() % 16:
+        return None
+    if x.dim() != 2 or x.dtype != torch.float32 or not x.is_contiguous() or _head_dw_ok(x, layer, x.shape[0]):
+        return None
+    return ops.dual_dw_plan(x.shape[0], layer.in_features, layer.out_features)
 
 
 def _operand_split_ok(a, K, N, module=None):
diff --git a/bayesian-neural-nets_amd/ops.py b/bayesian-neural-nets_amd/ops.py
--- a/bayesian-neural-nets_amd/ops.py
+++ b/bayesian-neural-nets_amd/ops.py
@@ -15,6 +15,7 @@
 F_F16S = 0x40
 F_VAR1 = 0x80
 F_XPLANES = 0x100
+F_DUAL_RAW = 0x800
 
 STREAM_EPS_OUT = 0
 STREAM_EPS_Z = 1
@@ -194,16 +195,17 @@
 
 
 def output_grad(g_out, *, out=None, std=None, eps=None, rng=None, rng_stream: int = 0, row_offset: int = 0,
-                relu: bool = False, gv_scale=None, want_g: bool = True, defer_sums=None):
+                relu: bool = False, gv_scale=None, want_g: bool = True, defer_sums=None, t_operand: bool = False):
     B, O = g_out.shape
     f = dict(dtype=torch.float32, device=g_out.device)
     if g_out.stride(1) != 1:
         g_out = g_out.contiguous()
     stoch = std is not None
-    gm, gmT, g_sum = (torch.empty((B, O), **f) if want_g else None), torch.empty((O, B), **f), torch.empty(O, **f)
+    t_ld = operand_ld(B) if (t_operand and B > 0) else 0
+    gm, gmT, g_sum = (torch.empty((B, O), **f) if want_g else None), torch.empty((O, t_ld or B), **f), torch.empty(O, **f)
     gv = gvT = gv_sum = None
     if stoch:
-        gv, gvT, gv_sum = (torch.empty((B, O), **f) if want_g else None), torch.empty((O, B), **f), torch.empty(O, **f)
+        gv, gvT, gv_sum = (torch.empty((B, O), **f) if want_g else None), torch.empty((O, t_ld or B), **f), torch.empty(O, **f)
     if B == 0:
         g_sum.zero_()
         if stoch:
@@ -231,6 +233,7 @@
     a.row_offset, a.rng_stream = row_offset, rng_stream
     a.gv_scale = _ptr(gv_scale, "gv_scale") if (stoch and gv_scale is not None) else None
     a.B, a.O, a.ldg, a.ldo, a.relu = B, O, g_out.stride(0), ldo, 1 if relu else 0
+    a.t_ld = t_ld
     _lib.check(_lib.lib().lbbnn_output_grad(ctypes.byref(a), _stream()), "lbbnn_output_grad")
     return gm, gv, gmT, gvT, g_sum, gv_sum
 
@@ -270,6 +273,31 @@
                                         M, K, N, kchunk, _stream())
     _lib.check(rc, "lbbnn_matmul_splitk")
     return out
+
+
+def dual_dw_plan(B: int, I: int, O: int):
+    if B <= 0 or I <= 0 or O <= 16:
+        return None
+    ld = operand_ld(B)
+    if ((I - 1) * ld + ld) * 4 >= 0x7FFFFFF0 or O * ld * 4 >= 0x7FFFFFF0:
+        return None
+    tiles = ((O + 79) // 80) * ((I + 127) // 128 if I >= 96 else (I + 31) // 32)
+    S = max(1, min(16, (400 + tiles - 1) // tiles, B // 256))
+    kchunk = ((B + S - 1) // S + 31) // 32 * 32
+    return S, kchunk
+
+
+def matmul_dual_splitk(xt, gm_op, gv_op, *, B: int, I: int, O: int, kchunk: int):
+    ld = operand_ld(B)
+    if tuple(xt.shape) != (I, ld) or tuple(gm_op.shape) != (O, ld) or tuple(gv_op.shape) != (O, ld):
+        raise RuntimeError("bnn_amd: matmul_dual_splitk takes x^T (%d,%d) and operands (%d,%d)" % (I, ld, O, ld))
+    S = (ld + kchunk - 1) // kchunk if kchunk > 0 else 1
+    dWm = torch.empty((S, O, I), dtype=torch.float32, device=xt.device)
+    dWv = torch.empty((S, O, I), dtype=torch.float32, device=xt.device)
+    rc = _lib.lib().lbbnn_matmul_dual_splitk(_ptr(xt, "xt"), ld, _ptr(gm_op, "gm_op"), _ptr(gv_op, "gv_op"), ld,
+                                             dWm.data_ptr(), dWv.data_ptr(), I, I, B, O, kchunk, _stream())
+    _lib.check(rc, "lbbnn_matmul_dual_splitk")
+    return dWm, dWv
 
 
 def dx_combine(gx, gxv, x):
diff --git a/include/lbbnn.h b/include/lbbnn.h
--- a/include/lbbnn.h
+++ b/include/lbbnn.h
@@ -25,6 +25,7 @@
 #define LBBNN_F_LOG_SOFTMAX 0x8
 #define LBBNN_F_HALF16 0x20
 #define LBBNN_F_SINGLE16 0x10
+#define LBBNN_F_DUAL_RAW 0x800
 
 #define LBBNN_STREAM_EPS_OUT 0
 #define LBBNN_STREAM_EPS_Z 1
@@ -510,6 +511,7 @@
     uint32_t rng_stream;
     int B, O, ldg, ldo, relu;
     const float* gv_scale;
+    int t_ld;
 } lbbnn_outgrad_args_t;
 
 int64_t lbbnn_output_grad_workspace(int B, int O);
@@ -589,6 +591,9 @@
 
 int lbbnn_matmul_splitk(const float* x, int ldx, const void* w_op, int ld, float* out, int ldo,
                         int B, int I, int O, int kchunk, void* stream);
+
+int lbbnn_matmul_dual_splitk(const float* xt, int ldx, const void* gm_op, const void* gv_op, int ld,
+                             float* dwm, float* dwv, int ldo, int M, int K, int N, int kchunk, void* stream);
 
 typedef struct lbbnn_copy_list {
     float* dst[LBBNN_ADAM_MAX_TENSORS];
```

Measured after the change: 35.16 million. About the same (-0.1%).
